# IvanPopov/video-flow-ml

Hardware: AMD Instinct MI355X
Metric: flow-fields/sec @1080p seq5 MOF_sintel (higher is better)
Workload: dtype mixed (per-layer MFMA count, f32 accumulate): {"corr": 1, "update_block.encoder.convf1": 1, "update_block.encoder.convf2": 1, "update_block.gru.convq1.iter": "2a", "update_block.gru.convzr1.iter": 1, "update_block.gru.convzr2.iter": 1, "update_block.mask.0": 1, "update_block.mask.2": 1, "update_bloc

## Files before the change

include/vfml.h:

```cpp
#ifndef VFML_H
#define VFML_H
#include <stddef.h>
#include <stdint.h>

#ifdef __cplusplus
extern "C" {
#endif

#define VFML_ABI_VERSION 27

enum {
  VFML_EPI_NONE = 0,
  VFML_EPI_RELU = 1,
  VFML_EPI_TANH = 2,
  VFML_EPI_SIGMOID = 3,
  VFML_EPI_TANH_RELU = 4,
  VFML_EPI_GRU_ZR = 5,
  VFML_EPI_GRU_Q = 6,
  VFML_EPI_ADD_AUX = 7,
};

enum { VFML_FMT_F32 = 0, VFML_FMT_S16 = 1,
       VFML_FMT_F16 = 2 };

// ... 25 lines not shown

int vfml_conv2d(const vfml_conv_desc* d, void* stream);

int vfml_conv2d_variant(const vfml_conv_desc* d, char* buf, int len);
int vfml_conv2d_split_variant(const vfml_conv_desc* d, const void* w_hi, const void* w_lo, int kp, float w_scale,
                              int in_fmt, int out_fmt, int aux_fmt, int k_order, char* buf, int len);
int vfml_conv2d_split_variant_at(int index, char* buf, int len);

int vfml_conv2d_split(const vfml_conv_desc* d, const void* w_hi, const void* w_lo, int kp, float w_scale,
                      int in_fmt, int out_fmt, int aux_fmt, int k_order, void* stream);
enum { VFML_KORDER_TAP = 0, VFML_KORDER_CBLOCK = 1, VFML_KORDER_CBLOCK64 = 2 };

int vfml_to_s16(const float* src, int64_t rows, int c, int ld_src, float* dst, int ld_dst, float scale, void* stream);

int vfml_split_f16(const float* src, int64_t rows, int k, int ld, float scale, void* hi, void* lo, int kp,
                   void* stream);

int vfml_softmax_rows_s16(const float* x, int64_t rows, int cols, int64_t ld_in, float* out, int64_t ld_out, float scale,
                          void* stream);

int vfml_softmax_rows_f16(const float* x, int64_t rows, int cols, int64_t ld_in, void* out, int64_t ld_out, float scale,
                          void* stream);

int64_t vfml_attention_plane_workspace_bytes(int p);
int vfml_attention_plane_f16(const float* q, int64_t ld_q, const float* k, int64_t ld_k, int p, int d, float score_scale,
                             float prob_scale, void* plane, int64_t ld_plane, void* workspace, void* stream);

int vfml_attention_bank_planes_f16(const float* q, int64_t ld_q, const float* const* keys, int64_t ld_k, int n_seg, int p, int d,
                                   float score_scale, float prob_scale, void* const* planes, int64_t ld_plane, void* workspace,
                                   void* stream);

int vfml_axpy_f32(const float* x, float* y, int64_t n, float scale, void* stream);

int vfml_transpose_to_s16(const float* src, int rows, int c, int ld, float scale, float* dst, int64_t ld_dst, void* stream);

enum { VFML_DW_RESIDUAL = 1, VFML_DW_GELU = 2 };
int vfml_dwconv2d(const float* x, int64_t ld_x, int n, int h, int w, int c, int k, const float* weight, const float* bias,
                  float* out, int64_t ld_out, int in_fmt, int out_fmt, int flags, void* stream);

int vfml_gelu_rows(const float* x, int64_t ld_x, float* out, int64_t ld_out, int64_t rows, int c, int in_fmt, int out_fmt,
                   void* stream);

int vfml_layernorm_rows(const float* x, int64_t ld_x, float* out, int64_t ld_out, int64_t rows, int c, const float* gamma,
                        const float* beta, float eps, int in_fmt, int out_fmt, void* stream);

int vfml_window_attention(const float* qkv, int64_t ld, int n, int h, int w, int c, int heads, int ws, const float* pad_row,
                          float* out, int64_t ld_out, int in_fmt, int out_fmt, void* stream);

int vfml_attention_shared_keys(const float* q, int64_t ld_q, const float* kv, int64_t ld_kv, int n, int p, int pk, int c, int heads,
                               float* out, int64_t ld_out, int q_fmt, int kv_fmt, int out_fmt, void* stream);

int vfml_add_to_s16(const float* x, int64_t ldx, const float* aux, int64_t ld_aux, float* out, int64_t ld_out, int64_t rows,
                    int c, float scale, void* stream);

int vfml_transpose_split_f16(const float* src, int rows, int c, int ld, float scale, void* hi, void* lo, int kp,
                             void* stream);

int vfml_frames_to_nhwc4(const void* src, int kind, int n, int H, int W,
                         float scale, float shift, float* dst, void* stream);

int64_t vfml_instnorm_workspace_bytes(int n, int hw, int c);
int vfml_instnorm_stats(const float* x, int n, int hw, int c, float eps,
                        float* stats, void* workspace, void* stream);
int vfml_instnorm_apply(const float* x, const float* stats, const float* res,
                        const float* res_stats, int n, int hw, int c, float* out, int out_fmt, void* stream);

int vfml_avgpool2x2(const float* x, int n, int h, int w, int c, float* out, void* stream);

int vfml_corr_lookup(const float* const* pyr, const int32_t* hl, const int32_t* wl,
                     const int32_t* ld, int levels, int radius, int nmaps, int q_per_map,
                     const float* coords, int ld_coords, float* out, int ld_out, int out_fmt, int vol_fmt, int vol_tile,
                     void* stream);
#define VFML_VOL_F16_LEVELS(m) (0x100 | (m))

int vfml_corr_lookup_indirect(const float* const* table, const int32_t* hl, const int32_t* wl, const int32_t* ld,
                              int levels, int radius, int nmaps, int q_per_map, const float* coords, int ld_coords,
                              float* out, int ld_out, int out_fmt, int vol_fmt, int vol_tile, void* stream);
int vfml_corr_lookup_indirect_bidir(const float* const* table, const int32_t* hl, const int32_t* wl, const int32_t* ld,
                                    int levels, int radius, int nmaps, int q_per_map, const float* coords, int ld_coords,
                                    int dir_coords, float* out, int ld_out, int dir_out, int dir_tab, int out_fmt, int vol_fmt,
                                    int vol_tile, void* stream);
int vfml_ptr_table_set(void* table, const void* const* ptrs, int n, void* stream);

#define VFML_SEED_NONE 0
#define VFML_SEED_LOAD 1
#define VFML_SEED_STORE 2
int vfml_window_seed(const void* cells, int ncentres, int rows, int cols, float* state, int ld_state, int h_off, int mf_off,
                     int ld_ctx, void* stream);

int vfml_flow_rows7(const float* flow, int n, int h, int w, float* rows, void* stream);

int vfml_conv3x3_c64(const float* in, int ld_in, int n, int h, int w, const void* w_hi, const void* w_lo, int kp, float w_scale,
                     const float* bias, float* out, int ldo, double* stats_part, void* stream);

int vfml_flow_half(const float* flow, int n, int h, int w, const void* w1_hi, int kp1, float w1_scale, const float* b1,
                   const void* w2_hi, int kp2, float w2_scale, const float* b2, float* out, int ld_out, void* stream);

int vfml_tapsum3x3(const float* t, int ld_t, const float* bias, int n, int h, int w, float* out, int parts, int64_t part_stride,
                   void* stream);
int vfml_tapsum3x3_update(const float* t, int ld_t, const float* bias, int n, int h, int w, int parts, int64_t part_stride,
                          float* coords1, float* flow_a, int ld_a, float* flow_b, int ld_b, int fmt_b, void* stream);

int vfml_coords_update(float* coords1, const float* delta, int n, int h, int w,
                       float* flow_a, int ld_a, float* flow_b, int ld_b, int fmt_b, void* stream);

int64_t vfml_flow_forward_interpolate_workspace_bytes(int n, int h, int w);
int vfml_flow_forward_interpolate(const float* flow, int ld_in, int n, int h, int w, float* out, int ld_out, int32_t* index,
                                  void* workspace, int64_t workspace_bytes, void* stream);
int vfml_coords_init(float* coords1, int n, int h, int w, void* stream);

int vfml_convex_upsample(const float* coords1, int ch, const float* mask, int ld_mask,
                         int h, int w, float* out, void* stream);

int64_t vfml_instnorm_finalize_workspace_bytes(int chunks, int c);
int vfml_instnorm_finalize(const double* part, int n, int chunks, int c, int hw, float eps, float* stats,
                           void* workspace, int64_t workspace_bytes, void* stream);

int vfml_stem7x7s2_chunks(int h, int w);
int vfml_stem7x7s2(const float* frames, int n, int h, int w, const void* w_hi, const void* w_lo, float w_scale,
                   const float* bias, float* out, double* stats_part, void* stream);

int vfml_flow_lod(const float* flow, int h, int w, float* out, void* stream);

enum { VFML_ENCODE_GAMEDEV = 0, VFML_ENCODE_RG8 = 1, VFML_ENCODE_RGB8 = 2 };
int vfml_flow_encode(const float* flow, int h, int w, int mode, float width, float height, float scale,
                     float clamp, float two_clamp, unsigned char* out, void* stream);

enum { VFML_TAA_SIMPLE = 0, VFML_TAA_BILINEAR = 1, VFML_TAA_BILATERAL = 2 };
enum { VFML_PIX_U8 = 0, VFML_PIX_F32 = 1, VFML_PIX_F64 = 2 };
int vfml_taa_blend(const void* current, int cur_type, const float* flow, const void* history, int hist_type,
                   void* out, int out_type, int h, int w, int mode, double alpha, double sigma_color, void* stream);

int vfml_flow_quality_map(const unsigned char* frame1, const unsigned char* frame2, const float* flow, int fh, int fw,
                          int h, int w, float threshold, unsigned char* out, void* stream);

#define VFML_CORRECT_RECORD 16
size_t vfml_flow_correct_workspace_bytes(int h, int w);
int vfml_flow_correct(const unsigned char* frame1, const unsigned char* frame2, const float* flow, const float* lod,
                      int lh, int lw, int h, int w, const double* twiddles, double good_threshold,
                      double fine_threshold, double region_radius, double template_radius, double search_radius,
                      float* out_flow, int* counts, double* records, int64_t record_capacity, void* workspace,
                      size_t workspace_bytes, void* stream);

enum { VFML_COLORIZE_HSV = 0, VFML_COLORIZE_WHEEL = 1 };
int vfml_flow_colorize(const float* flow, int h, int w, int mode, void* workspace, unsigned char* out, void* stream);

int vfml_flow_decode(const unsigned char* encoded, int h, int w, int mode, float clamp, float* flow, void* stream);

int vfml_flow_diff_overlay(const float* flow_a, const float* flow_b, int h, int w, unsigned char* out, void* stream);

enum { VFML_COMPOSE_SIDE_BY_SIDE = 0, VFML_COMPOSE_STACKED = 1, VFML_COMPOSE_GRID_2X2 = 2,
       VFML_COMPOSE_GRID_2X3 = 3 };
enum { VFML_COMPOSE_BGR = 1, VFML_COMPOSE_BOTTOM_UP = 2 };
int vfml_compose_frame(const void* const* tiles, const int* tile_types, int h, int w, int layout, int flags,
                       int64_t row_stride, unsigned char* out, void* stream);

int vfml_text_draw(const int32_t* plan, int plan_words, unsigned char* img, int h, int w, int64_t row_stride, int flags,
                   void* stream);

size_t vfml_flow_turbulence_workspace_bytes(int h, int w);
int vfml_flow_turbulence_map(const float* flow, int fh, int fw, int h, int w, int ksize, void* workspace,
                             unsigned char* out_bgr, unsigned char* out_index, float* out_tv, float* out_lohi,
                             void* stream);

int vfml_resize_u8(const unsigned char* src, int n, int H, int W, int64_t src_frame_stride, unsigned char* dst, int h,
                   int w, int64_t dst_frame_stride, const int32_t* xtab, const int32_t* ytab, void* stream);
// ... 67 lines not shown
```

video-flow-ml_amd/processing/videoflow_processor.py:

```python
import collections
import hashlib
import os

import numpy as np
import torch

from .videoflow_core import VideoFlowCore

try:
    import xxhash

    def _digest(buf):
        return xxhash.xxh3_128_digest(buf)
except ImportError:
    def _digest(buf):
        return hashlib.blake2b(buf, digest_size=16).digest()

HOST_FRAME_CACHE = 24


class VideoFlowProcessor:
    def __init__(self, device, fast_mode=False, tile_mode=False, sequence_length=5,
                 dataset='sintel', architecture='mof', variant='standard'):
        self.device = device
        self.fast_mode = fast_mode
        self.tile_mode = tile_mode
        self.sequence_length = sequence_length
        self.dataset = dataset
        self.architecture = architecture
        self.variant = variant
        self.core = VideoFlowCore(device, fast_mode, dataset, architecture, variant)
        self._dev_frames = collections.OrderedDict()
        print("VideoFlow Processor initialized:")
        for label, value in (("Device", device), ("Fast mode", fast_mode), ("Tile mode", tile_mode),
                             ("Sequence length", sequence_length), ("Dataset", dataset),
                             ("Architecture", architecture.upper()), ("Variant", variant)):
            print(f"  {label}: {value}")

    def load_model(self):
        print(f"VideoFlow model loaded successfully from: {self.core.load_model()}")

    def calculate_tile_grid(self, width, height, tile_size=1280):
        cols = -(-width // tile_size)
        rows = -(-height // tile_size)
        tiles = [{'x': c * tile_size, 'y': r * tile_size,
                  'width': min(tile_size, width - c * tile_size),
                  'height': min(tile_size, height - r * tile_size),
                  'col': c, 'row': r}
                 for r in range(rows) for c in range(cols)]
        return tile_size, tile_size, cols, rows, tiles

    def extract_tile(self, frame, tile_info):
        x, y = tile_info['x'], tile_info['y']
        return frame[y:y + tile_info['height'], x:x + tile_info['width']]

    def window_indices(self, num_frames, frame_idx):
        T = self.sequence_length
        half = T // 2
        start = max(0, frame_idx - half)
        idx = list(range(start, min(num_frames, frame_idx + half + 1)))
        while len(idx) < T:
            if start == 0:
                idx.insert(0, idx[0])
            else:
                idx.append(idx[-1])
        return idx[:T]

    def prepare_frame_sequence(self, frames, frame_idx):
        planes = []
        for i in self.window_indices(len(frames), frame_idx):
            f = frames[i]
            a = f.astype(np.float32) / 255.0 if f.dtype == np.uint8 else f.astype(np.float32)
            planes.append(torch.from_numpy(a).permute(2, 0, 1))
        return torch.stack(planes).unsqueeze(0).to(self.device)

    def _require_model(self):
        if not self.core.is_model_loaded():
            raise RuntimeError("Model not loaded. Call load_model() first.")

    def _flow_from_host_u8(self, frames, frame_idx):
        model = self.core.model
        if not (str(self.device).startswith('cuda') and hasattr(model, "forward_u8")):
            return None
        ids = self.window_indices(len(frames), frame_idx)
        f0 = frames[ids[0]]
        if not all(isinstance(frames[i], np.ndarray) and frames[i].dtype == np.uint8 and frames[i].ndim == 3 and
                   frames[i].shape == f0.shape for i in set(ids)):
            return None
        H, W, C = f0.shape
        if C != 3 or H % 8 or W % 8:
            return None
        keys = {}
        for i in set(ids):
            a = np.ascontiguousarray(frames[i])
            k = ("host-u8", _digest(memoryview(a).cast("B")), a.shape)
            keys[i] = k
            if k in self._dev_frames:
                self._dev_frames.move_to_end(k)
            else:
                self._dev_frames[k] = torch.from_numpy(a).to(self.device)
                while len(self._dev_frames) > HOST_FRAME_CACHE:
                    self._dev_frames.popitem(last=False)
        win = torch.stack([self._dev_frames[keys[i]] for i in ids])
        flows, _ = model.forward_u8(win, return_lowres=False, frame_keys=[keys[i] for i in ids], pick_only=self.PICK_ONLY)
        return flows[0, flows.shape[1] // 2].permute(1, 2, 0).cpu().numpy()

    def compute_optical_flow(self, frames, frame_idx):
        self._require_model()
        fast = self._flow_from_host_u8(frames, frame_idx)
        if fast is not None:
            return fast
        flow = self.core.compute_flow_from_tensor(self.prepare_frame_sequence(frames, frame_idx))
        return flow.permute(1, 2, 0).cpu().numpy()

    def compute_optical_flow_with_progress(self, frames, frame_idx, tile_pbar=None):
        self._require_model()

        def step(desc, n=0, reset=False):
            if tile_pbar is not None:
                tile_pbar.set_description(desc)
                if reset:
                    tile_pbar.reset()
                if n:
                    tile_pbar.update(n)

        step("Preparing frames", reset=True)
        fast = self._flow_from_host_u8(frames, frame_idx)
        if fast is not None:
            step("Completed", 4)
            return fast
        batch = self.prepare_frame_sequence(frames, frame_idx)
        step("Running VideoFlow", 2)
        flow = self.core.compute_flow_from_tensor(batch)
        step("Processing output", 1)
        out = flow.permute(1, 2, 0).cpu().numpy()
        step("Completed", 1)
        return out

    def compute_optical_flow_tiled(self, frames, frame_idx, tile_pbar=None, overall_pbar=None):
        if not self.tile_mode:
            return self.compute_optical_flow(frames, frame_idx)
        height, width = frames[frame_idx].shape[:2]
        tiles = self.calculate_tile_grid(width, height)[4]
        full = np.zeros((height, width, 2), dtype=np.float32)
        for k, t in enumerate(tiles):
            if overall_pbar is not None:
                overall_pbar.set_description(f"Tile {k + 1}/{len(tiles)} ({t['width']}x{t['height']})")
            crops = [self.extract_tile(f, t) for f in frames]
            full[t['y']:t['y'] + t['height'], t['x']:t['x'] + t['width']] = \
                self.compute_optical_flow_with_progress(crops, frame_idx, tile_pbar)
            if overall_pbar is not None:
                overall_pbar.update(1)
        return full

    def upload_clip(self, frames):
        if any(f.dtype != np.uint8 for f in frames):
            raise ValueError("upload_clip expects uint8 frames")
        from vfml.clip_id import clip_token
        host = torch.from_numpy(np.stack(frames))
        if str(self.device).startswith('cuda'):
            host = host.pin_memory()
        clip = host.to(self.device, non_blocking=True)
        clip_token(clip)
        return clip

    def compute_optical_flow_resident(self, clip, frame_idx, tile=None):
        self._require_model()
        from vfml.clip_id import clip_token
        from vfml.network import take_frames
        frame_ids = self.window_indices(clip.shape[0], frame_idx)
        win = take_frames(clip, frame_ids)
        rect = None
        if tile is not None:
            rect = (tile['x'], tile['y'], tile['width'], tile['height'])
            win = win[:, tile['y']:tile['y'] + tile['height'], tile['x']:tile['x'] + tile['width']]
        H, W = win.shape[1:3]
        model = self.core.model
        if H % 8 == 0 and W % 8 == 0 and hasattr(model, "forward_u8"):
            tok = clip_token(clip)
            keys = [(tok, i, rect) for i in frame_ids]
            flows, _ = model.forward_u8(win, return_lowres=False, frame_keys=keys, pick_only=self.PICK_ONLY)
            if ((tile is None or getattr(self, "tiles_in_frame_order", False)) and frame_idx + 1 < clip.shape[0]
                    and hasattr(model, "prefetch_frames")):
                nxt = self.window_indices(clip.shape[0], frame_idx + 1)
                if (nxt != frame_ids and nxt == list(range(nxt[0], nxt[0] + len(nxt)))
                        and max(nxt) <= getattr(clip, "_vfml_frames_ready", clip.shape[0]) - 1):
                    nwin = take_frames(clip, nxt)
                    if tile is not None:
                        nwin = nwin[:, tile['y']:tile['y'] + tile['height'], tile['x']:tile['x'] + tile['width']]
                    model.prefetch_frames(nwin, [(tok, i, rect) for i in nxt])
            return flows[0, flows.shape[1] // 2].permute(1, 2, 0)
        batch = (win.float() / 255.0).permute(0, 3, 1, 2).unsqueeze(0)
        return self.core.compute_flow_from_tensor(batch).permute(1, 2, 0)

    def compute_optical_flow_resident_batch(self, clip, frame_idxs):
        self._require_model()
        from vfml.clip_id import clip_token
        from vfml.network import take_frames
        model = self.core.model
        frame_idxs = list(frame_idxs)
        F, H, W = clip.shape[0], clip.shape[1], clip.shape[2]
        can_batch = getattr(model, "tri_frame", False) and hasattr(model, "forward_u8") and H % 8 == 0 and W % 8 == 0
        lo = self.sequence_length // 2 - 1
        triples = [self.window_indices(F, i)[lo:lo + 3] if self.sequence_length >= 3 else None for i in frame_idxs]
        out, k = [], 0
        while k < len(frame_idxs):
            e = k
            if can_batch and triples[k] is not None and triples[k][0] + 1 == triples[k][1] == triples[k][2] - 1:
                while (e + 1 < len(frame_idxs) and e + 1 - k < self.TRI_BATCH and
                       triples[e + 1] == [t + 1 for t in triples[e]]):
                    e += 1
            if e == k:
                out.append(self.compute_optical_flow_resident(clip, frame_idxs[k]))
            else:
                B = e - k + 1
                ids = list(range(triples[k][0], triples[e][2] + 1))
                tok = clip_token(clip)
                keys = [(tok, i, None) for i in ids]
                flows, _ = model.forward_u8(take_frames(clip, ids), return_lowres=False, frame_keys=keys, tri_batch=True)
                out.extend(flows[0, B + j].permute(1, 2, 0) for j in range(B))
            k = e + 1
        return out

    TRI_BATCH = int(os.environ.get("VFML_TRI_BATCH", "8"))
    PICK_ONLY = not os.environ.get("VFML_FULL_OUTPUT")

    def is_model_loaded(self):
        return self.core.is_model_loaded()

    def get_model_info(self):
        info = self.core.get_model_info()
        if info["status"] == "loaded":
            info.update(tile_mode=self.tile_mode, sequence_length=self.sequence_length,
                        processor_type="VideoFlowProcessor")
        return info

    def get_memory_usage(self):
        return self.core.get_memory_usage()

    def validate_frames(self, frames, frame_idx):
        if not isinstance(frames, list):
            raise ValueError("Frames must be a list of numpy arrays")
        if not frames:
            raise ValueError("Frames list cannot be empty")
        if not 0 <= frame_idx < len(frames):
            raise ValueError(f"Frame index {frame_idx} out of range [0, {len(frames)-1}]")
        f = frames[0]
        if not isinstance(f, np.ndarray):
            raise ValueError("Frames must be numpy arrays")
        if f.ndim != 3:
            raise ValueError(f"Frames must be 3D arrays [H,W,C], got shape {f.shape}")
        if f.shape[2] != 3:
            raise ValueError(f"Frames must have 3 color channels, got {f.shape[2]}")
        if f.dtype not in (np.uint8, np.float32, np.float64):
            raise ValueError(f"Unsupported frame dtype: {f.dtype}")
        if f.dtype != np.uint8:
            lo, hi = float(f.min()), float(f.max())
            if (hi > 1.0 or lo < 0.0) and not (hi <= 255.0 and lo >= 0.0):
                raise ValueError("Float frames must be in range [0.0, 1.0] or [0.0, 255.0]")

    def set_tile_mode(self, enabled):
        self.tile_mode = enabled

    def set_sequence_length(self, length):
# ... 4 lines not shown
```

video-flow-ml_amd/vfml/csrc/conv_gemm_split.hip:

```cpp
#include "conv_split_common.h"

namespace {

template <int BN, int WM, int WN, bool BIGC, bool IN16, int NM = 3>
__global__ __launch_bounds__(WM * WN * 64, 2) void conv_gemm_split_kernel(const SplitArgs a) {
  constexpr bool ALO = NM == 3 || NM == 2, BLO = NM == 3 || NM == 4;
  constexpr int NT = WM * WN * 64;
  constexpr int LR = NT / 4;
  constexpr int TM = BM / (WM * 32);
  constexpr int TN = BN / (WN * 32);
  constexpr int AU = BM / LR;
  constexpr int BU = BN / LR;
  constexpr int BUN = BU > 0 ? BU : 1;
  constexpr int RSA = BM + 2;
  constexpr int RSB = BN + 2;
  constexpr int SA = KG * RSA;
  constexpr int SB = KG * RSB;
  constexpr int LDC = BN + 4;

  extern __shared__ __attribute__((aligned(16))) char smem_raw[];
  h16x8* sAh = reinterpret_cast<h16x8*>(smem_raw);
  h16x8* sAl = sAh + 2 * SA;
  h16x8* sBh = sAl + 2 * SA;
  h16x8* sBl = sBh + 2 * SB;
  float* sC = reinterpret_cast<float*>(smem_raw);

  const int nwg = a.mtiles * a.ntiles;
  int bid = blockIdx.x;
  {
    const int q = nwg >> 3, r = nwg & 7, xcd = bid & 7;
    bid = (xcd < r ? xcd * (q + 1) : r * (q + 1) + (xcd - r) * q) + (bid >> 3);
  }
  const int nt = bid % a.ntiles;
  const int mt = bid / a.ntiles;
  const int m0 = mt * BM;
  const int n0 = nt * BN;

  const int t = threadIdx.x;
  const int kg = t & 3;
  const int lrow = t >> 2;

  int rp0[AU], rp1[AU];
  unsigned long long tapok[AU];
#pragma unroll
  for (int i = 0; i < AU; ++i) {
    const int m = m0 + lrow + LR * i;
    int iy0[1], ix0[1];
    tapok[i] = 0ull;
    if (m < a.M) {
      const int hw = a.ho * a.wo;
      const int n = m / hw;
      const int rem = m - n * hw;
      const int oy = rem / a.wo;
      const int ox = rem - oy * a.wo;
      iy0[0] = oy * a.stride - a.pad_h;
      ix0[0] = ox * a.stride - a.pad_w;
      const int pix = (n * a.H + iy0[0]) * a.W + ix0[0];
      rp0[i] = pix * a.ld0 + a.d0off;
      rp1[i] = pix * a.ld1 + a.d1off;
      for (int ky = 0; ky < a.kh; ++ky)
        for (int kx = 0; kx < a.kw; ++kx)
          if ((unsigned)(iy0[0] + ky) < (unsigned)a.H && (unsigned)(ix0[0] + kx) < (unsigned)a.W)
            tapok[i] |= 1ull << (ky * a.kw + kx);
    } else {
      rp0[i] = rp1[i] = 0;
    }
  }
  int kc[2], kky[2], kkx[2];
#pragma unroll
  for (int hf = 0; hf < 2; ++hf) {
    const int k = kg * 8 + hf * 4;
    const int tap = k / a.ctot;
    kc[hf] = k - tap * a.ctot;
    kky[hf] = tap / a.kw;
    kkx[hf] = tap - kky[hf] * a.kw;
  }
  int colbase[BUN];
#pragma unroll
  for (int i = 0; i < BUN; ++i) {
    const int col = n0 + lrow + LR * i;
    const bool colok = (BU > 0 || lrow < BN) && col < a.cout;
    colbase[i] = colok ? col * a.Kp * 2 : 0x40000000;
  }
// ... 96 lines not shown
      for (int e = 0; e < 16; ++e) acc[i][j][e] = 0.f;

  auto compute = [&](int buf) {
    const int oa = buf * SA + wm * (BM / WM) + r;
    const int ob = buf * SB + wn * (BN / WN) + r;
#pragma unroll
    for (int ks = 0; ks < KG / 2; ++ks) {
      h16x8 ah[TM], al[TM], bh[TN], bl[TN];
#pragma unroll
      for (int i = 0; i < TM; ++i) {
        ah[i] = sAh[oa + (2 * ks + half) * RSA + i * 32];
        if constexpr (ALO) al[i] = sAl[oa + (2 * ks + half) * RSA + i * 32];
      }
#pragma unroll
      for (int j = 0; j < TN; ++j) {
        bh[j] = sBh[ob + (2 * ks + half) * RSB + j * 32];
        if constexpr (BLO) bl[j] = sBl[ob + (2 * ks + half) * RSB + j * 32];
      }
#pragma unroll
      for (int i = 0; i < TM; ++i)
#pragma unroll
        for (int j = 0; j < TN; ++j) {
          acc[i][j] = __builtin_amdgcn_mfma_f32_32x32x16_f16(ah[i], bh[j], acc[i][j], 0, 0, 0);
          if constexpr (BLO) acc[i][j] = __builtin_amdgcn_mfma_f32_32x32x16_f16(ah[i], bl[j], acc[i][j], 0, 0, 0);
          if constexpr (ALO) acc[i][j] = __builtin_amdgcn_mfma_f32_32x32x16_f16(al[i], bh[j], acc[i][j], 0, 0, 0);
        }
    }
  };

  const int nk = ((a.K + BK - 1) / BK + 1) & ~1;
  load_tile(st0, 0);
  load_tile(st1, BK);
  store_tile(st0, 0);
  __syncthreads();
  for (int kt = 0; kt < nk; kt += 2) {
    load_tile(st0, (kt + 2) * BK);
    __builtin_amdgcn_sched_barrier(0);
    compute(0);
    __builtin_amdgcn_sched_barrier(0);
    store_tile(st1, 1);
    __syncthreads();
    load_tile(st1, (kt + 3) * BK);
    __builtin_amdgcn_sched_barrier(0);
    compute(1);
    __builtin_amdgcn_sched_barrier(0);
    store_tile(st0, 0);
    __syncthreads();
  }

  acc_to_lds<TM, TN, LDC>(acc, sC, wm * (BM / WM), wn * (BN / WN), r, half);
  __syncthreads();
  if (!epilogue_rows_fast<BN, NT>(a, sC, m0, n0, t, BM, 32, 0)) epilogue_rows<BN, NT>(a, sC, m0, n0, t);
  if (a.stats_part) {
    constexpr int RG = NT / BN;
    const int ch = t % BN, rg = t / BN;
    double s1 = 0.0, s2 = 0.0;
    if (n0 + ch < a.cout) {
      const float b = a.bias ? a.bias[n0 + ch] : 0.f;
      for (int row = rg; row < BM; row += RG) {
        if (m0 + row >= a.M) break;
        const double v = (double)((sC[row * LDC + ch] * a.w_inv + b) * a.out_scale);
        s1 += v;
        s2 += v * v;
      }
    }
    __syncthreads();
    double* fold = reinterpret_cast<double*>(sC);
    fold[(rg * BN + ch) * 2] = s1;
    fold[(rg * BN + ch) * 2 + 1] = s2;
    __syncthreads();
    if (rg == 0 && n0 + ch < a.cout) {
      for (int g = 1; g < RG; ++g) {
        s1 += vfml_lds_f64(&fold[(g * BN + ch) * 2]);
        s2 += vfml_lds_f64(&fold[(g * BN + ch) * 2 + 1]);
      }
      double* o = a.stats_part + ((int64_t)(m0 / BM) * a.cout + n0 + ch) * 2;
      o[0] = s1;
      o[1] = s2;
    }
  }
}



template <bool H16, bool BIAS>
__device__ __forceinline__ void gemm_resident_walk(const SplitArgs& a, char* smem) {
  constexpr int NW = 4;
  constexpr int RBM = 128, RBN = 64;
  constexpr int NSTEP = VFML_RESIDENT_KMAX / 64;
  constexpr int ASTEP = RBM * 128, BSTEP = RBN * 128;
  constexpr int BOFF = 0, BBUF = NSTEP * BSTEP, SLAB = BOFF + 2 * BBUF;
  constexpr int AP = RBM / (8 * NW), BP = RBN / (8 * NW);
  constexpr int ES = H16 ? 2 : 4;
  constexpr int NSTORE = 8, NSTORE_T = 16;
  constexpr int STORE_NT = 2;
  static_assert(NSTEP * ASTEP == 2 * BBUF, "the A image of a unit fills the two B buffers");
  static_assert(SLAB + NW * 32 * 32 * 4 == VFML_RESIDENT_LDS, "LDS budget of the resident-A walk: two workgroups per CU");

  const int t = threadIdx.x;
  const int lane = t & 63;
  const int wave = __builtin_amdgcn_readfirstlane(t >> 6);
  const int lrow = 8 * wave + (lane >> 3);
  const int piece = (lane & 7) ^ ((4 * wave + (lane >> 4)) & 7);
  const int nk = (a.Kp / 64 + 1) & ~1;
  const __amdgpu_buffer_rsrc_t rb = __builtin_amdgcn_make_buffer_rsrc(const_cast<char*>(a.wbase), 0, a.bytesb, 0x00020000);
  const int r = lane & 31, half = lane >> 5;
  const int q16 = (((r >> 1) & 7) ^ half) * 16;
  const int aoff = (wave * 32 + r) * 128 + q16;
  const int boff = r * 128 + q16;
  float* ws = reinterpret_cast<float*>(smem + SLAB) + wave * (32 * 32);
  const int c4 = (lane % 8) * 4, rr = lane / 8;

  const int units = a.mtiles * a.res_nc;
  for (int u = blockIdx.x; u < units; u += gridDim.x) {
    const int run = u / a.mtiles, mt = u - run * a.mtiles;
    const int nt0 = run * a.res_cl;
    const int nt1 = nt0 + a.res_cl < a.ntiles ? nt0 + a.res_cl : a.ntiles;
    const int m0 = mt * RBM;
    const int rows_valid = a.M - m0 < RBM ? a.M - m0 : RBM;
    __amdgpu_buffer_rsrc_t r0;
    if (a.tilebase)
      r0 = __builtin_amdgcn_make_buffer_rsrc(const_cast<float*>(a.in0) + (int64_t)m0 * a.ld0, 0,
                                             ((rows_valid - 1) * a.ld0 + a.d0off + a.c0) * 4, 0x00020000);
    else
      r0 = __builtin_amdgcn_make_buffer_rsrc(const_cast<float*>(a.in0), 0, a.bytes0, 0x00020000);
    int va[AP];
#pragma unroll
    for (int j = 0; j < AP; ++j) {
      const int m = m0 + 8 * NW * j + lrow;
      const int mrow = a.tilebase ? m - m0 : m;
      va[j] = m < a.M ? (mrow * a.ld0 + a.d0off) * 4 + piece * 32 : OOB;
    }
    auto issue_b = [&](int nt, int buf) {
      int colbase[BP];
#pragma unroll
      for (int j = 0; j < BP; ++j) {
        const int col = nt * RBN + 8 * NW * j + lrow;
        colbase[j] = col < a.cout ? a.whi_off + col * a.Kp * 2 + piece * 16 : (a.bhi ? 0x7ffffff0 : 0x40000000);
      }
      for (int s = 0; s < nk; ++s)
#pragma unroll
        for (int j = 0; j < BP; ++j)
          dma16(rb, colbase[j], s * 128, smem + BOFF + buf * BBUF + s * BSTEP + wave * (8 * 128) + j * (8 * NW * 128));
    };

    h16x8 af[4 * NSTEP];
#pragma unroll
    for (int q = 0; q < 4 * NSTEP; ++q) af[q] = h16x8{0, 0, 0, 0, 0, 0, 0, 0};
    lds_barrier();
    for (int s = 0; s < nk; ++s) {
      const bool past = s * 64 >= a.ctot;
#pragma unroll
      for (int j = 0; j < AP; ++j)
        dma16(r0, past ? OOB : va[j], s * 256, smem + s * ASTEP + wave * (8 * 128) + j * (8 * NW * 128));
    }
    asm volatile("s_waitcnt vmcnt(0)" ::: "memory");
    lds_barrier();
    static_for<NSTEP>([&](auto sc) {
      constexpr int s = decltype(sc)::value;
      if (s < nk) {
#pragma unroll
        for (int ks = 0; ks < 4; ++ks) af[s * 4 + ks] = *reinterpret_cast<const h16x8*>(smem + s * ASTEP + (aoff ^ (ks * 32)));
      }
    });
    lds_barrier();
    issue_b(nt0, 0);

    for (int nt = nt0; nt < nt1; ++nt) {
      const int buf = (nt - nt0) & 1;
      const int n0 = nt * RBN;
      if (nt == nt0) asm volatile("s_waitcnt vmcnt(0)" ::: "memory");
      else if (a.out_t) asm volatile("s_waitcnt vmcnt(%0)" ::"n"(NSTORE_T) : "memory");
      else asm volatile("s_waitcnt vmcnt(%0)" ::"n"(NSTORE) : "memory");
      lds_barrier();
      f32x4 bv[2] = {{0.f, 0.f, 0.f, 0.f}, {0.f, 0.f, 0.f, 0.f}};
      if constexpr (BIAS) {
#pragma unroll
        for (int j = 0; j < 2; ++j)
          if (n0 + j * 32 + c4 < a.cout) bv[j] = *reinterpret_cast<const f32x4*>(a.bias + n0 + j * 32 + c4);
      }
      if (nt + 1 < nt1) issue_b(nt + 1, buf ^ 1);

      f32x16 acc[2];
#pragma unroll
      for (int j = 0; j < 2; ++j)
#pragma unroll
        for (int e = 0; e < 16; ++e) acc[j][e] = 0.f;
      const char* bb = smem + BOFF + buf * BBUF;
      static_for<NSTEP / 2>([&](auto pc) {
        constexpr int s0 = 2 * decltype(pc)::value;
        if (s0 < nk) {
          h16x8 b0[8], b1[8];
#pragma unroll
          for (int q = 0; q < 8; ++q) {
            b0[q] = *reinterpret_cast<const h16x8*>(bb + (s0 + (q >> 2)) * BSTEP + (boff ^ ((q & 3) * 32)));
            b1[q] = *reinterpret_cast<const h16x8*>(bb + (s0 + (q >> 2)) * BSTEP + (boff ^ ((q & 3) * 32)) + 4096);
          }
#pragma unroll
          for (int q = 0; q < 8; ++q) {
            acc[0] = __builtin_amdgcn_mfma_f32_32x32x16_f16(af[s0 * 4 + q], b0[q], acc[0], 0, 0, 0);
            acc[1] = __builtin_amdgcn_mfma_f32_32x32x16_f16(af[s0 * 4 + q], b1[q], acc[1], 0, 0, 0);
          }
        }
      });

      const int cols_valid = a.cout - n0 < RBN ? a.cout - n0 : RBN;
      char* tbase = reinterpret_cast<char*>(a.out) + ((int64_t)m0 * a.ldo + n0) * ES;
      const __amdgpu_buffer_rsrc_t ro =
          __builtin_amdgcn_make_buffer_rsrc(tbase, 0, ((rows_valid - 1) * a.ldo + cols_valid) * ES, 0x00020000);
      const int rows_t = cols_valid, cols_t = rows_valid;
      __amdgpu_buffer_rsrc_t rt = ro;
      if (a.out_t) {
        char* tbase_t = reinterpret_cast<char*>(a.out_t) + ((int64_t)n0 * a.ld_out_t + m0) * ES;
        rt = __builtin_amdgcn_make_buffer_rsrc(tbase_t, 0, ((rows_t - 1) * a.ld_out_t + cols_t) * ES, 0x00020000);
      }
      static_for<2>([&](auto jc) {
        constexpr int j = decltype(jc)::value;
        const int gcol = j * 32 + c4;
#pragma unroll
        for (int e = 0; e < 16; ++e) ws[((e & 3) + 8 * (e >> 2) + 4 * half) * 32 + r] = acc[j][e];
#pragma unroll
        for (int p = 0; p < 4; ++p) {
          f32x4 v = *reinterpret_cast<const f32x4*>(ws + (p * 8 + rr) * 32 + c4);
#pragma unroll
          for (int e = 0; e < 4; ++e) {
            v[e] = (v[e] * a.w_inv + bv[j][e]) * a.out_scale;
            if (a.epilogue == VFML_EPI_RELU) v[e] = fmaxf(v[e], 0.f);
          }
          const int off = gcol < cols_valid ? ((wave * 32 + p * 8 + rr) * a.ldo + gcol) * ES : OOB;
          if constexpr (H16) {
            const h16x2 p0 = {(_Float16)v[0], (_Float16)v[1]}, p1 = {(_Float16)v[2], (_Float16)v[3]};
            const u32x2 hv = {__builtin_bit_cast(unsigned, p0), __builtin_bit_cast(unsigned, p1)};
            __builtin_amdgcn_raw_buffer_store_b64(hv, ro, off, 0, STORE_NT);
          } else {
            __builtin_amdgcn_raw_buffer_store_b128(__builtin_bit_cast(u32x4, v), ro, off, 0, STORE_NT);
          }
        }
        if (a.out_t) {
#pragma unroll
          for (int e = 0; e < 16; ++e) {
            const int row = (e & 3) + 8 * (e >> 2) + 4 * half;
            ws[r * 32 + ((row + (r >> 1)) & 31)] = acc[j][e];
          }
          const int g = lane >> 3, cl = lane & 7;
#pragma unroll
          for (int pp = 0; pp < 4; ++pp) {
            const int c = pp * 8 + cl;
            f32x4 v;
#pragma unroll
            for (int k = 0; k < 4; ++k) v[k] = ws[c * 32 + ((4 * g + k + (c >> 1)) & 31)] * a.w_inv * a.out_scale;
            const int trow = j * 32 + c;
            const int q0 = wave * 32 + 4 * g;
            const bool ok = trow < rows_t && q0 < cols_t;
            if constexpr (H16) {
              const h16x2 p0 = {(_Float16)v[0], (_Float16)v[1]}, p1 = {(_Float16)v[2], (_Float16)v[3]};
              const u32x2 hv = {__builtin_bit_cast(unsigned, p0), __builtin_bit_cast(unsigned, p1)};
              __builtin_amdgcn_raw_buffer_store_b64(hv, rt, ok ? (trow * a.ld_out_t + q0) * 2 : OOB, 0, STORE_NT);
            } else {
              __builtin_amdgcn_raw_buffer_store_b128(__builtin_bit_cast(u32x4, v), rt, ok ? (trow * a.ld_out_t + q0) * 4 : OOB, 0, STORE_NT);
            }
          }
        }
      });
    }
  }
}

template <int TM, int TN, int WM, int WN, bool PERSIST, bool FASTK, bool CSWAP = false, int NM = 3, bool MF16 = false, bool H16 = false>
__global__ __launch_bounds__(WM * WN * 64, (WM * WN == 4 ? 2 : 1)) void conv_gemm_dma_kernel(const SplitArgs a) {
  static_assert(!H16 || PERSIST, "VFML_FMT_F16 outputs (H16) exist in the persistent GEMM form only");
  static_assert(!(MF16 && PERSIST), "the persistent GEMM form runs 32x32x16 MFMAs (its 16x16x32 epilogue branches below are not maintained)");
  constexpr bool H64 = NM == 5;
  static_assert(!H64 || FASTK, "64-channel steps exist for the uniform-step loader only");
  constexpr bool BHI = NM == 2 || NM == 1 || H64;
  constexpr bool AHI = NM == 4 || NM == 1 || H64;
  constexpr int KSTEP = H64 ? 64 : BK;
  constexpr int NW = WM * WN, NT = NW * 64;
  constexpr int TBM = 32 * TM * WM, TBN = 32 * TN * WN;
  constexpr int AP = TBM / (8 * NW), BP = TBN / (8 * NW);
  static_assert(TBM % (8 * NW) == 0 && TBN % (8 * NW) == 0, "tile rows must split into whole pieces per wave");
  constexpr int ASZ = TBM * 128, BSZ = TBN * 128, STG = ASZ + BSZ;
  constexpr int LDC = TBN + 4;

  extern __shared__ __attribute__((aligned(16))) char smem_raw[];
  float* sC = reinterpret_cast<float*>(smem_raw);

  if constexpr (PERSIST && FASTK && !CSWAP && NM == 5 && !MF16) {
    if (a.resident) {
      if (a.bias) gemm_resident_walk<H16, true>(a, smem_raw);
      else gemm_resident_walk<H16, false>(a, smem_raw);
      return;
    }
  }

  const int total = a.mtiles * a.ntiles * (PERSIST ? a.ksplit : 1);
  int tile, tile_end, tile_step;
  {
    const int G = gridDim.x, xcd = blockIdx.x & 7, lw = blockIdx.x >> 3;
    const int q = total >> 3, r = total & 7;
    const int start = xcd < r ? xcd * (q + 1) : r * (q + 1) + (xcd - r) * q;
    tile_step = (G - xcd + 7) >> 3;
    tile = start + lw;
    tile_end = start + q + (xcd < r ? 1 : 0);
  }
  if (tile >= tile_end) return;

  const int t = threadIdx.x;
  const int lane = t & 63;
  const int wave = __builtin_amdgcn_readfirstlane(t >> 6);
  const int lrow = 8 * wave + (lane >> 3);
  const int piece = (lane & 7) ^ (MF16 && !H64 ? swz16((4 * wave + (lane >> 4)) & 7) : ((4 * wave + (lane >> 4)) & 7));
  const int kg = piece >> 1, hl = piece & 1;

  int rp0[AP], rp1[AP];
  unsigned long long tapok[AP];
  int colbase[BP];
  int kc, kky, kkx;
  int scb = 0, sky = 0, skx = 0;
  int m0, n0;
  int ks = 0;
  __amdgpu_buffer_rsrc_t r0 = __builtin_amdgcn_make_buffer_rsrc(
      reinterpret_cast<char*>(const_cast<float*>(a.in0)) - a.abias, 0, a.bytes0 + a.abias, 0x00020000);
  const __amdgpu_buffer_rsrc_t rb = __builtin_amdgcn_make_buffer_rsrc(const_cast<char*>(a.wbase), 0, a.bytesb, 0x00020000);

  const int nk = PERSIST && a.ksplit == 2 ? (((a.Kp / KSTEP + 1) >> 1) + 1) & ~1 : (a.Kp / KSTEP + 1) & ~1;
  auto setup = [&](int tl) {
    int nt, mt;
    if (PERSIST && a.ksplit == 2) {
      ks = tl & 1;
      tl >>= 1;
    }
    if (a.ntiles >= 8) {
      constexpr int GM = 8;
      const int gsz = GM * a.ntiles;
      const int g = tl / gsz, rem = tl - g * gsz;
      const int left = a.mtiles - g * GM;
      const int mrows = left < GM ? left : GM;
      nt = rem / mrows;
      mt = g * GM + (rem - nt * mrows);
    } else {
      nt = tl % a.ntiles;
      mt = tl / a.ntiles;
    }
    m0 = mt * TBM;
    n0 = nt * TBN;
#pragma unroll
    for (int j = 0; j < AP; ++j) {
      const int m = m0 + 8 * NW * j + lrow;
      tapok[j] = 0ull;
// ... 1030 lines not shown
             (out_fmt == VFML_FMT_F32 || out_fmt == VFML_FMT_F16) && !d->stats_part &&
             (d->cout >= DIRECT_MIN_COUT || out_fmt == VFML_FMT_F16) && d->cout % 4 == 0 && d->ldo % 4 == 0 && vfml_aligned16(d->out) &&
             (!d->bias || vfml_aligned16(d->bias));
  VFML_REQUIRE(out_fmt != VFML_FMT_F16 || (a.direct && a.fastk),
               "vfml_conv2d_split: VFML_FMT_F16 outputs are written by the GEMM form only (1x1 over whole 32-channel blocks, no "
               "addend / activation beyond ReLU, cout %% 4 == 0, ldo %% 4 == 0, 16-byte aligned out)");
  if (d->flags & VFML_CONV_SWAP_CROSS) {
    VFML_REQUIRE(a.direct && a.fastk, "vfml_conv2d_split: VFML_CONV_SWAP_CROSS is implemented by the GEMM form only "
                                      "(1x1 over whole 32-channel blocks, plain f32 out, cout >= 1024, cout %% 4 == 0)");
    a.cswap = 1;
  }
  if (bhi)
    VFML_REQUIRE(a.direct && a.fastk && !a.cswap, "vfml_conv2d_split: a weight operand without lo plane is implemented by the "
                                                    "GEMM form only (1x1 over whole 32-channel blocks, plain f32 out, cout >= 1024)");
  if (d->out_t) {
    VFML_REQUIRE(a.direct && a.fastk && a.pointwise && !d->bias && d->epilogue == VFML_EPI_NONE && a.M % 4 == 0 &&
                 d->ld_out_t % 4 == 0 && d->ld_out_t >= a.M && vfml_aligned16(d->out_t),
                 "vfml_conv2d_split: out_t needs the GEMM form (1x1 over whole 32-channel blocks, plain f32 out, cout >= 1024, cout %% 4 == 0), no bias / "
                 "epilogue, pixels %% 4 == 0, ld_out_t %% 4 == 0 and >= pixels, 16-byte alignment");
    a.out_t = d->out_t; a.ld_out_t = d->ld_out_t;
  }
  if (d->ksplit_ws) {
    VFML_REQUIRE(vfml_aligned16(d->ksplit_ws), "vfml_conv2d_split: ksplit_ws must be 16-byte aligned");
    const int64_t tiles = (int64_t)((a.M + 127) / 128) * ((d->cout + 127) / 128);
    const bool ksplit = a.direct && a.fastk && a.pointwise && out_fmt == VFML_FMT_F32 && !a.cswap && tiles <= 256 &&
                        kp >= 4096;
    if (ksplit) {
      a.ksplit = 2;
      a.out_k1 = d->ksplit_ws;
      a.out_t_k1 = d->ksplit_ws + (int64_t)a.M * d->ldo;
    }
  }
  if (d->proj_out) {
    VFML_REQUIRE(d->epilogue == VFML_EPI_RELU && !d->addend && !d->stats_part && !d->out_t && !a.direct,
                 "vfml_conv2d_split: proj_out goes with VFML_EPI_RELU, no addend / stats_part / out_t");
    VFML_REQUIRE(a.fastk && (a.nm == 3 || a.nm == 4) && d->cout % 128 == 0,
                 "vfml_conv2d_split: proj_out needs the uniform-step loader (channel-block weight order, whole 32-channel "
                 "blocks), the full split product or VFML_CONV_MFMA2A (which then holds for the projection too) and "
                 "cout %% 128 == 0");
    VFML_REQUIRE(d->proj_hi && d->proj_lo && d->proj_n > 0 && d->proj_n <= 48 && d->proj_n % 4 == 0 && d->proj_kp >= d->cout &&
                     d->proj_kp % 8 == 0 && d->ld_proj >= d->proj_n && d->ld_proj % 4 == 0 && vfml_aligned16(d->proj_out) &&
                     vfml_aligned16(d->proj_hi) && vfml_aligned16(d->proj_lo) && d->proj_scale > 0.f,
                 "vfml_conv2d_split: proj_hi / proj_lo [proj_n <= 48, %% 4 == 0][proj_kp >= cout] f16 planes, ld_proj >= proj_n, "
                 "16-byte alignment");
    const char* ph2 = (const char*)d->proj_hi;
    const char* pl2 = (const char*)d->proj_lo;
    const int64_t plane = (int64_t)d->proj_n * d->proj_kp * 2;
    VFML_REQUIRE(pl2 >= ph2 && (pl2 - ph2) + plane < (1ll << 30), "vfml_conv2d_split: proj_lo must follow proj_hi within 1 GiB");
    a.proj_w = ph2; a.proj_lo_off = (int)(pl2 - ph2); a.proj_bytes = (int)((pl2 - ph2) + plane);
    a.proj_n = d->proj_n; a.proj_kp = d->proj_kp; a.proj_inv = 1.0f / d->proj_scale;
    a.proj_out = d->proj_out; a.ld_proj = d->ld_proj;
  }
  return 0;
}

static int dma_tile_env() {
  const char* tile_env = getenv("VFML_DMA_TILE");
  if (!tile_env) return 0;
  int tm = 2, tn = 2, wm = 2, wn = 2;
  sscanf(tile_env, "%d,%d,%d,%d", &tm, &tn, &wm, &wn);
  return tm * 1000 + tn * 100 + wm * 10 + wn;
}

static int split_prepare(const vfml_conv_desc* d, const void* w_hi, const void* w_lo, int kp, float w_scale, int in_fmt, int out_fmt,
                         int aux_fmt, int k_order, int forced_tile, SplitArgs& a, SplitPlan& plan, const SplitVariant*& row) {
  if (const int rc = split_fill(d, w_hi, w_lo, kp, w_scale, in_fmt, out_fmt, aux_fmt, k_order, a)) return rc;
  if (const int rc = vfml_detail::plan_split(a, in_fmt == VFML_FMT_S16, d->flags, forced_tile, &plan)) return rc;
  a.nm = plan.nm;
  a.fastk = plan.fastk;
  a.resident = plan.resident ? 1 : 0;
  if (!plan.fastk) a.abias = 0;
  row = plan.family == vfml_detail::SPLIT_TAPX ? vfml_detail::tapx_variant(plan)
        : plan.family == vfml_detail::SPLIT_DMA ? vfml_detail::find_variant(DMA_VARIANTS, sizeof(DMA_VARIANTS) / sizeof(DMA_VARIANTS[0]), plan)
                                                : vfml_detail::find_variant(REG_VARIANTS, sizeof(REG_VARIANTS) / sizeof(REG_VARIANTS[0]), plan);
  if (!row) {
    char name[160];
    vfml_detail::variant_name(plan, name, sizeof(name));
    vfml_set_error("vfml_conv2d_split: no such variant: %s", name);
    return 1;
  }
  return 0;
}

extern "C" int vfml_conv2d_split(const vfml_conv_desc* d, const void* w_hi, const void* w_lo, int kp, float w_scale,
                                 int in_fmt, int out_fmt, int aux_fmt, int k_order, void* stream) {
  SplitArgs a;
  SplitPlan plan;
  const SplitVariant* row;
  if (const int rc = split_prepare(d, w_hi, w_lo, kp, w_scale, in_fmt, out_fmt, aux_fmt, k_order, dma_tile_env(), a, plan, row)) return rc;
  hipStream_t s = reinterpret_cast<hipStream_t>(stream);
  const int rc = row->launch(a, s);
  if (rc || !plan.add_rows) return rc;
  const int64_t quads = (int64_t)a.M * (d->cout / 4);
  const dim3 grid((unsigned)((quads + 255) / 256 < 65535 * 16 ? (quads + 255) / 256 : 65535 * 16));
  hipLaunchKernelGGL(add_rows_kernel, grid, dim3(256), 0, s, d->out, d->ksplit_ws, a.M, d->cout / 4, d->ldo);
  if (d->out_t)
    hipLaunchKernelGGL(add_rows_kernel, grid, dim3(256), 0, s, d->out_t, a.out_t_k1, d->cout, a.M / 4, d->ld_out_t);
  return vfml_check_launch("vfml_conv2d_split");
}

extern "C" int vfml_conv2d_split_variant(const vfml_conv_desc* d, const void* w_hi, const void* w_lo, int kp, float w_scale,
                                         int in_fmt, int out_fmt, int aux_fmt, int k_order, char* buf, int len) {
  VFML_REQUIRE(buf && len > 0, "vfml_conv2d_split_variant: no buffer");
  SplitArgs a;
  SplitPlan plan;
  const SplitVariant* row;
  if (const int rc = split_prepare(d, w_hi, w_lo, kp, w_scale, in_fmt, out_fmt, aux_fmt, k_order, dma_tile_env(), a, plan, row)) return rc;
  VFML_REQUIRE(vfml_detail::variant_name(row->key, buf, len) < len, "vfml_conv2d_split_variant: the name needs more than %d bytes", len);
  return 0;
}


extern "C" int vfml_conv2d_split_variant_at(int index, char* buf, int len) {
  VFML_REQUIRE(buf && len > 0, "vfml_conv2d_split_variant_at: no buffer");
  constexpr int nreg = (int)(sizeof(REG_VARIANTS) / sizeof(REG_VARIANTS[0])), ndma = (int)(sizeof(DMA_VARIANTS) / sizeof(DMA_VARIANTS[0]));
  if (index < 0) return 1;
  const SplitVariant* row = index < nreg          ? &REG_VARIANTS[index]
                            : index < nreg + ndma ? &DMA_VARIANTS[index - nreg]
                                                  : vfml_detail::tapx_variant_at(index - nreg - ndma);
  if (!row) return 1;
  VFML_REQUIRE(vfml_detail::variant_name(row->key, buf, len) < len, "vfml_conv2d_split_variant_at: the name needs more than %d bytes", len);
  return 0;
}
```

video-flow-ml_amd/vfml/csrc/conv_split_common.h:

```cpp
#pragma once
#include <hip/hip_fp16.h>
#include <stdlib.h>
#include <utility>
#include "vfml_common.h"


namespace vfml_detail {
struct SplitArgs {
  const float* in0; const float* in1;
  const _Float16* whi; const _Float16* wlo; const float* bias;
  const float* aux0; const float* aux1; const float* addend;
  float* out;
  int c0, ld0, c1, ld1, ctot, ld_addend;
  int H, W, ho, wo;
  int kh, kw, stride, pad_h, pad_w;
  int M, K, Kp, cout;
  int d0off, d1off;
  int bytes0, bytesw;
  int ldo, ld_aux0, ld_aux1;
  int epilogue, split;
  float out_scale, w_inv;
  int mtiles, ntiles;
  int vec_ok;
  int out16, aux16;
  int out_h16;
  const char* wbase; int whi_off, wlo_off, bytesb;
  int korder;
  int direct;
  int pointwise;
  int fastk, abias, src1_delta;
  int tilebase;
  float* out_t; int ld_out_t;
  int cswap;
  int bhi;
  double* stats_part;
  int nm;
  int ksplit; float* out_k1; float* out_t_k1;
  const char* proj_w; int proj_lo_off, proj_bytes, proj_n, proj_kp; float proj_inv; float* proj_out; int ld_proj;
  const float* const* addend_ind;
  int resident, res_nc, res_cl;
};
#define VFML_RESIDENT_KMAX 256
#define VFML_RESIDENT_LDS (80 * 1024)
#define VFML_TAPX_KWMAX 5

enum SplitFamily { SPLIT_REG, SPLIT_DMA, SPLIT_TAPX };
struct SplitPlan {
  SplitFamily family;
  int bn;
  int tm, tn;
  int wm, wn;
  bool bigc, in16;
  bool persist, fastk, cswap, mf16, h16;
  int nm;
  bool add_rows;
  bool resident;
};
int plan_split(const SplitArgs& a, bool in16, int flags, int forced_tile, SplitPlan* plan);
constexpr SplitPlan reg_plan(int bn, int wm, int wn, bool bigc, bool in16, int nm) {
  return {SPLIT_REG, bn, 0, 0, wm, wn, bigc, in16, false, false, false, false, false, nm, false};
}
constexpr SplitPlan dma_plan(int tm, int tn, int wm, int wn, bool persist, bool fastk, bool cswap, int nm, bool mf16, bool h16) {
  return {SPLIT_DMA, 0, tm, tn, wm, wn, false, false, persist, fastk, cswap, mf16, h16, nm, false};
}
constexpr SplitPlan tapx_plan(int tm, int tn, int wm, int wn, int nm) {
  return {SPLIT_TAPX, 0, tm, tn, wm, wn, false, false, false, true, false, true, false, nm, false};
}
struct SplitVariant {
  SplitPlan key;
  int (*launch)(SplitArgs& a, hipStream_t s);
};
const SplitVariant* find_variant(const SplitVariant* rows, size_t n, const SplitPlan& plan);
int variant_name(const SplitPlan& key, char* buf, int len);
const SplitVariant* tapx_variant(const SplitPlan& plan);
const SplitVariant* tapx_variant_at(int index);
}
using vfml_detail::SplitArgs;
using vfml_detail::SplitPlan;
using vfml_detail::SplitVariant;

namespace {

template <class F, int... I>
__device__ __forceinline__ void static_for_impl(F&& f, std::integer_sequence<int, I...>) {
  (f(std::integral_constant<int, I>{}), ...);
}
template <int N, class F>
__device__ __forceinline__ void static_for(F&& f) {
  static_for_impl(f, std::make_integer_sequence<int, N>{});
}

typedef _Float16 h16x8 __attribute__((ext_vector_type(8)));
typedef _Float16 h16x2 __attribute__((ext_vector_type(2)));
typedef __fp16 fp16x2 __attribute__((ext_vector_type(2)));

constexpr int BM = 128;
constexpr int BK = 32;
constexpr int KG = BK / 8;

typedef unsigned int u32x4 __attribute__((ext_vector_type(4)));
typedef unsigned int u32x2 __attribute__((ext_vector_type(2)));

__device__ __forceinline__ u32x4 bload16(__amdgpu_buffer_rsrc_t rsrc, int voff_bytes) {
  return __builtin_bit_cast(u32x4, __builtin_amdgcn_raw_buffer_load_b128(rsrc, voff_bytes, 0, 0));
}
constexpr int OOB = 0x7fffffff;

__device__ __forceinline__ float sigmoidf_(float v) { return 1.0f / (1.0f + expf(-v)); }

typedef const __attribute__((address_space(1))) float* vfml_gfptr;
typedef const __attribute__((address_space(1))) f32x4* vfml_gf4ptr;
__device__ __forceinline__ vfml_gfptr addend_of(const SplitArgs& a) {
  return (vfml_gfptr)(a.addend_ind ? *a.addend_ind : a.addend);
}

union U8 {
  h16x8 v;
  h16x2 p[4];
};

__device__ __forceinline__ void split4(const f32x4 x, U8& hi, U8& lo, int at) {
#pragma unroll
  for (int e = 0; e < 2; ++e) vfml_split2(x[2 * e], x[2 * e + 1], hi.p[at / 2 + e], lo.p[at / 2 + e]);
}

__device__ __forceinline__ float epi1(float v, int epilogue, bool lowhalf, float x0, float x1) {
  switch (epilogue) {
    case VFML_EPI_RELU: return fmaxf(v, 0.f);
    case VFML_EPI_TANH: return tanhf(v);
    case VFML_EPI_SIGMOID: return sigmoidf_(v);
    case VFML_EPI_TANH_RELU: return lowhalf ? tanhf(v) : fmaxf(v, 0.f);
    case VFML_EPI_GRU_ZR: v = sigmoidf_(v); return lowhalf ? v : v * x0;
    case VFML_EPI_GRU_Q: return (1.f - x0) * x1 + x0 * tanhf(v);
    case VFML_EPI_ADD_AUX: return x0 + v;
    default: return v;
  }
}

template <int TM, int TN, int LDC>
__device__ __forceinline__ void acc_to_lds(const f32x16 (&acc)[TM][TN], float* sC, int row0, int col0, int r, int half) {
#pragma unroll
  for (int j = 0; j < TN; ++j)
#pragma unroll
    for (int i = 0; i < TM; ++i)
#pragma unroll
      for (int e = 0; e < 16; ++e) {
        const int row = row0 + i * 32 + (e & 3) + 8 * (e >> 2) + 4 * half;
        const int col = col0 + j * 32 + r;
        sC[row * LDC + col] = acc[i][j][e];
      }
}

template <int BN, int NT>
__device__ __forceinline__ void epilogue_rows(const SplitArgs& a, const float* sC, int m0, int n0, int t,
                                              int nrows = BM, int rstride = 32, int roff = 0) {
  constexpr int LDC = BN + 4;
  constexpr int C8 = BN / 8;
  constexpr int RPP = NT / C8;
// ... 315 lines not shown
```

video-flow-ml_amd/vfml/csrc/flow_ops.hip:

```cpp
#include <stdlib.h>
#include "vfml_common.h"

namespace {

constexpr int MAX_LEVELS = 6;
constexpr int MAX_MAPS = 8;
constexpr int MAX_RADIUS = 4;
constexpr int PATCH = 2 * MAX_RADIUS + 2;
#ifndef VFML_LOOKUP_WAVES
#define VFML_LOOKUP_WAVES 4
#endif
constexpr int LOOKUP_WAVES = VFML_LOOKUP_WAVES;
constexpr int FIXED_LEVELS = 4;
static_assert(FIXED_LEVELS == 4, "corr_lookup_fixed_kernel selects among four levels");

struct LookupArgs {
  const float* pyr[MAX_MAPS][MAX_LEVELS];
  const float* const* table;
  int hl[MAX_LEVELS], wl[MAX_LEVELS], ld[MAX_LEVELS];
  int levels, radius, nq, q_per_map;
  const float* coords; int ld_coords;
  float* out; int ld_out;
  int out16;
  int vol16;
  int tws, ths;
  int qw;
  int dir_maps, dir_coords, dir_out;
  int dir_tab;
};

__device__ __forceinline__ void lookup_rows(const LookupArgs& a, int q, int& map, int64_t& crow, int64_t& orow) {
  const int dir = a.dir_maps && map >= a.dir_maps;
  const int64_t qd = q - (dir ? a.dir_maps * a.q_per_map : 0);
  if (dir) map += a.dir_tab - a.dir_maps;
  crow = qd * a.ld_coords + (dir ? a.dir_coords : 0);
  orow = qd * a.ld_out + (dir ? a.dir_out : 0);
}

__device__ __forceinline__ int tiled_at(int y, int x, int w, int tws, int ths) {
  const int tpr = (w + (1 << tws) - 1) >> tws;
  return ((((y >> ths) * tpr + (x >> tws)) << (tws + ths)) + ((y & ((1 << ths) - 1)) << tws) + (x & ((1 << tws) - 1)));
}

__device__ __forceinline__ float bilinear4(float nw, float ne, float sw, float se, float wx0, float fx, float wy0, float fy) {
  float v = ne * (fx * wy0);
  v = __builtin_fmaf(nw, wx0 * wy0, v);
  v = __builtin_fmaf(sw, wx0 * fy, v);
  v = __builtin_fmaf(se, fx * fy, v);
  return v;
}

__global__ __launch_bounds__(64 * LOOKUP_WAVES) void corr_lookup_kernel(const LookupArgs a) {
  __shared__ float patch[LOOKUP_WAVES][MAX_LEVELS][PATCH * PATCH];
  __shared__ float frac[LOOKUP_WAVES][MAX_LEVELS][2];
  const int lane = threadIdx.x & 63;
  const int wv = threadIdx.x >> 6;
  const int q = blockIdx.x * LOOKUP_WAVES + wv;
  const bool live = q < a.nq;
  int map = live ? q / a.q_per_map : 0;
  const int qq = q - map * a.q_per_map;
  const int side = 2 * a.radius + 2;
  const int win = 2 * a.radius + 1;
  const int psz = side * side;
  int64_t crow = 0, orow = 0;
  if (live) lookup_rows(a, q, map, crow, orow);
  if (live) {
    const float cx = a.coords[crow + 0];
    const float cy = a.coords[crow + 1];
    const int total = a.levels * psz;
    const int qrow = (a.tws | a.ths) ? tiled_at(qq / a.qw, qq % a.qw, a.qw, a.tws, a.ths) : qq;
    for (int e = lane; e < total; e += 64) {
      const int l = e / psz;
      const int idx = e - l * psz;
      const int py = idx / side, px = idx - py * side;
      const float inv = 1.0f / (float)(1 << l);
      const float x = cx * inv, y = cy * inv;
      const float fx0 = floorf(x), fy0 = floorf(y);
      const int x0 = (int)fminf(fmaxf(fx0, -65536.f), 65536.f) - a.radius;
      const int y0 = (int)fminf(fmaxf(fy0, -65536.f), 65536.f) - a.radius;
      const int xx = x0 + px, yy = y0 + py;
      float v = 0.f;
      if (xx >= 0 && xx < a.wl[l] && yy >= 0 && yy < a.hl[l])
        v = (a.table ? a.table[map * a.levels + l] : a.pyr[map][l])[(int64_t)qrow * a.ld[l] + tiled_at(yy, xx, a.wl[l], a.tws, a.ths)];
      patch[wv][l][idx] = v;
      if (idx == 0) {
        frac[wv][l][0] = x - fx0;
        frac[wv][l][1] = y - fy0;
      }
    }
  }
  __syncthreads();
  if (!live) return;
  const int nout = a.levels * win * win;
  float* o = a.out + orow;
  const int nwrite = a.out16 ? (nout + 7) & ~7 : nout;
  for (int c = lane; c < nwrite; c += 64) {
    if (c >= nout) {
      _Float16* u = reinterpret_cast<_Float16*>(o + (c & ~7));
      u[c & 7] = (_Float16)0.f;
      u[8 + (c & 7)] = (_Float16)0.f;
      continue;
    }
    const int l = c / (win * win);
    const int rem = c - l * win * win;
    const int i = rem / win, j = rem - i * win;
    const float fx = frac[wv][l][0], fy = frac[wv][l][1];
    const float* p = &patch[wv][l][j * side + i];
    const float wx0 = 1.f - fx, wy0 = 1.f - fy;
    const float v = bilinear4(p[0], p[1], p[side], p[side + 1], wx0, fx, wy0, fy);
    if (a.out16) {
      vfml_h16x2 hh, ll;
      vfml_split2(v, 0.f, hh, ll);
      _Float16* u = reinterpret_cast<_Float16*>(o + (c & ~7));
      u[c & 7] = hh[0];
      u[8 + (c & 7)] = ll[0];
    } else {
      o[c] = v;
    }
  }
}

__device__ __forceinline__ float bilinear4w(float nw, float ne, float sw, float se, float w00, float w10, float w01, float w11) {
  float v = ne * w10;
  v = __builtin_fmaf(nw, w00, v);
  v = __builtin_fmaf(sw, w01, v);
  v = __builtin_fmaf(se, w11, v);
  return v;
}

__device__ __forceinline__ void wave_lds_sync() {
  __builtin_amdgcn_fence(__ATOMIC_RELEASE, "workgroup");
  __builtin_amdgcn_wave_barrier();
  __builtin_amdgcn_fence(__ATOMIC_ACQUIRE, "workgroup");
}

template <int R, bool OUT16, int V16 = 0>
__global__ __launch_bounds__(64 * LOOKUP_WAVES) void corr_lookup_fixed_kernel(const LookupArgs a) {
  constexpr int SIDE = 2 * R + 2, PSZ = SIDE * SIDE, WIN = 2 * R + 1, WW = WIN * WIN;
  constexpr int NOUTPAD = (FIXED_LEVELS * WW + 7) & ~7;
  static_assert(PSZ <= 128 && FIXED_LEVELS * WIN <= 64 && NOUTPAD / 8 <= 64, "one wave: at most two gather passes per level");
  __shared__ float patch[LOOKUP_WAVES][FIXED_LEVELS][PSZ];
  __shared__ __attribute__((aligned(16))) float outs[LOOKUP_WAVES][NOUTPAD];
  const int lane = threadIdx.x & 63;
  const int wv = __builtin_amdgcn_readfirstlane(threadIdx.x >> 6);
  const int q = blockIdx.x * LOOKUP_WAVES + wv;
  if (q >= a.nq) return;
  int map = __builtin_amdgcn_readfirstlane(q / a.q_per_map);
  const int qq = q - map * a.q_per_map;
  const int qrow = __builtin_amdgcn_readfirstlane((a.tws | a.ths) ? tiled_at(qq / a.qw, qq % a.qw, a.qw, a.tws, a.ths) : qq);
  int64_t crow, orow;
  lookup_rows(a, q, map, crow, orow);
  const float cx = a.coords[crow + 0];
  const float cy = a.coords[crow + 1];
  const int pyA = lane / SIDE, pxA = lane - pyA * SIDE;
  const int pyB = (lane + 64) / SIDE, pxB = (lane + 64) - pyB * SIDE;
  const bool inB = lane + 64 < PSZ;
  const float* pl[FIXED_LEVELS];
  if (a.table) {
#pragma unroll
    for (int l = 0; l < FIXED_LEVELS; ++l) pl[l] = a.table[map * a.levels + (l < a.levels ? l : 0)];
  } else {
#pragma unroll
    for (int l = 0; l < FIXED_LEVELS; ++l) pl[l] = a.pyr[map][l < a.levels ? l : 0];
  }
  float va[FIXED_LEVELS], vb[FIXED_LEVELS];
  bool oka[FIXED_LEVELS], okb[FIXED_LEVELS];
#pragma unroll
  for (int l = 0; l < FIXED_LEVELS; ++l) {
    const bool have = l < a.levels;
    const int ll = have ? l : 0;
    const bool v16 = (V16 >> l) & 1;
    const int ES = v16 ? 2 : 4;
    const char* base = reinterpret_cast<const char*>(pl[l]) + (int64_t)qrow * a.ld[ll] * ES;
    const int wl = a.wl[ll], hl = a.hl[ll];
    const float inv = __builtin_bit_cast(float, (127 - l) << 23);
    const float x = cx * inv, y = cy * inv;
    const int x0 = (int)fminf(fmaxf(floorf(x), -65536.f), 65536.f) - R;
    const int y0 = (int)fminf(fmaxf(floorf(y), -65536.f), 65536.f) - R;
    auto texel = [&](int px, int py, bool in, float& out, bool& ok) {
      const int xx = x0 + px, yy = y0 + py;
      ok = have && in && xx >= 0 && xx < wl && yy >= 0 && yy < hl;
      const int at = tiled_at(min(max(yy, 0), hl - 1), min(max(xx, 0), wl - 1), wl, a.tws, a.ths);
      if (v16) out = (float)((const __attribute__((address_space(1))) _Float16*)base)[at];
      else out = ((const __attribute__((address_space(1))) float*)base)[at];
    };
    texel(pxA, pyA, true, va[l], oka[l]);
    if constexpr (PSZ > 64) texel(pxB, pyB, inB, vb[l], okb[l]);
    else { vb[l] = 0.f; okb[l] = false; }
  }
#pragma unroll
  for (int l = 0; l < FIXED_LEVELS; ++l) {
    va[l] = oka[l] ? va[l] : 0.f;
    vb[l] = okb[l] ? vb[l] : 0.f;
  }
#pragma unroll
  for (int l = 0; l < FIXED_LEVELS; ++l) {
    if (l < a.levels) {
      if (PSZ > 64 || lane < PSZ) patch[wv][l][lane] = va[l];
      if constexpr (PSZ > 64) if (inB) patch[wv][l][lane + 64] = vb[l];
    }
  }
  const int nout = a.levels * WW;
  const int nunits = (nout + 7) >> 3;
  if (lane >= 56 && nout + (lane - 56) < nunits * 8) outs[wv][nout + (lane - 56)] = 0.f;
  wave_lds_sync();
  if (lane < a.levels * WIN) {
    const int l = lane / WIN, i = lane - l * WIN;
    const float inv = __builtin_bit_cast(float, (127 - l) << 23);
    const float x = cx * inv, y = cy * inv;
    const float fx = x - floorf(x), fy = y - floorf(y);
    const float wx0 = 1.f - fx, wy0 = 1.f - fy;
    const float w00 = wx0 * wy0, w10 = fx * wy0, w01 = wx0 * fy, w11 = fx * fy;
    const float* p = &patch[wv][l][i];
    float* o = &outs[wv][l * WW + i * WIN];
    float nw = p[0], ne = p[1];
#pragma unroll
    for (int j = 0; j < WIN; ++j) {
      const float sw = p[(j + 1) * SIDE], se = p[(j + 1) * SIDE + 1];
      o[j] = bilinear4w(nw, ne, sw, se, w00, w10, w01, w11);
      nw = sw; ne = se;
    }
  }
  wave_lds_sync();
  if (lane < nunits) {
    float* o = a.out + orow + lane * 8;
    const f32x4 v0 = *reinterpret_cast<const f32x4*>(&outs[wv][lane * 8]);
    const f32x4 v1 = *reinterpret_cast<const f32x4*>(&outs[wv][lane * 8 + 4]);
    if (OUT16) {
      vfml_h16x2 h0, h1, h2, h3, l0, l1, l2, l3;
      vfml_split2(v0[0], v0[1], h0, l0);
      vfml_split2(v0[2], v0[3], h1, l1);
      vfml_split2(v1[0], v1[1], h2, l2);
      vfml_split2(v1[2], v1[3], h3, l3);
      uint4 hv, lv;
      hv.x = __builtin_bit_cast(unsigned, h0); hv.y = __builtin_bit_cast(unsigned, h1);
      hv.z = __builtin_bit_cast(unsigned, h2); hv.w = __builtin_bit_cast(unsigned, h3);
      lv.x = __builtin_bit_cast(unsigned, l0); lv.y = __builtin_bit_cast(unsigned, l1);
      lv.z = __builtin_bit_cast(unsigned, l2); lv.w = __builtin_bit_cast(unsigned, l3);
      *reinterpret_cast<uint4*>(o) = hv;
      *reinterpret_cast<uint4*>(o + 4) = lv;
    } else {
#pragma unroll
      for (int h = 0; h < 2; ++h) {
        const int c = lane * 8 + 4 * h;
        const f32x4 w = h ? v1 : v0;
        if (c + 3 < nout && (((uintptr_t)(o + 4 * h)) & 15u) == 0) {
          *reinterpret_cast<f32x4*>(o + 4 * h) = w;
        } else {
#pragma unroll
          for (int k = 0; k < 4; ++k)
            if (c + k < nout) o[4 * h + k] = w[k];
        }
      }
    }
  }
}

__global__ void coords_init_kernel(f32x4* __restrict__ coords, int h, int w, int64_t total) {
  for (int64_t p = (int64_t)blockIdx.x * blockDim.x + threadIdx.x; p < total; p += (int64_t)gridDim.x * blockDim.x) {
    const int x = (int)(p % w);
    const int y = (int)((p / w) % h);
// ... 483 lines not shown
```

video-flow-ml_amd/vfml/hip.py:

```python
import ctypes
import os
import subprocess
from ctypes import POINTER, c_char_p, c_double, c_float, c_int, c_int32, c_int64, c_void_p

import torch

_HERE = os.path.dirname(os.path.abspath(__file__))
LIB_PATH = os.environ.get("VFML_LIB") or os.path.join(_HERE, "libvfml_hip.so")
CSRC = os.path.join(_HERE, "csrc")
SOURCES = ["api.hip", "conv_gemm.hip", "conv_gemm_split.hip", "conv_gemm_tapx.hip", "conv_split_plan.hip", "stem.hip", "flow_half.hip", "enc_conv.hip", "norm_pool.hip", "flow_ops.hip", "effects.hip", "correct.hip", "render.hip", "text.hip", "turbulence.hip", "resize.hip", "jpeg.hip", "jpeg_decode.hip", "jpeg_decode_sync.hip", "deflate.hip", "attention.hip", "dwconv.hip", "twins.hip", "warm_start.hip"]

STATS_ROWS_F32, STATS_ROWS_S16 = 128, 32
EPI_NONE, EPI_RELU, EPI_TANH, EPI_SIGMOID, EPI_TANH_RELU, EPI_GRU_ZR, EPI_GRU_Q, EPI_ADD_AUX = range(8)
FMT_F32, FMT_S16, FMT_F16 = 0, 1, 2


def vol_f16_levels(mask):
    return 0x100 | mask


def _vol_mask(vol_fmt, levels):
    return (15 if vol_fmt == FMT_F16 else (vol_fmt & 15 if vol_fmt & 0x100 else 0)) & ((1 << levels) - 1)

KORDER_TAP, KORDER_CBLOCK, KORDER_CBLOCK64 = 0, 1, 2
CONV_SWAP_CROSS, CONV_MFMA2, CONV_MFMA1, CONV_MFMA2A, CONV_PER_TAP = 1, 2, 4, 8, 16


class ConvDesc(ctypes.Structure):
    _fields_ = [
        ("in0", c_void_p), ("c0", c_int32), ("ld0", c_int32),
        ("in1", c_void_p), ("c1", c_int32), ("ld1", c_int32),
        ("n", c_int32), ("h", c_int32), ("w", c_int32),
        ("weight", c_void_p), ("bias", c_void_p),
        ("cout", c_int32), ("kh", c_int32), ("kw", c_int32), ("stride", c_int32),
        ("pad_h", c_int32), ("pad_w", c_int32),
        ("out", c_void_p), ("ldo", c_int32),
        ("epilogue", c_int32), ("split", c_int32), ("out_scale", c_float),
        ("aux0", c_void_p), ("ld_aux0", c_int32),
        ("aux1", c_void_p), ("ld_aux1", c_int32),
        ("addend", c_void_p), ("ld_addend", c_int32),
        ("out_t", c_void_p), ("ld_out_t", c_int32),
        ("flags", c_int32),
        ("stats_part", c_void_p),
        ("ksplit_ws", c_void_p),
        ("proj_hi", c_void_p), ("proj_lo", c_void_p), ("proj_n", c_int32), ("proj_kp", c_int32), ("proj_scale", c_float),
        ("proj_out", c_void_p), ("ld_proj", c_int32),
        ("addend_ind", c_void_p),
    ]


COMMON_FLAGS = ["-fno-slp-vectorize"]
EXTRA_FLAGS = {}


def build(force=False, verbose=False):
    srcs = [os.path.join(CSRC, s) for s in SOURCES]
    hdrs = [os.path.join(CSRC, "vfml_common.h"), os.path.join(CSRC, "conv_split_common.h"),
            os.path.join(CSRC, "jet_table.inc"), os.path.join(CSRC, "jpeg_tables.inc"), os.path.join(CSRC, "jpeg_decode_common.h"),
            os.path.join(CSRC, "jpeg_sync_steps.h"), os.path.join(CSRC, "deflate_code.h"), os.path.join(_HERE, "..", "..", "include", "vfml.h")]
    deps = srcs + hdrs
    if not force and os.path.exists(LIB_PATH) and all(
            os.path.getmtime(LIB_PATH) >= os.path.getmtime(d) for d in deps):
        return LIB_PATH
    objdir = os.path.join(CSRC, "_obj")
    os.makedirs(objdir, exist_ok=True)
    newest_hdr = max(os.path.getmtime(h) for h in hdrs)
    jobs = []
    for src in srcs:
        obj = os.path.join(objdir, os.path.basename(src) + ".o")
        if force or not os.path.exists(obj) or os.path.getmtime(obj) < max(os.path.getmtime(src), newest_hdr):
            cmd = ["hipcc", "--offload-arch=gfx950", "-O3", "-std=c++17", "-fPIC"] + COMMON_FLAGS + EXTRA_FLAGS.get(os.path.basename(src), []) + [
                "-c", src, "-o", obj]
            if verbose:
                print(" ".join(cmd))
            jobs.append((cmd, subprocess.Popen(cmd)))
    for cmd, p in jobs:
        if p.wait() != 0:
            raise subprocess.CalledProcessError(p.returncode, cmd)
    cmd = ["hipcc", "--offload-arch=gfx950", "-fPIC", "-shared", "-o", LIB_PATH] + [
        os.path.join(objdir, os.path.basename(src) + ".o") for src in srcs]
    if verbose:
        print(" ".join(cmd))
    subprocess.run(cmd, check=True)
    return LIB_PATH


_lib = None


def lib():
    global _lib
    if _lib is not None:
        return _lib
    if not os.path.exists(LIB_PATH):
        raise RuntimeError(
            f"vfml HIP extension not built: {LIB_PATH} is missing. Run `python -c 'import __graft_entry__ as g; "
            f"g.build()'` (needs hipcc). There is no CPU fallback for the flow engine.")
    L = ctypes.CDLL(LIB_PATH)
    L.vfml_last_error.restype = c_char_p
    L.vfml_abi_version.restype = c_int
    L.vfml_conv2d.argtypes = [POINTER(ConvDesc), c_void_p]
    L.vfml_conv2d_split.argtypes = [POINTER(ConvDesc), c_void_p, c_void_p, c_int, c_float, c_int, c_int, c_int, c_int,
                                    c_void_p]
    L.vfml_conv2d_variant.argtypes = [POINTER(ConvDesc), c_char_p, c_int]
    L.vfml_conv2d_split_variant.argtypes = L.vfml_conv2d_split.argtypes[:-1] + [c_char_p, c_int]
    L.vfml_conv2d_split_variant_at.argtypes = [c_int, c_char_p, c_int]
    L.vfml_to_s16.argtypes = [c_void_p, c_int64, c_int, c_int, c_void_p, c_int, c_float, c_void_p]
    L.vfml_softmax_rows_s16.argtypes = [c_void_p, c_int64, c_int, c_int64, c_void_p, c_int64, c_float, c_void_p]
    L.vfml_transpose_split_f16.argtypes = [c_void_p, c_int, c_int, c_int, c_float, c_void_p, c_void_p, c_int, c_void_p]
    L.vfml_split_f16.argtypes = [c_void_p, c_int64, c_int, c_int, c_float, c_void_p, c_void_p, c_int, c_void_p]
    L.vfml_frames_to_nhwc4.argtypes = [c_void_p, c_int, c_int, c_int, c_int, c_float, c_float, c_void_p, c_void_p]
    L.vfml_instnorm_workspace_bytes.restype = c_int64
    L.vfml_instnorm_workspace_bytes.argtypes = [c_int, c_int, c_int]
    L.vfml_instnorm_stats.argtypes = [c_void_p, c_int, c_int, c_int, c_float, c_void_p, c_void_p, c_void_p]
    L.vfml_softmax_rows_f16.argtypes = [c_void_p, c_int64, c_int, c_int64, c_void_p, c_int64, c_float, c_void_p]
    L.vfml_attention_plane_workspace_bytes.restype = c_int64
    L.vfml_attention_plane_workspace_bytes.argtypes = [c_int]
    L.vfml_attention_plane_f16.argtypes = [c_void_p, c_int64, c_void_p, c_int64, c_int, c_int, c_float, c_float, c_void_p, c_int64,
                                           c_void_p, c_void_p]
    L.vfml_attention_bank_planes_f16.argtypes = [c_void_p, c_int64, POINTER(c_void_p), c_int64, c_int, c_int, c_int, c_float, c_float,
                                                 POINTER(c_void_p), c_int64, c_void_p, c_void_p]
    L.vfml_axpy_f32.argtypes = [c_void_p, c_void_p, c_int64, c_float, c_void_p]
    L.vfml_dwconv2d.argtypes = [c_void_p, c_int64, c_int, c_int, c_int, c_int, c_int, c_void_p, c_void_p, c_void_p, c_int64, c_int, c_int,
                                c_int, c_void_p]
    L.vfml_gelu_rows.argtypes = [c_void_p, c_int64, c_void_p, c_int64, c_int64, c_int, c_int, c_int, c_void_p]
    L.vfml_layernorm_rows.argtypes = [c_void_p, c_int64, c_void_p, c_int64, c_int64, c_int, c_void_p, c_void_p, c_float, c_int, c_int,
                                      c_void_p]
    L.vfml_window_attention.argtypes = [c_void_p, c_int64, c_int, c_int, c_int, c_int, c_int, c_int, c_void_p, c_void_p, c_int64,
                                        c_int, c_int, c_void_p]
    L.vfml_attention_shared_keys.argtypes = [c_void_p, c_int64, c_void_p, c_int64, c_int, c_int, c_int, c_int, c_int, c_void_p,
                                             c_int64, c_int, c_int, c_int, c_void_p]
    L.vfml_transpose_to_s16.argtypes = [c_void_p, c_int, c_int, c_int, c_float, c_void_p, c_int64, c_void_p]
    L.vfml_add_to_s16.argtypes = [c_void_p, c_int64, c_void_p, c_int64, c_void_p, c_int64, c_int64, c_int, c_float, c_void_p]
    L.vfml_instnorm_finalize.argtypes = [c_void_p, c_int, c_int, c_int, c_int, c_float, c_void_p, c_void_p, c_int64, c_void_p]
    L.vfml_instnorm_finalize_workspace_bytes.restype = c_int64
    L.vfml_instnorm_finalize_workspace_bytes.argtypes = [c_int, c_int]
    L.vfml_stem7x7s2_chunks.argtypes = [c_int, c_int]
    L.vfml_stem7x7s2.argtypes = [c_void_p, c_int, c_int, c_int, c_void_p, c_void_p, c_float, c_void_p, c_void_p, c_void_p, c_void_p]
    L.vfml_instnorm_apply.argtypes = [c_void_p, c_void_p, c_void_p, c_void_p, c_int, c_int, c_int, c_void_p, c_int, c_void_p]
    L.vfml_avgpool2x2.argtypes = [c_void_p, c_int, c_int, c_int, c_int, c_void_p, c_void_p]
    L.vfml_corr_lookup.argtypes = [POINTER(c_void_p), POINTER(c_int32), POINTER(c_int32), POINTER(c_int32),
                                   c_int, c_int, c_int, c_int, c_void_p, c_int, c_void_p, c_int, c_int, c_int, c_int, c_void_p]
    L.vfml_corr_lookup_indirect.argtypes = [c_void_p, POINTER(c_int32), POINTER(c_int32), POINTER(c_int32),
                                            c_int, c_int, c_int, c_int, c_void_p, c_int, c_void_p, c_int, c_int, c_int, c_int,
                                            c_void_p]
    L.vfml_corr_lookup_indirect_bidir.argtypes = [c_void_p, POINTER(c_int32), POINTER(c_int32), POINTER(c_int32),
                                                  c_int, c_int, c_int, c_int, c_void_p, c_int, c_int, c_void_p, c_int, c_int,
                                                  c_int, c_int, c_int, c_int, c_void_p]
    L.vfml_ptr_table_set.argtypes = [c_void_p, POINTER(c_void_p), c_int, c_void_p]
    L.vfml_window_seed.argtypes = [c_void_p, c_int, c_int, c_int, c_void_p, c_int, c_int, c_int, c_int, c_void_p]
    L.vfml_tapsum3x3_update.argtypes = [c_void_p, c_int, c_void_p, c_int, c_int, c_int, c_int, ctypes.c_int64, c_void_p, c_void_p,
                                        c_int, c_void_p, c_int, c_int, c_void_p]
    L.vfml_conv3x3_c64.argtypes = [c_void_p, c_int, c_int, c_int, c_int, c_void_p, c_void_p, c_int, c_float, c_void_p, c_void_p,
                                   c_int, c_void_p, c_void_p]
    L.vfml_flow_half.argtypes = [c_void_p, c_int, c_int, c_int, c_void_p, c_int, c_float, c_void_p, c_void_p, c_int, c_float,
                                 c_void_p, c_void_p, c_int, c_void_p]
    L.vfml_coords_init.argtypes = [c_void_p, c_int, c_int, c_int, c_void_p]
    L.vfml_flow_rows7.argtypes = [c_void_p, c_int, c_int, c_int, c_void_p, c_void_p]
    L.vfml_tapsum3x3.argtypes = [c_void_p, c_int, c_void_p, c_int, c_int, c_int, c_void_p, c_int, ctypes.c_int64, c_void_p]
    L.vfml_coords_update.argtypes = [c_void_p, c_void_p, c_int, c_int, c_int, c_void_p, c_int, c_void_p, c_int,
                                     c_int, c_void_p]
    L.vfml_flow_forward_interpolate_workspace_bytes.restype = c_int64
    L.vfml_flow_forward_interpolate_workspace_bytes.argtypes = [c_int, c_int, c_int]
    L.vfml_flow_forward_interpolate.argtypes = [c_void_p, c_int, c_int, c_int, c_int, c_void_p, c_int, c_void_p, c_void_p, c_int64,
                                                c_void_p]
    L.vfml_flow_lod.argtypes = [c_void_p, c_int, c_int, c_void_p, c_void_p]
    L.vfml_flow_encode.argtypes = [c_void_p, c_int, c_int, c_int, c_float, c_float, c_float, c_float, c_float, c_void_p,
                                   c_void_p]
    L.vfml_taa_blend.argtypes = [c_void_p, c_int, c_void_p, c_void_p, c_int, c_void_p, c_int, c_int, c_int, c_int, c_double,
                                 c_double, c_void_p]
    L.vfml_flow_quality_map.argtypes = [c_void_p, c_void_p, c_void_p, c_int, c_int, c_int, c_int, c_float, c_void_p, c_void_p]
    L.vfml_flow_correct_workspace_bytes.argtypes = [c_int, c_int]
    L.vfml_flow_correct_workspace_bytes.restype = ctypes.c_size_t
    L.vfml_flow_correct.argtypes = [c_void_p, c_void_p, c_void_p, c_void_p, c_int, c_int, c_int, c_int, c_void_p,
                                    c_double, c_double, c_double, c_double, c_double, c_void_p, c_void_p, c_void_p,
                                    ctypes.c_int64, c_void_p, ctypes.c_size_t, c_void_p]
    L.vfml_flow_colorize.argtypes = [c_void_p, c_int, c_int, c_int, c_void_p, c_void_p, c_void_p]
    L.vfml_flow_decode.argtypes = [c_void_p, c_int, c_int, c_int, c_float, c_void_p, c_void_p]
    L.vfml_flow_diff_overlay.argtypes = [c_void_p, c_void_p, c_int, c_int, c_void_p, c_void_p]
    L.vfml_compose_frame.argtypes = [POINTER(c_void_p), POINTER(c_int32), c_int, c_int, c_int, c_int, c_int64, c_void_p,
                                     c_void_p]
    L.vfml_text_draw.argtypes = [c_void_p, c_int, c_void_p, c_int, c_int, c_int64, c_int, c_void_p]
    L.vfml_flow_turbulence_workspace_bytes.argtypes = [c_int, c_int]
    L.vfml_flow_turbulence_workspace_bytes.restype = ctypes.c_size_t
    L.vfml_flow_turbulence_map.argtypes = [c_void_p, c_int, c_int, c_int, c_int, c_int, c_void_p, c_void_p, c_void_p, c_void_p,
                                           c_void_p, c_void_p]
    L.vfml_resize_u8.argtypes = [c_void_p, c_int, c_int, c_int, c_int64, c_void_p, c_int, c_int, c_int64, c_void_p, c_void_p,
                                 c_void_p]
    L.vfml_jpeg_workspace_bytes.restype = c_int64
    L.vfml_jpeg_workspace_bytes.argtypes = [c_int, c_int]
    L.vfml_jpeg_scan_capacity.restype = c_int64
    L.vfml_jpeg_scan_capacity.argtypes = [c_int, c_int]
    L.vfml_jpeg_encode_rgb.argtypes = [c_void_p, c_int, c_int, c_int64, c_void_p, c_void_p, c_void_p, c_int64, c_void_p,
                                       c_void_p]
    L.vfml_jpeg_sampled_workspace_bytes.restype = c_int64
    L.vfml_jpeg_sampled_workspace_bytes.argtypes = [c_int, c_int, c_int]
    L.vfml_jpeg_sampled_scan_capacity.restype = c_int64
    L.vfml_jpeg_sampled_scan_capacity.argtypes = [c_int, c_int, c_int]
    L.vfml_jpeg_encode_rgb_sampled.argtypes = [c_void_p, c_int, c_int, c_int64, c_int, c_void_p, c_void_p, c_void_p, c_int64,
                                               c_void_p, c_void_p]
    L.vfml_jpeg_decode_workspace_bytes.restype = c_int64
    L.vfml_jpeg_decode_workspace_bytes.argtypes = [c_int, c_int, c_int64]
    L.vfml_jpeg_decode_rgb.argtypes = [c_void_p, c_int64, c_int, c_int, c_int, c_void_p, c_void_p, c_int, c_int, c_void_p,
                                       c_void_p, c_int64, c_void_p, c_void_p]
    L.vfml_jpeg_decode_sync_workspace_bytes.restype = c_int64
    L.vfml_jpeg_decode_sync_workspace_bytes.argtypes = [c_int, c_int, c_int64, c_int]
    L.vfml_jpeg_decode_rgb_sync.argtypes = [c_void_p, c_int64, c_int, c_int, c_int, c_void_p, c_void_p, c_int, c_int, c_int,
                                            c_void_p, c_void_p, c_int64, c_void_p, c_void_p]
    L.vfml_jpeg_decode_sampled_workspace_bytes.restype = c_int64
    L.vfml_jpeg_decode_sampled_workspace_bytes.argtypes = [c_int, c_int, c_int, c_int64]
    L.vfml_jpeg_decode_rgb_sampled.argtypes = [c_void_p, c_int64, c_int, c_int, c_int, c_int, c_void_p, c_void_p, c_int, c_int,
                                               c_void_p, c_void_p, c_int64, c_void_p, c_void_p]
    L.vfml_jpeg_decode_sync_sampled_workspace_bytes.restype = c_int64
    L.vfml_jpeg_decode_sync_sampled_workspace_bytes.argtypes = [c_int, c_int, c_int, c_int64, c_int]
    L.vfml_jpeg_decode_rgb_sync_sampled.argtypes = [c_void_p, c_int64, c_int, c_int, c_int, c_int, c_void_p, c_void_p, c_int,
                                                    c_int, c_int, c_void_p, c_void_p, c_int64, c_void_p, c_void_p]
    for fn in (L.vfml_deflate_capacity, L.vfml_deflate_workspace_bytes, L.vfml_inflate_workspace_bytes):
        fn.restype = c_int64
        fn.argtypes = [c_int64, c_int]
    L.vfml_deflate_huffman.argtypes = [c_void_p, c_int64, c_int, ctypes.c_uint32, c_void_p, c_void_p, c_int64, c_void_p, c_void_p,
                                       c_void_p, c_void_p]
    L.vfml_inflate_chunks.argtypes = [c_void_p, c_int64, c_void_p, c_int, c_int, c_int64, ctypes.c_uint32, c_void_p, c_void_p,
                                      c_void_p, c_void_p, c_void_p]
    L.vfml_convex_upsample.argtypes = [c_void_p, c_int, c_void_p, c_int, c_int, c_int, c_void_p, c_void_p]
    for name in EXPORTS:
        getattr(L, name)
    if L.vfml_abi_version() != 27:
        raise RuntimeError("libvfml_hip.so ABI version mismatch")
    _lib = L
    return L


EXPORTS = [
    "vfml_conv2d", "vfml_conv2d_split", "vfml_conv2d_variant", "vfml_conv2d_split_variant", "vfml_conv2d_split_variant_at", "vfml_split_f16", "vfml_to_s16", "vfml_softmax_rows_s16", "vfml_softmax_rows_f16", "vfml_attention_plane_workspace_bytes", "vfml_attention_plane_f16", "vfml_attention_bank_planes_f16", "vfml_axpy_f32", "vfml_dwconv2d", "vfml_gelu_rows", "vfml_layernorm_rows", "vfml_window_attention", "vfml_attention_shared_keys", "vfml_transpose_to_s16", "vfml_add_to_s16",
    "vfml_transpose_split_f16", "vfml_frames_to_nhwc4", "vfml_instnorm_workspace_bytes", "vfml_instnorm_stats",
    "vfml_instnorm_apply", "vfml_instnorm_finalize", "vfml_instnorm_finalize_workspace_bytes", "vfml_avgpool2x2", "vfml_corr_lookup", "vfml_corr_lookup_indirect", "vfml_corr_lookup_indirect_bidir",
    "vfml_ptr_table_set", "vfml_window_seed", "vfml_coords_update", "vfml_coords_init", "vfml_tapsum3x3", "vfml_tapsum3x3_update", "vfml_flow_rows7", "vfml_flow_half", "vfml_conv3x3_c64",
    "vfml_flow_forward_interpolate_workspace_bytes", "vfml_flow_forward_interpolate",
    "vfml_convex_upsample", "vfml_stem7x7s2", "vfml_stem7x7s2_chunks", "vfml_flow_lod", "vfml_flow_encode", "vfml_taa_blend", "vfml_flow_quality_map", "vfml_flow_correct_workspace_bytes", "vfml_flow_correct",
    "vfml_flow_colorize", "vfml_compose_frame", "vfml_flow_decode", "vfml_flow_diff_overlay", "vfml_text_draw",
    "vfml_flow_turbulence_workspace_bytes", "vfml_flow_turbulence_map", "vfml_resize_u8",
    "vfml_jpeg_workspace_bytes", "vfml_jpeg_scan_capacity", "vfml_jpeg_encode_rgb",
    "vfml_jpeg_sampled_workspace_bytes", "vfml_jpeg_sampled_scan_capacity", "vfml_jpeg_encode_rgb_sampled",
    "vfml_jpeg_decode_workspace_bytes", "vfml_jpeg_decode_rgb",
    "vfml_jpeg_decode_sync_workspace_bytes", "vfml_jpeg_decode_rgb_sync",
    "vfml_jpeg_decode_sampled_workspace_bytes", "vfml_jpeg_decode_rgb_sampled",
    "vfml_jpeg_decode_sync_sampled_workspace_bytes", "vfml_jpeg_decode_rgb_sync_sampled",
    "vfml_deflate_capacity", "vfml_deflate_workspace_bytes", "vfml_deflate_huffman",
    "vfml_inflate_workspace_bytes", "vfml_inflate_chunks",
    "vfml_last_error", "vfml_abi_version",
]


def _check(rc, what):
    if rc != 0:
        raise RuntimeError(f"{what} failed (rc={rc}): {lib().vfml_last_error().decode()}")


def _stream():
    return c_void_p(torch.cuda.current_stream().cuda_stream)


def _ptr(t, offset=0):
    if t is None:
        return None
    return c_void_p(t.data_ptr() + 4 * offset)


def _dev(t, dtype=torch.float32):
    if not (t.is_cuda and t.dtype == dtype and t.is_contiguous()):
        raise ValueError(f"expected a contiguous {dtype} device tensor, got {t.dtype} {t.device} "
                         f"contiguous={t.is_contiguous()}")
    return t


_PROFILE = None


_PROFILE_HBM = None


def profile_begin():
    global _PROFILE, _PROFILE_HBM
    _PROFILE = []
    _PROFILE_HBM = []


def profile_end_hbm():
    rec = _PROFILE_HBM or []
    torch.cuda.synchronize()
    out = {}
    for name, nbytes, e0, e1 in rec:
        d = out.setdefault(name, {"launches": 0, "bytes": 0.0, "ms": 0.0})
        d["launches"] += 1
        d["bytes"] += nbytes
        d["ms"] += e0.elapsed_time(e1)
    return out


def profile_end():
    global _PROFILE, _PROFILE_HBM
    rec, _PROFILE = _PROFILE or [], None
    _PROFILE_HBM = None
    torch.cuda.synchronize()
    out = {}
    for variant, flops, nbytes, e0, e1, shape in rec:
        d = out.setdefault(variant, {"launches": 0, "flops": 0.0, "bytes": 0.0, "ms": 0.0, "shapes": {}})
        ms = e0.elapsed_time(e1)
        for t in (d, d["shapes"].setdefault(shape, {"launches": 0, "flops": 0.0, "bytes": 0.0, "ms": 0.0})):
            t["launches"] += 1
            t["flops"] += flops
            t["bytes"] += nbytes
            t["ms"] += ms
    return out


class SplitWeight:

    def __init__(self, rows, k, device):
        self.rows, self.k, self.kp = rows, k, (k + 31) // 32 * 32
# ... 209 lines not shown

ATT_BANK_MAX = 9


def attention_bank_planes(q, keys, p, planes, score_scale=None, d=128, ld_q=None, ld_k=None, q_off=0, k_offs=None,
                          workspace=None):
    n = len(keys)
    if len(planes) != n or not all(isinstance(a, PlainWeight) for a in planes):
        raise ValueError("attention_bank_planes: one PlainWeight per key set")
    if n and any(a.kp != planes[0].kp or a.scale != planes[0].scale or a.rows < p for a in planes):
        raise ValueError("attention_bank_planes: planes of one row stride and one scale, at least p rows each")
    dev = planes[0].hi.device if n else q.device
    if workspace is None:
        workspace = torch.empty(max(1, attention_plane_workspace_bytes(p) // 4), dtype=torch.float32, device=dev)
    if workspace.dtype != torch.float32 or workspace.numel() * 4 < attention_plane_workspace_bytes(p):
        raise ValueError("attention_bank_planes: workspace of 2 p floats")
    k_offs = k_offs or [0] * n
    kptr = (c_void_p * max(1, n))(*[_dev(k).data_ptr() + 4 * o for k, o in zip(keys, k_offs)])
    pptr = (c_void_p * max(1, n))(*[a.hi.data_ptr() for a in planes])
    _check(lib().vfml_attention_bank_planes_f16(_ptr(_dev(q), q_off), ld_q or d, kptr, ld_k or d, n, p, d,
                                                float(score_scale if score_scale is not None else 1.0 / d ** 0.5),
                                                planes[0].scale if n else 1.0, pptr, planes[0].kp if n else 0,
                                                c_void_p(workspace.data_ptr()), _stream()),
           "vfml_attention_bank_planes_f16")


def axpy_f32(x, y, n, scale=1.0, x_off=0, y_off=0):
    _check(lib().vfml_axpy_f32(_ptr(_dev(x), x_off), _ptr(_dev(y), y_off), n, float(scale), _stream()), "vfml_axpy_f32")


DW_RESIDUAL, DW_GELU = 1, 2


def dwconv2d(x, ld_x, n, h, w, c, k, weight, bias, out, ld_out, x_off=0, out_off=0, in_fmt=FMT_F32, out_fmt=FMT_F32,
             residual=False, gelu=False):
    _check(lib().vfml_dwconv2d(_ptr(_dev(x), x_off), ld_x, n, h, w, c, k, _ptr(_dev(weight)), _ptr(_dev(bias)),
                               _ptr(_dev(out), out_off), ld_out, in_fmt, out_fmt,
                               (DW_RESIDUAL if residual else 0) | (DW_GELU if gelu else 0), _stream()), "vfml_dwconv2d")


def gelu_rows(x, ld_x, out, ld_out, rows, c, x_off=0, out_off=0, in_fmt=FMT_F32, out_fmt=FMT_F32):
    _check(lib().vfml_gelu_rows(_ptr(_dev(x), x_off), ld_x, _ptr(_dev(out), out_off), ld_out, rows, c, in_fmt, out_fmt,
                                _stream()), "vfml_gelu_rows")


def layernorm_rows(x, ld_x, out, ld_out, rows, c, gamma, beta, eps=1e-5, x_off=0, out_off=0, in_fmt=FMT_F32, out_fmt=FMT_F32):
    _check(lib().vfml_layernorm_rows(_ptr(_dev(x), x_off), ld_x, _ptr(_dev(out), out_off), ld_out, rows, c, _ptr(_dev(gamma)),
                                     _ptr(_dev(beta)), float(eps), in_fmt, out_fmt, _stream()), "vfml_layernorm_rows")


def window_attention(qkv, ld, n, h, w, c, heads, ws, pad_row, out, ld_out, qkv_off=0, out_off=0, in_fmt=FMT_F32, out_fmt=FMT_F32):
    _check(lib().vfml_window_attention(_ptr(_dev(qkv), qkv_off), ld, n, h, w, c, heads, ws, _ptr(_dev(pad_row)),
                                       _ptr(_dev(out), out_off), ld_out, in_fmt, out_fmt, _stream()), "vfml_window_attention")


def attention_shared_keys(q, ld_q, kv, ld_kv, n, p, pk, c, heads, out, ld_out, q_off=0, kv_off=0, out_off=0, q_fmt=FMT_F32,
                          kv_fmt=FMT_F32, out_fmt=FMT_F32):
    _check(lib().vfml_attention_shared_keys(_ptr(_dev(q), q_off), ld_q, _ptr(_dev(kv), kv_off), ld_kv, n, p, pk, c, heads,
                                            _ptr(_dev(out), out_off), ld_out, q_fmt, kv_fmt, out_fmt, _stream()),
           "vfml_attention_shared_keys")


def transpose_to_s16(src, rows, c, ld, dst, ld_dst, scale=1.0, src_off=0, dst_off=0):
    _check(lib().vfml_transpose_to_s16(_ptr(_dev(src), src_off), rows, c, ld, float(scale), _ptr(_dev(dst), dst_off), ld_dst,
                                       _stream()), "vfml_transpose_to_s16")


def add_to_s16(x, ldx, aux, ld_aux, out, ld_out, rows, c, scale=1.0, x_off=0, aux_off=0, out_off=0):
    _check(lib().vfml_add_to_s16(_ptr(_dev(x), x_off), ldx, _ptr(_dev(aux), aux_off), ld_aux, _ptr(_dev(out), out_off), ld_out,
                                 rows, c, float(scale), _stream()), "vfml_add_to_s16")


def to_s16(src, rows, c, ld_src, dst, ld_dst, src_off=0, dst_off=0, scale=1.0):
    _check(lib().vfml_to_s16(_ptr(_dev(src), src_off), rows, c, ld_src, _ptr(_dev(dst), dst_off), ld_dst, float(scale),
                             _stream()), "vfml_to_s16")


def ptr_table_set(table, tensors):
    n = len(tensors)
    if not (table.is_cuda and table.dtype == torch.int64 and table.numel() >= n):
        raise ValueError("ptr_table_set: table must be an int64 device tensor with room for the pointers")
    ptrs = (c_void_p * n)(*[t if isinstance(t, int) else t.data_ptr() for t in tensors])
    _check(lib().vfml_ptr_table_set(c_void_p(table.data_ptr()), ptrs, n, _stream()), "vfml_ptr_table_set")


SEED_NONE, SEED_LOAD, SEED_STORE = 0, 1, 2


def window_seed(cells, ncentres, rows, cols, state, ld_state, h_off, mf_off, ld_ctx):
    if not (cells.is_cuda and cells.dtype == torch.int64 and cells.numel() >= 3 * ncentres):
        raise ValueError("window_seed: cells must be an int64 device tensor, three per centre frame")
    _check(lib().vfml_window_seed(c_void_p(cells.data_ptr()), ncentres, rows, cols, _ptr(_dev(state)), ld_state, h_off, mf_off,
                                  ld_ctx, _stream()), "vfml_window_seed")


def corr_lookup(pyrs, hl, wl, ld, radius, q_per_map, coords, coords_off, ld_coords, out, out_off, ld_out,
                out_fmt=FMT_F32, table=None, nmaps=None, vol_fmt=FMT_F32, vol_tile=0, bidir=None):
    L = len(hl)
    if bidir is not None:
        dir_coords, dir_out, dir_tab = bidir

        def launch():
            _check(lib().vfml_corr_lookup_indirect_bidir(c_void_p(table.data_ptr()), (c_int32 * L)(*hl), (c_int32 * L)(*wl),
                                                         (c_int32 * L)(*ld), L, radius, nmaps, q_per_map,
                                                         _ptr(_dev(coords), coords_off), ld_coords, dir_coords,
                                                         _ptr(_dev(out), out_off), ld_out, dir_out, dir_tab, out_fmt, vol_fmt,
                                                         vol_tile, _stream()), "vfml_corr_lookup_indirect_bidir")
    elif table is not None:
        def launch():
            _check(lib().vfml_corr_lookup_indirect(c_void_p(table.data_ptr()), (c_int32 * L)(*hl), (c_int32 * L)(*wl),
                                                   (c_int32 * L)(*ld), L, radius, nmaps, q_per_map,
                                                   _ptr(_dev(coords), coords_off), ld_coords, _ptr(_dev(out), out_off),
                                                   ld_out, out_fmt, vol_fmt, vol_tile, _stream()), "vfml_corr_lookup_indirect")
    else:
        if pyrs and torch.is_tensor(pyrs[0]):
            pyrs = [pyrs]
        nmaps, L = len(pyrs), len(pyrs[0])
        ptrs = (c_void_p * (nmaps * L))(*[p.data_ptr() for m in pyrs for p in m])

        def launch():
            _check(lib().vfml_corr_lookup(ptrs, (c_int32 * L)(*hl), (c_int32 * L)(*wl), (c_int32 * L)(*ld), L, radius,
                                          nmaps, q_per_map, _ptr(_dev(coords), coords_off), ld_coords,
                                          _ptr(_dev(out), out_off), ld_out, out_fmt, vol_fmt, vol_tile, _stream()), "vfml_corr_lookup")
    if _PROFILE_HBM is None:
        launch()
        return
    e0, e1 = torch.cuda.Event(enable_timing=True), torch.cuda.Event(enable_timing=True)
    e0.record()
    launch()
    e1.record()
    q = (2 if bidir is not None else 1) * nmaps * q_per_map
    m16 = _vol_mask(vol_fmt, L)
    texel_bytes = sum(2.0 if (m16 >> l) & 1 else 4.0 for l in range(L))
    _PROFILE_HBM.append(("corr_lookup", q * ((2 * radius + 2) ** 2 * texel_bytes + L * (2 * radius + 1) ** 2 * 4.0), e0, e1))


class VolTile:

    def __init__(self, tws, ths):
        self.tws, self.ths = tws, ths
        self.code = tws + 16 * ths
        self._pos = {}

    def count(self, h, w):
        return ((((h - 1) >> self.ths) + 1) * (((w - 1) >> self.tws) + 1)) << (self.tws + self.ths)

    def position(self, h, w, dev):
        key = (h, w, str(dev))
        if key not in self._pos:
            y = torch.arange(h, device=dev, dtype=torch.int64).view(h, 1)
            x = torch.arange(w, device=dev, dtype=torch.int64).view(1, w)
            tpr = ((w - 1) >> self.tws) + 1
            pos = ((((y >> self.ths) * tpr + (x >> self.tws)) << (self.tws + self.ths))
                   + ((y & ((1 << self.ths) - 1)) << self.tws) + (x & ((1 << self.tws) - 1)))
            self._pos[key] = pos.reshape(-1).contiguous()
        return self._pos[key]

    def rows(self, x, h, w, c):
        n = self.count(h, w)
        out = torch.zeros(n, c, device=x.device, dtype=x.dtype)
        out.index_copy_(0, self.position(h, w, x.device), x.view(h * w, c))
        return out.view(-1)


def coords_init(coords1, n, h, w):
    _check(lib().vfml_coords_init(_ptr(_dev(coords1)), n, h, w, _stream()), "vfml_coords_init")
# ... 659 lines not shown
```

video-flow-ml_amd/vfml/network.py:

```python
import os
import types

import torch
import torch.nn as nn

from . import hip, update_block
from .weights import (BASE_CORR_LEVELS, BASE_CORR_RADIUS, GMA_NO_BIAS, TWINS_STAGES, TWINS_WS, conv_spec, corr_channel_subset,
                      is_depthwise, pack_conv_weight, pcblock_hidden, sk_blocks, twins_spec)

ATT_SCALE = 16384.0


def cor_pad(cor, split):
    return (cor + 15) // 16 * 16 if split else (cor + 3) // 4 * 4


def take_frames(src, idx):
    idx = list(idx)
    if all(b == a + 1 for a, b in zip(idx, idx[1:])):
        return src[idx[0]:idx[0] + len(idx)]
    return torch.stack([src[i] for i in idx])


class _Holder(nn.Module):
# ... 670 lines not shown

        def stats_of(t, hw, c, slot):
            s = st[slot * n * 128 * 2:]
            hip.instnorm_stats(t, n, hw, c, s, ws)
            return s

        split_prec = self._split()
        AF = hip.FMT_S16 if split_prec else hip.FMT_F32
        part_len = n * ((h2 * w2 + 31) // 32) * 64 * 2
        parts = self._buf("enc_part", 3 * part_len, dev, torch.float64) if split_prec else None
        fold_ws = self._buf("enc_foldws", min(n, 8) * 64 * 128 * 2, dev, torch.float64) if split_prec else None

        def conv_stats(src, c, hh_, ww_, name, planes, dst, slot, k, stride=1, pad=0, src_fmt=hip.FMT_F32):
            wgt, b = P[name]
            nm = self._nm(name) if split_prec else 3
            ho_, wo_ = (hh_ + 2 * pad - k) // stride + 1, (ww_ + 2 * pad - k) // stride + 1
            hw = ho_ * wo_
            rows = hip.STATS_ROWS_S16 if src_fmt == hip.FMT_S16 else hip.STATS_ROWS_F32
            if not (split_prec and (n == 1 or hw % rows == 0)):
                hip.conv2d(src, c, c, n, hh_, ww_, wgt, b, planes, k, k, dst, planes, stride=stride, pad_h=pad, pad_w=pad,
                           mfma=nm, in_fmt=src_fmt)
                return stats_of(dst, hw, planes, slot)
            chunks = (hw + rows - 1) // rows
            part = parts[slot * part_len:]
            if (c == 64 and planes == 64 and k == 3 and stride == 1 and pad == 1 and nm == 3 and src_fmt == hip.FMT_S16
                    and ww_ % 32 == 0 and getattr(wgt, "order", None) == hip.KORDER_CBLOCK and wgt.kp == 576 and wgt.lo is not None):
                hip.conv3x3_c64(src, c, n, hh_, ww_, wgt, b, dst, planes, stats_part=part)
            else:
                hip.conv2d(src, c, c, n, hh_, ww_, wgt, b, planes, k, k, dst, planes, stride=stride, pad_h=pad, pad_w=pad,
                           stats_part=part, mfma=nm, in_fmt=src_fmt)
            s = st[slot * n * 128 * 2:]
            hip.instnorm_finalize(part, n, chunks, planes, hw, s, workspace=fold_ws)
            return s

        stem = P.get(f"{prefix}.conv1.stem")
        if stem is not None and split_prec and self._nm(f"{prefix}.conv1") == 3:
            chunks = hip.stem_chunks(H, W)
            part = parts[0:]
            hip.stem7x7s2(x, n, H, W, stem[0], stem[1], raw, stats_part=part)
            s0 = st[0:]
            hip.instnorm_finalize(part, n, chunks, 64, h2 * w2, s0, workspace=fold_ws)
        else:
            s0 = conv_stats(x, 4, H, W, f"{prefix}.conv1", 64, raw, 0, 7, stride=2, pad=3)
        cur = act[0]
        hip.instnorm_apply(raw, s0, n, h2 * w2, 64, cur, out_fmt=AF)
        ch, hh, ww, ci = 64, h2, w2, 0
        for li, (planes, stride) in enumerate([(64, 1), (96, 2), (128, 2)], start=1):
            for bi in range(2):
                stv = stride if bi == 0 else 1
                ho, wo = (hh, ww) if stv == 1 else ((hh - 1) // 2 + 1, (ww - 1) // 2 + 1)
                name = f"{prefix}.layer{li}.{bi}"
                y = act[(ci + 1) % 3]
                nxt = act[(ci + 2) % 3]
                s1 = conv_stats(cur, ch, hh, ww, f"{name}.conv1", planes, raw, 0, 3, stride=stv, pad=1, src_fmt=AF)
                hip.instnorm_apply(raw, s1, n, ho * wo, planes, y, out_fmt=AF)
                s2 = conv_stats(y, planes, ho, wo, f"{name}.conv2", planes, raw, 1, 3, pad=1, src_fmt=AF)
                if stv != 1:
                    s3 = conv_stats(cur, ch, hh, ww, f"{name}.downsample.0", planes, raw2, 2, 1, stride=stv, src_fmt=AF)
                    hip.instnorm_apply(raw, s2, n, ho * wo, planes, nxt, res=raw2, res_stats=s3, out_fmt=AF)
                else:
                    hip.instnorm_apply(raw, s2, n, ho * wo, planes, nxt, res=cur, out_fmt=AF)
                cur, ci = nxt, (ci + 2) % 3
                ch, hh, ww = planes, ho, wo
        wgt, b = P[f"{prefix}.conv2"]
        hip.conv2d(cur, 128, 128, n, hh, ww, wgt, b, 256, 1, 1, out, ldo, out_off=out_off, epilogue=epilogue,
                   split=split, out_fmt=out_fmt, in_fmt=AF, mfma=self._nm(f"{prefix}.conv2") if split_prec else 3)
        return hh, ww

    @torch.no_grad()
    def forward(self, images, data=None, return_lowres=True):
        if not isinstance(images, torch.Tensor) or not images.is_cuda:
            raise RuntimeError("MOFNetHIP runs on an MI355X (HIP) device only; got "
                               f"{getattr(images, 'device', type(images))}. There is no CPU fallback in the shipped engine.")
        if images.dim() != 5 or images.shape[2] != 3:
            raise ValueError(f"images must be [B,N,3,H,W], got {tuple(images.shape)}")
        if images.shape[0] != 1:
            raise ValueError(f"Batch size must be 1, got {images.shape[0]}")
        src = images[0]
        if src.dtype != torch.float32:
            src = src.float()
        return self._run(src.contiguous(), src.shape[0], src.shape[2], src.shape[3], return_lowres)

    @torch.no_grad()
    def forward_u8(self, frames, return_lowres=True, frame_keys=None, tri_batch=False, pick_only=False):
        if not (isinstance(frames, torch.Tensor) and frames.is_cuda and frames.dtype == torch.uint8
                and frames.dim() == 4 and frames.shape[3] == 3):
            raise ValueError("forward_u8 expects a uint8 [N,H,W,3] device tensor")
        if frame_keys is not None and len(frame_keys) != frames.shape[0]:
            raise ValueError("frame_keys must have one entry per frame")
        if tri_batch and not self.tri_frame:
            raise ValueError("tri_batch applies to tri-frame (BOF) networks")
        return self._run(frames.contiguous(), frames.shape[0], frames.shape[1], frames.shape[2], return_lowres,
                         frame_keys, tri_batch, pick_only and not return_lowres)

    FEATURE_CACHE_FRAMES = 12
    FMAP_ROW_SCALE = 16.0

    def clear_feature_cache(self):
        self._join_prefetch()
        self._feat_cache.clear()
        self._pyr_free = []

    def prefetch_frames(self, frames, frame_keys):
        if (frame_keys is None or self._pre_body is None or os.environ.get("VFML_PREFETCH", "1") == "0" or self.tri_frame):
            return
        cfg = self.cfg
        N, H, W = frames.shape[0], frames.shape[1], frames.shape[2]
        if N < 3 or H % 8 or W % 8 or len(frame_keys) != N:
            return
        L, dev = cfg.corr_levels, frames.device
        h, w = H // 8, W // 8
        AF = hip.FMT_S16 if self._split() else hip.FMT_F32
        geo = self._volume_geometry(H, W, L, AF)
        hl, wl, Sl = geo.hl, geo.wl, geo.Sl
        keys = [(k, H, W, L, self._plan_key(), self._packed_serial) for k in frame_keys]
        need_f = [j for j in range(N) if ("f", keys[j]) not in self._feat_cache]
        need_c = [j for j in range(1, N - 1) if ("c", keys[j]) not in self._feat_cache]
        if not need_f and not need_c:
            return
        main = torch.cuda.current_stream(dev)
        side = self._side.get(dev)
        if side is None:
            side = self._side[dev] = torch.cuda.Stream(device=dev)
        P = self._pack(dev)
        if "serial" in os.environ.get("VFML_PREFETCH_DBG", ""):
            side.wait_stream(main)
        else:
            side.wait_event(self._pre_body)
        frames.record_stream(side)
        with torch.cuda.stream(side):
            new = []
            if need_f:
                new += list(self._frame_features(frames, need_f, keys, H, W, P, dev, L, hl, wl, Sl, vt=geo.VT).values())
            if need_c:
                new += list(self._frame_context(frames, need_c, keys, H, W, P, dev, h * w, N - 2).values())
            done = torch.cuda.Event()
            done.record(side)

        def walk(x):
            if isinstance(x, torch.Tensor):
                x.record_stream(main)
            elif isinstance(x, (list, tuple)):
                for y in x:
                    walk(y)
            elif isinstance(x, dict):
                for y in x.values():
                    walk(y)
            elif hasattr(x, "planes") and isinstance(getattr(x, "planes"), torch.Tensor):
                x.planes.record_stream(main)
        walk(new)
        self._prefetch_done, self._prefetch_dev = done, dev

    def _pyramid_buffers(self, sizes, dev, limit):
        while sum(1 for k in self._feat_cache if k[0] == "p") >= limit:
            oldest = next(k for k in self._feat_cache if k[0] == "p")
            self._pyr_free.append(self._feat_cache.pop(oldest))
        for i, bufs in enumerate(self._pyr_free):
            if [b.numel() for b in bufs] == sizes and bufs[0].device == dev:
                return self._pyr_free.pop(i)
        del self._pyr_free[:]
        return [torch.empty(n, device=dev) for n in sizes]

    def _cache_get(self, kind, key):
        ent = self._feat_cache.get((kind, key))
        if ent is not None:
            self._feat_cache.move_to_end((kind, key))
        return ent

    def _cache_put(self, kind, key, value, limit=None):
        self._feat_cache[(kind, key)] = value
        while sum(1 for k in self._feat_cache if k[0] == kind) > (limit or self.FEATURE_CACHE_FRAMES):
            oldest = next(k for k in self._feat_cache if k[0] == kind)
            del self._feat_cache[oldest]

    def _volume_geometry(self, H, W, L, AF):
        cfg = self.cfg
        h, w = H // 8, W // 8
        hl, wl = [h], [w]
        for l in range(1, L):
            hl.append(hl[-1] // 2)
            wl.append(wl[-1] // 2)
        Sl = [hl[l] * wl[l] for l in range(L)]
        VT = self._tile()
        Nl = [VT.count(hl[l], wl[l]) for l in range(L)] if VT is not None else Sl
        Pv = Nl[0]
        TILE = VT.code if VT is not None else 0
        mask = self.CORR_VOLUMES[getattr(cfg, "corr_volume", "f32")] & ((1 << L) - 1)
        if not (mask and AF == hip.FMT_S16 and Pv % 4 == 0 and all(s % 4 == 0 for s in Nl) and L <= 4
                and cfg.corr_radius in (3, 4)):
            mask = 0
        v16 = [bool((mask >> l) & 1) for l in range(L)]
        VFl = [hip.FMT_F16 if v16[l] else hip.FMT_F32 for l in range(L)]
        VF = (hip.FMT_F32 if not mask else hip.FMT_F16 if mask == (1 << L) - 1 else hip.vol_f16_levels(mask))
        ldl = []
        for l in range(L):
            unit = 64 if v16[l] else 32
            n = (Nl[l] + unit - 1) // unit * unit
            ldl.append(n if (n // unit) % 2 else n + unit)
        psz = [(Pv * ldl[l] + 1) // 2 if v16[l] else Pv * ldl[l] for l in range(L)]
        return types.SimpleNamespace(L=L, AF=AF, hl=hl, wl=wl, Sl=Sl, VT=VT, Nl=Nl, Pv=Pv, TILE=TILE, vol16=mask, VF=VF,
                                     VFl=VFl, ldl=ldl, psz=psz)

    def _window_pyramids(self, feats, keys, N, geo, dev):
        D, L = self.cfg.feat_dim, geo.L
        AF, VFl, Nl, Pv, ldl, psz = geo.AF, geo.VFl, geo.Nl, geo.Pv, geo.ldl, geo.psz
        scale = 1.0 / float(D) ** 0.5
        if AF == hip.FMT_S16:
            scale /= self.FMAP_ROW_SCALE
        lim = 2 * (N - 2) + 2
        pyrs = {"f": [], "b": []}
        for c in range(1, N - 1):
            for d, tgt in (("f", c + 1), ("b", c - 1)):
                pk = ("p", keys[c], keys[tgt]) if keys is not None else None
                if pk is not None and self.gma and d == "b" and keys[c] == keys[tgt]:
                    pk += ("b",)
                pyr = self._cache_get("p", pk) if pk is not None else None
                if pyr is None:
                    if pk is None:
                        pyr = [self._buf(f"pyr_{d}{c}_{l}", psz[l], dev) for l in range(L)]
                    else:
                        pyr = self._pyramid_buffers(psz, dev, limit=lim)
                        self._cache_put("p", pk, pyr, limit=lim)
                    rk = ("p", keys[tgt], keys[c]) if pk is not None else None
                    gemm_form = AF == hip.FMT_S16 and Pv % 4 == 0 and Nl[0] >= 1024
                    dual = rk is not None and d == "f" and gemm_form and ("p", rk) not in self._feat_cache
                    rev = None
                    if dual:
                        rev = self._pyramid_buffers(psz, dev, limit=lim)
                        self._cache_put("p", rk, rev, limit=lim)
                    cnm = self._nm("corr") if self._split() else 3
                    for l in range(L):
                        hip.conv2d(feats[c][0], D, D, 1, 1, Pv, feats[tgt][1][l], None, Nl[l], 1, 1, pyr[l],
                                   ldl[l], out_scale=scale, in_fmt=AF, out_fmt=VFl[l],
                                   swap_cross=(d == "b" and l == 0 and gemm_form and cnm == 3),
                                   out_t=rev[0] if dual and l == 0 else None, ld_out_t=ldl[0] if dual and l == 0 else 0,
                                   mfma=cnm)
                    if dual:
                        for l in range(1, L):
                            hip.conv2d(feats[tgt][0], D, D, 1, 1, Pv, feats[c][1][l], None, Nl[l], 1, 1, rev[l],
                                       ldl[l], out_scale=scale, in_fmt=AF, out_fmt=VFl[l], mfma=cnm)
                pyrs[d].append(pyr)
        return pyrs

    def _frame_features(self, src, sel, keys, H, W, P, dev, L, hl, wl, Sl, vt=None):
        D = self.cfg.feat_dim
        split = self._split()
        out, todo = {}, []
        for j in sel:
            ent = self._cache_get("f", keys[j]) if keys is not None else None
            if ent is not None:
                out[j] = ent
            else:
                todo.append(j)
        if todo:
            m, Pn = len(todo), hl[0] * wl[0]
            frames = self._buf("frames", m * H * W * 4, dev)
            hip.frames_to_nhwc4(take_frames(src, todo).contiguous(), m, H, W, float(self.cfg.input_scale), float(self.cfg.input_shift),
                                frames)
            fmap = torch.empty(m * Pn * D, device=dev)
            (self._twins_encoder if self.twins else self._encoder)("fnet", frames, m, H, W, P, dev, fmap, D, 0, hip.EPI_NONE, 0)
            levels = [fmap]
            for l in range(1, L):
                t = torch.empty(m * Sl[l] * D, device=dev)
                hip.avgpool2x2(levels[-1], m, hl[l - 1], wl[l - 1], D, t)
                levels.append(t)
            for i, j in enumerate(todo):
                tg = []
                for l in range(L):
                    f = levels[l][i * Sl[l] * D:(i + 1) * Sl[l] * D]
                    nl = Sl[l]
                    if vt is not None:
                        f, nl = vt.rows(f, hl[l], wl[l], D), vt.count(hl[l], wl[l])
                    tg.append(hip.SplitWeight(nl, D, dev).fill(f, scale=16.0) if split else f)
                fm = fmap[i * Pn * D:(i + 1) * Pn * D]
                if vt is not None:
                    fm, Pn_rows = vt.rows(fm, hl[0], wl[0], D), vt.count(hl[0], wl[0])
                else:
                    Pn_rows = Pn
                if split:
                    fm16 = torch.empty(Pn_rows * D, device=dev)
                    hip.to_s16(fm, Pn_rows, D, D, fm16, D, scale=self.FMAP_ROW_SCALE)
                    fm = fm16
                ent = (fm, tg)
                out[j] = ent
                if keys is not None:
                    self._cache_put("f", keys[j], ent)
        return out

    def _frame_context(self, src, sel, keys, H, W, P, dev, Pn, M=1):
        out, todo = {}, []
        st = self._context_store(dev, Pn, max(M, len(sel)))
        att = self._attention_store(dev, Pn, max(M, len(sel))) if self.gma else None
        for j in sel:
            ent = self._cache_get("c", keys[j]) if keys is not None else None
            if ent is not None and ent[3] == st["serial"] and (att is None or ent[5] == att["serial"]):
                out[j] = ent
            else:
                todo.append(j)
        if todo:
            m = len(todo)
            frames = self._buf("frames", m * H * W * 4, dev)
            hip.frames_to_nhwc4(take_frames(src, todo).contiguous(), m, H, W,
                                float(self.cfg.input_scale), float(self.cfg.input_shift), frames)
            ctx = torch.empty(m * Pn * 256, device=dev)
            AF = hip.FMT_S16 if self._split() else hip.FMT_F32
            (self._twins_encoder if self.twins else self._encoder)("cnet", frames, m, H, W, P, dev, ctx, 256, 0, hip.EPI_TANH_RELU,
                                                                   self.hidden_dim, out_fmt=AF)
            h8, w8 = H // 8, W // 8
            R, Mst = st["R"], st["M"]
            for i, j in enumerate(todo):
                cx = ctx[i * Pn * 256:(i + 1) * Pn * 256]
                busy = {e[2] for e in out.values()}
                slot = self._context_slot(st, ("c", keys[j]) if keys is not None else None, busy)
                add = {}
                for k, (kh, kw) in () if self.sk else (("1", (1, 5)), ("2", (5, 1))):
                    for g, co in (("zr", 256), ("q", 128)):
                        wgt, b = P[f"update_block.gru.conv{g}{k}.ctx"]
                        S = st["S"][g + k]
                        hip.conv2d(cx, 128, 256, 1, h8, w8, wgt, b, co, kh, kw, S, co, in0_off=128, out_off=slot * Pn * co,
                                   pad_h=kh // 2, pad_w=kw // 2, in_fmt=AF,
                                   mfma=self._nm(f"update_block.gru.conv{g}{k}.ctx") if self._split() else 3)
                        add[g + k] = S[slot * Pn * co:(slot + 1) * Pn * co]
                        if slot < Mst - 1:
                            S[(R + slot) * Pn * co:(R + slot + 1) * Pn * co].copy_(add[g + k])
                ent = (cx, add, slot, st["serial"])
                if att is not None:
                    aslot = self._attention_slot(att, ("c", keys[j]) if keys is not None else None,
                                                 {e[4] for e in out.values()})
                    self._build_attention(att, aslot, cx, h8, w8, Pn, P, dev, AF)
                    ent += (aslot, att["serial"])
                out[j] = ent
                if keys is not None:
                    self._cache_put("c", keys[j], out[j])
        return out

    def _state_columns(self):
        GLD, cols = 768, dict(Z=0, RH=128, HH=256, INP=384, MF=512, MT=640, MG=None, XC=256)
        if self.gma:
            GLD = 896
            cols.update(MG=768, XC=384)
        if self.sk:
            GLD = 640 if self.gma else 512
            cols.update(HH=0, INP=128, MF=256, MT=384, MG=512)
        return GLD, cols

    def _window_state(self, P, dev, M, h, w, geo, R, AF, cor_p):
        MP = M * h * w
        GLD, cols = self._state_columns()
        if self.gma and self._att_store is not None:
            self._att_store["live"] = set()

        def rows(name, c):
            return self._buf(name, MP * c, dev)
        return update_block.window_state(
            P, self._nm if self._split() else (lambda layer: 3),
            AF, h, w, geo, R, rows("gru_state", GLD), GLD, cols, 2 * cor_p, cor_p, self._rows7, self._tapsum,
            corr=self._buf("corr", MP * 2 * cor_p, dev, zero=True),
            c1=rows("c1", 256), cf=rows("cf", 256), f1=rows("f1", 128), fh=rows("fh", 256), flow4=rows("flow4", 4),
            delta=rows("delta", 4), fh_taps=rows("fh_taps", 2 * 36),
            frows=rows("flow_rows7", 32), coords1=rows("coords1", 4))

    def _seed_plan(self, s, ctx, keys, dev, M, R, pick_only):
        cfg, it0 = self.cfg, None
        if (self.iter0_store and not self.sk and keys is not None and self._split() and not self.tri_frame and M >= 2
                and cfg.decoder_depth >= 1 and not (pick_only and cfg.decoder_depth + 1 < M)):
            it0 = self._iter0_store(dev, s.Pn, M)
            warm, seeds, it0_new = it0["ring"].plan(keys, tail=(R,))
            self.iter0_stats["warm" if warm else "cold"] += 1
            self.iter0_last = (warm, [slot for slot, _ in seeds])
        else:
            warm, seeds, it0_new = False, [(None, hip.SEED_NONE)] * M, []
        seed_cells = self._buf("seed_cells", 64, dev, torch.int64)
        hip.ptr_table_set(seed_cells, [v for i, (slot, mode) in enumerate(seeds) for v in
                                       (ctx[i + 1][0], it0["S"][slot * s.Pn * 128:] if slot is not None else 0, mode)])
        return it0, warm, it0_new, seed_cells

    def _gate_addends(self, ctx, dev, Pn, M):
        st = self._ctx_store
        RING, Mst = st["R"], st["M"]
        slots = [ctx[c][2] for c in range(1, M + 1)]
        st["live"] = set(slots)
        first = slots[0]
        if not self.sk and (not self._split() or os.environ.get("VFML_CTX_GATHER", "0") == "1" or
                            not all(s == first + i or (first + i >= RING and s == first + i - RING and s < Mst - 1)
                                    for i, s in enumerate(slots))):
            first = RING + Mst - 1
            for i, c in enumerate(range(1, M + 1)):
                for name, co in self.CTX_GATES:
                    st["S"][name][(first + i) * Pn * co:(first + i + 1) * Pn * co].copy_(ctx[c][1][name])
        gate_add = {name: st["S"].get(name) for name, _ in self.CTX_GATES}
        gate_off = {name: first * Pn * co for name, co in self.CTX_GATES}
        gate_ind = None
        if self._split() and not self.sk:
            cells = self._buf("gate_add_cells", 8, dev, torch.int64)
            hip.ptr_table_set(cells, [st["S"][name][gate_off[name]:] for name, _ in self.CTX_GATES])
            gate_ind = {name: (cells, i) for i, (name, _) in enumerate(self.CTX_GATES)}
        return gate_add, gate_off, gate_ind

    def _pyramid_tables(self, pyrs, dev, M, L, cor_p):
        if 2 * M <= 8 and 2 * M * L <= 48:
            tab_fb = self._buf("pyr_table_fb", 64, dev, torch.int64)
            hip.ptr_table_set(tab_fb, [p for d in ("f", "b") for m in pyrs[d] for p in m])
            return (tab_fb,), (2, cor_p, M)
        tab_f = self._buf("pyr_table_f", 64, dev, torch.int64)
        tab_b = self._buf("pyr_table_b", 64, dev, torch.int64)
        hip.ptr_table_set(tab_f, [p for m in pyrs["f"] for p in m])
        hip.ptr_table_set(tab_b, [p for m in pyrs["b"] for p in m])
        return (tab_f, tab_b), None

    def _gma_readout(self, s, win, ng):
        att = self._att_store
        update_block.attention_readout(s, "update_block.aggregator.to_v", [att["A"][k] for k in win.att_slots[:ng]],
                                       att["plain"], att["ldA"], att["P8"], self._gamma, ATT_SCALE, s.MF, s.MG, win.readout)

    def _iteration(self, s, win, it, ng, nm, branch):
        ub = update_block
        ne, r0 = (1, (win.M - 1) * s.Pn) if win.warm and it == 0 else (nm, 0)
        join = None
        if branch is not None:
            fork = torch.cuda.Event()
            fork.record()
            with torch.cuda.stream(branch):
                branch.wait_event(fork)
                ub.flow_half(s, ne, r0)
                join = torch.cuda.Event()
                join.record()
        ub.lookup(s, ne, r0, win.tables, win.bidir)
        ub.convc1(s, ne, r0)
        ub.convc2(s, ne, r0)
        if join is None:
            ub.flow_half(s, ne, r0)
        else:
            torch.cuda.current_stream(win.dev).wait_event(join)
        ub.encoder_conv(s, ne, r0)
        if it == 0:
            hip.window_seed(win.seed_cells, win.M, s.Pn, 128, s.G, s.GLD, s.HH, s.MF, 256)
        if self.gma:
            self._gma_readout(s, win, ng)
        update_block.temporal_fusion(s, win.M if self.tri_frame else nm, stack=not self.tri_frame)
        ub.sep_conv_gru(s, ng, *win.gates)
        ub.flow_head(s, ng)

    def _sk_iteration(self, s, win, ng, nm):
        ub, P, h, w, G, GLD, ws = "update_block", s.P, s.h, s.w, s.G, s.GLD, win.sk_ws
        blk = self._pcblock
        update_block.lookup(s, nm, 0, win.tables, win.bidir)
        blk(f"{ub}.encoder.convc1", P, s.corr, s.ld_corr, 0, nm, h, w, s.c1, 256, 0, ws, gelu_out=True)
        blk(f"{ub}.encoder.convc2", P, s.c1, 256, 0, nm, h, w, s.cf, 256, 0, ws)
        wgt, b = P[f"{ub}.encoder.convf1"]
        hip.conv2d(s.flow4, 4, 4, nm, h, w, wgt, b, 128, 1, 1, s.f1, 128, out_fmt=s.AF, mfma=s.nm(f"{ub}.encoder.convf1"))
        blk(f"{ub}.encoder.convf2", P, s.f1, 128, 0, nm, h, w, s.cf, 256, 192, ws)
        blk(f"{ub}.encoder.conv", P, s.cf, 256, 0, nm, h, w, G, GLD, s.MF, ws)
        if self.gma:
            self._gma_readout(s, win, ng)
        update_block.temporal_fusion(s, win.M if self.tri_frame else nm, stack=not self.tri_frame)
        blk(f"{ub}.gru", P, G, GLD, 0, ng, h, w, G, GLD, s.HH, ws)
        blk(f"{ub}.flow_head", P, G, GLD, s.HH, ng, h, w, s.delta, 4, 0, ws, out_fmt=hip.FMT_F32)
        update_block.update_coords(s, ng)

    def _run(self, src, N, H, W, return_lowres, frame_keys=None, tri_batch=False, pick_only=False):
        cfg = self.cfg
        if N < 3:
            raise ValueError(f"need at least 3 frames, got {N}")
        if self.tri_frame and N > 3 and not tri_batch:
            lo = N // 2 - 1
            src = src[lo:lo + 3].contiguous()
            frame_keys = frame_keys[lo:lo + 3] if frame_keys is not None else None
            N = 3
        if H % 8 or W % 8:
            raise ValueError("H and W must be multiples of 8 (use InputPadder)")
        L, R = cfg.corr_levels, cfg.corr_radius
        h, w = H // 8, W // 8
        if (h >> (L - 1)) < 2 or (w >> (L - 1)) < 2:
            raise ValueError(f"frame {H}x{W} too small for a {L}-level correlation pyramid")
        dev = src.device
        self._join_prefetch()
        M = N - 2
        Pn = h * w
        if self.gma and Pn > 32768:
            raise ValueError(f"frame {H}x{W}: the GMA aggregator attends over all {Pn} cells of a frame and is built for at "
                             f"most 32768; process larger frames in tiles (--tile)")
        MP = M * Pn
        P = self._pack(dev)
        AF = hip.FMT_S16 if self._split() else hip.FMT_F32
        cor_p = cor_pad(L * (2 * R + 1) ** 2, AF == hip.FMT_S16)
        short = pick_only and not self.tri_frame

        with torch.cuda.device(dev):
            geo = self._volume_geometry(H, W, L, AF)
            keys = None
            if frame_keys is not None:
                keys = [(k, H, W, L, self._plan_key(), self._packed_serial) for k in frame_keys]

            feats = self._frame_features(src, list(range(N)), keys, H, W, P, dev, L, geo.hl, geo.wl, geo.Sl, vt=geo.VT)
            pyrs = self._window_pyramids(feats, keys, N, geo, dev)
            s = self._window_state(P, dev, M, h, w, geo, R, AF, cor_p)
            ctx = self._frame_context(src, list(range(1, N - 1)), keys, H, W, P, dev, Pn, M)
            win = types.SimpleNamespace(M=M, dev=dev, att_slots=(), readout=None)
            if self.gma:
                att = self._att_store
                win.att_slots = tuple(ctx[c][4] for c in range(1, N - 1))
                att["live"] = set(win.att_slots)
                win.readout = update_block.readout_scratch(self._buf, dev, MP, Pn, self.ATT_DIM, att["ldA"], att["plain"],
                                                           att["vt"])
            it0, win.warm, it0_new, win.seed_cells = self._seed_plan(s, ctx, keys, dev, M, R, pick_only)
            win.gates = self._gate_addends(ctx, dev, Pn, M)
            win.sk_ws = self._sk_workspace(MP, dev) if self.sk else None
            win.tables, win.bidir = self._pyramid_tables(pyrs, dev, M, L, cor_p)
            no, nflows = (1, 1) if short else (M, 2 * M)
            up_fixed = self._buf("up_out", nflows * H * W * 2, dev)
            mask = self._buf("mask", MP * 1152, dev)

            def body():
                update_block.init_coords(s, M)
                branch = None
                if os.environ.get("VFML_FLOW_BRANCH", "0") == "1" and self._split():
                    branch = self._side2.get(dev)
                    if branch is None:
                        branch = self._side2[dev] = torch.cuda.Stream(device=dev)
                if self.sk:
                    hip.window_seed(win.seed_cells, M, Pn, 256, s.G, s.GLD, s.HH, s.MF, 256)
                for it in range(cfg.decoder_depth):
                    left = cfg.decoder_depth - 1 - it
                    ng = min(M, left + 1) if short else M
                    nm = min(M, left + 2) if short else M
                    if self.sk:
                        self._sk_iteration(s, win, ng, nm)
                    else:
                        self._iteration(s, win, it, ng, nm, branch)
                if cfg.decoder_depth == 0 and not self.sk:
                    hip.window_seed(win.seed_cells, M, Pn, 128, s.G, s.GLD, s.HH, s.MF, 256)
                update_block.mask_head(s, no, mask, 1152)
                if short:
                    hip.convex_upsample(s.coords1, 0, 2, mask, 576, 1152, h, w, up_fixed)
                else:
                    for d in range(2):
                        for c in range(M):
                            hip.convex_upsample(s.coords1, c * Pn * 4, 2 * d, mask, c * Pn * 1152 + d * 576, 1152, h, w,
                                                up_fixed, out_off=(d * M + c) * H * W * 2)

            gkey = (H, W, N, M, bool(tri_batch), bool(pick_only), cfg.decoder_depth, L, R, self._plan_key(), geo.vol16,
                    self._packed_serial, str(dev), os.environ.get("VFML_FLOW_BRANCH", "0"), win.warm, win.att_slots)
            if self.sk:
                gkey += ("sk",)
            self._pre_body = torch.cuda.Event()
            self._pre_body.record(torch.cuda.current_stream(dev))
            try:
                self._run_body(body, gkey, dev)
            except BaseException:
                if it0_new:
                    it0["ring"].forget(it0_new)
                raise
            up = up_fixed.clone().view(nflows, H, W, 2)
            flow = up.permute(0, 3, 1, 2).unsqueeze(0)
            if short:
                return flow, None
            low = s.flow4.view(M, h, w, 4)[..., :].clone() if return_lowres else None
        return flow, low


def build_network(cfg):
    return MOFNetHIP(cfg)
```

video-flow-ml_amd/vfml/update_block.py:

```python
import types

from . import hip

UB = "update_block"


def window_state(P, nm, AF, h, w, geo, R, G, GLD, cols, ld_corr, cor_p, rows7, tapsum, **maps):
    return types.SimpleNamespace(P=P, nm=nm, AF=AF, h=h, w=w, Pn=h * w, geo=geo, R=R, G=G, GLD=GLD, ld_corr=ld_corr, cor_p=cor_p,
                                 rows7=rows7, tapsum=tapsum,
                                 fuse=AF == hip.FMT_S16,
                                 **cols, **maps)


def _put_flow(s):
    return dict(flow_a=s.flow4, ld_a=4, flow_b=s.G, ld_b=s.GLD, flow_b_off=s.MF + 124, fmt_b=s.AF)


def init_coords(s, n, flow_init=None):
    hip.coords_init(s.coords1, n, s.h, s.w)
    hip.coords_update(s.coords1, flow_init, n, s.h, s.w, **_put_flow(s))


def lookup(s, n, r0, tables=(), bidir=None, pyrs=None):
    g = s.geo
    if pyrs is not None:
        hip.corr_lookup(pyrs, g.hl, g.wl, g.ldl, s.R, s.Pn, s.coords1, r0 * 4, 4, s.corr, r0 * s.ld_corr, s.ld_corr,
                        out_fmt=s.AF, vol_fmt=g.VF, vol_tile=g.TILE)
        return
    t0 = r0 // s.Pn * g.L
    for d, tab in enumerate(tables):
        hip.corr_lookup(None, g.hl, g.wl, g.ldl, s.R, s.Pn, s.coords1, r0 * 4 + 2 * d, 4, s.corr, r0 * s.ld_corr + d * s.cor_p,
                        s.ld_corr, out_fmt=s.AF, table=tab[t0:], nmaps=n, vol_fmt=g.VF, vol_tile=g.TILE, bidir=bidir)


def convc1(s, n, r0):
    wgt, b = s.P[f"{UB}.encoder.convc1"]
    hip.conv2d(s.corr, s.ld_corr, s.ld_corr, n, s.h, s.w, wgt, b, 256, 1, 1, s.c1, 256, epilogue=hip.EPI_RELU,
               in0_off=r0 * s.ld_corr, out_off=r0 * 256, in_fmt=s.AF, out_fmt=s.AF, mfma=s.nm(f"{UB}.encoder.convc1"))


def convc2(s, n, r0):
    wgt, b = s.P[f"{UB}.encoder.convc2"]
    hip.conv2d(s.c1, 256, 256, n, s.h, s.w, wgt, b, 192, 3, 3, s.cf, 256, in0_off=r0 * 256, out_off=r0 * 256,
               pad_h=1, pad_w=1, epilogue=hip.EPI_RELU, in_fmt=s.AF, out_fmt=s.AF, mfma=s.nm(f"{UB}.encoder.convc2"))


def flow_half(s, n, r0):
    nm1, nm2 = s.nm(f"{UB}.encoder.convf1"), s.nm(f"{UB}.encoder.convf2")
    wgt, b = s.P[f"{UB}.encoder.convf1"]
    wgt2, b2 = s.P[f"{UB}.encoder.convf2"]
    if (s.fuse and s.rows7 and nm1 == 1 and nm2 == 1
            and getattr(wgt2, "order", None) == hip.KORDER_CBLOCK64 and wgt.kp == 224 and wgt2.kp == 1152):
        hip.flow_half(s.flow4[r0 * 4:], n, s.h, s.w, wgt, b, wgt2, b2, s.cf, 256, out_off=r0 * 256 + 192)
        return
    if s.rows7:
        hip.flow_rows7(s.flow4[r0 * 4:], n, s.h, s.w, s.frows[r0 * 32:])
        hip.conv2d(s.frows, 32, 32, n, s.h, s.w, wgt, b, 128, 7, 1, s.f1, 128, pad_h=3, epilogue=hip.EPI_RELU,
                   in0_off=r0 * 32, out_off=r0 * 128, in_fmt=s.AF, out_fmt=s.AF, mfma=nm1)
    else:
        hip.conv2d(s.flow4, 4, 4, n, s.h, s.w, wgt, b, 128, 7, 7, s.f1, 128, pad_h=3, pad_w=3, epilogue=hip.EPI_RELU,
                   in0_off=r0 * 4, out_off=r0 * 128, out_fmt=s.AF, mfma=nm1)
    hip.conv2d(s.f1, 128, 128, n, s.h, s.w, wgt2, b2, 64, 3, 3, s.cf, 256, in0_off=r0 * 128, out_off=r0 * 256 + 192,
               pad_h=1, pad_w=1, epilogue=hip.EPI_RELU, in_fmt=s.AF, out_fmt=s.AF, mfma=nm2)


def encoder_conv(s, n, r0):
    wgt, b = s.P[f"{UB}.encoder.conv"]
    hip.conv2d(s.cf, 256, 256, n, s.h, s.w, wgt, b, 124, 3, 3, s.G, s.GLD, in0_off=r0 * 256, out_off=r0 * s.GLD + s.MF,
               pad_h=1, pad_w=1, epilogue=hip.EPI_RELU, in_fmt=s.AF, out_fmt=s.AF, mfma=s.nm(f"{UB}.encoder.conv"))


def readout_scratch(buf, dev, rows, Pn, AD, ldA, plain, vt=None):
    ro = types.SimpleNamespace(AD=AD, vt=vt, val=buf("att_v", rows * AD, dev))
    if plain:
        ro.vrows = buf("att_vt", AD * ldA, dev)
        ro.out = buf("att_ro", AD * ldA, dev)
        ro.out_t = buf("att_ro_t", Pn * AD, dev)
        ro.ws = buf("att_ro_ws", AD * ldA + Pn * AD, dev)
    return ro


def plane_readout(s, a, ldA, ro, val, val_off=0):
    hip.transpose_to_s16(val, s.Pn, ro.AD, ro.AD, ro.vrows, ldA, scale=16.0, src_off=val_off)
    hip.conv2d(ro.vrows, ldA, ldA, ro.AD, 1, 1, a, None, s.Pn, 1, 1, ro.out, ldA, out_scale=1.0 / 16.0,
               in_fmt=s.AF, out_t=ro.out_t, ld_out_t=ro.AD, mfma=1, ksplit_ws=ro.ws)


def attention_readout(s, layer, planes, plain, ldA, P8, gamma, att_scale, src, dst, ro, addend=None):
    if addend is not None and not (plain and len(planes) == 1):
        raise ValueError("attention_readout: an addend needs the plane form and a single frame")
    n, Pn, AD, G, GLD, AF = len(planes), s.Pn, ro.AD, s.G, s.GLD, s.AF
    wgt, b = s.P[layer]
    hip.conv2d(G, 128, GLD, n, s.h, s.w, wgt, b, AD, 1, 1, ro.val, AD, in0_off=src, in_fmt=AF, mfma=s.nm(layer))
    for k, a in enumerate(planes):
        if plain:
            plane_readout(s, a, ldA, ro, ro.val, k * Pn * AD)
            if addend is not None:
                hip.axpy_f32(addend, ro.out_t, Pn * AD)
            hip.add_to_s16(ro.out_t, AD, G, GLD, G, GLD, Pn, AD, scale=gamma, aux_off=k * Pn * GLD + src,
                           out_off=k * Pn * GLD + dst)
        else:
            vt = ro.vt.fill_transposed(ro.val, Pn, ld=AD, scale=16.0, src_off=k * Pn * AD)
            hip.conv2d(a, P8, ldA, Pn, 1, 1, vt, None, AD, 1, 1, G, GLD, out_off=k * Pn * GLD + dst,
                       out_scale=gamma / att_scale, epilogue=hip.EPI_ADD_AUX, aux0=G, ld_aux0=GLD,
                       aux0_off=k * Pn * GLD + src, in_fmt=AF, out_fmt=AF, aux_fmt=AF,
                       mfma=s.nm(layer.rsplit(".", 1)[0] + ".readout"))


def temporal_fusion(s, n, stack):
    wgt, b = s.P[f"{UB}.tprop"]
    nb, nh = (1, n) if stack else (n, 1)
    hip.conv2d(s.G, 128, s.GLD, nb, nh, s.Pn, wgt, b, 128, 3, 1, s.G, s.GLD, in0_off=s.MF, out_off=s.MT, pad_h=1,
               epilogue=hip.EPI_RELU, in_fmt=s.AF, out_fmt=s.AF, mfma=s.nm(f"{UB}.tprop"))


# ... 52 lines not shown
```

Baseline: 46.58.

## Compute level-0 correlation volume on demand around lookup windows

Stops computing the full level-0 all-pairs correlation GEMM up front and adds an ensure kernel that runs before each lookup. The kernel computes only the correlation tiles that the current coordinates' windows touch, and tracks which tiles are done in a per-pyramid bitmap. The resident-A GEMM walk moves into a shared header so the new kernel can reuse it. The aim is to skip level-0 tiles that are never sampled, at the cost of per-iteration ensure launches, bitmap bookkeeping and possible recomputation overhead; dense_corr disables the path for tiled crops.

```diff
diff --git a/include/vfml.h b/include/vfml.h
--- a/include/vfml.h
+++ b/include/vfml.h
@@ -131,6 +131,11 @@
                                     int vol_tile, void* stream);
 int vfml_ptr_table_set(void* table, const void* const* ptrs, int n, void* stream);
 
+int vfml_corr_level0_ensure(const vfml_conv_desc* d, const void* w_hi, const void* w_lo, int kp, float w_scale, int in_fmt,
+                            int out_fmt, int k_order, const void* const* cells, int centres, int dirs, int dir_cells,
+                            const float* coords, int ld_coords, int dir_coords, int h, int w, int radius, int vol_tile,
+                            uint32_t* counter, void* stream);
+
 #define VFML_SEED_NONE 0
 #define VFML_SEED_LOAD 1
 #define VFML_SEED_STORE 2
diff --git a/video-flow-ml_amd/processing/videoflow_processor.py b/video-flow-ml_amd/processing/videoflow_processor.py
--- a/video-flow-ml_amd/processing/videoflow_processor.py
+++ b/video-flow-ml_amd/processing/videoflow_processor.py
@@ -78,7 +78,7 @@
         if not self.core.is_model_loaded():
             raise RuntimeError("Model not loaded. Call load_model() first.")
 
-    def _flow_from_host_u8(self, frames, frame_idx):
+    def _flow_from_host_u8(self, frames, frame_idx, tile_crop=False):
         model = self.core.model
         if not (str(self.device).startswith('cuda') and hasattr(model, "forward_u8")):
             return None
@@ -102,7 +102,8 @@
                 while len(self._dev_frames) > HOST_FRAME_CACHE:
                     self._dev_frames.popitem(last=False)
         win = torch.stack([self._dev_frames[keys[i]] for i in ids])
-        flows, _ = model.forward_u8(win, return_lowres=False, frame_keys=[keys[i] for i in ids], pick_only=self.PICK_ONLY)
+        flows, _ = model.forward_u8(win, return_lowres=False, frame_keys=[keys[i] for i in ids], pick_only=self.PICK_ONLY,
+                                    dense_corr=tile_crop)
         return flows[0, flows.shape[1] // 2].permute(1, 2, 0).cpu().numpy()
 
     def compute_optical_flow(self, frames, frame_idx):
@@ -113,7 +114,7 @@
         flow = self.core.compute_flow_from_tensor(self.prepare_frame_sequence(frames, frame_idx))
         return flow.permute(1, 2, 0).cpu().numpy()
 
-    def compute_optical_flow_with_progress(self, frames, frame_idx, tile_pbar=None):
+    def compute_optical_flow_with_progress(self, frames, frame_idx, tile_pbar=None, tile_crop=False):
         self._require_model()
 
         def step(desc, n=0, reset=False):
@@ -125,7 +126,7 @@
                     tile_pbar.update(n)
 
         step("Preparing frames", reset=True)
-        fast = self._flow_from_host_u8(frames, frame_idx)
+        fast = self._flow_from_host_u8(frames, frame_idx, tile_crop)
         if fast is not None:
             step("Completed", 4)
             return fast
@@ -148,7 +149,7 @@
                 overall_pbar.set_description(f"Tile {k + 1}/{len(tiles)} ({t['width']}x{t['height']})")
             crops = [self.extract_tile(f, t) for f in frames]
             full[t['y']:t['y'] + t['height'], t['x']:t['x'] + t['width']] = \
-                self.compute_optical_flow_with_progress(crops, frame_idx, tile_pbar)
+                self.compute_optical_flow_with_progress(crops, frame_idx, tile_pbar, tile_crop=True)
             if overall_pbar is not None:
                 overall_pbar.update(1)
         return full
@@ -179,7 +180,8 @@
         if H % 8 == 0 and W % 8 == 0 and hasattr(model, "forward_u8"):
             tok = clip_token(clip)
             keys = [(tok, i, rect) for i in frame_ids]
-            flows, _ = model.forward_u8(win, return_lowres=False, frame_keys=keys, pick_only=self.PICK_ONLY)
+            flows, _ = model.forward_u8(win, return_lowres=False, frame_keys=keys, pick_only=self.PICK_ONLY,
+                                        dense_corr=tile is not None)
             if ((tile is None or getattr(self, "tiles_in_frame_order", False)) and frame_idx + 1 < clip.shape[0]
                     and hasattr(model, "prefetch_frames")):
                 nxt = self.window_indices(clip.shape[0], frame_idx + 1)
diff --git a/video-flow-ml_amd/vfml/csrc/conv_gemm_split.hip b/video-flow-ml_amd/vfml/csrc/conv_gemm_split.hip
--- a/video-flow-ml_amd/vfml/csrc/conv_gemm_split.hip
+++ b/video-flow-ml_amd/vfml/csrc/conv_gemm_split.hip
@@ -1,4 +1,5 @@
 #include "conv_split_common.h"
+#include "gemm_resident_walk.h"
 
 namespace {
 
@@ -261,189 +262,6 @@
 }
 
 
-
-template <bool H16, bool BIAS>
-__device__ __forceinline__ void gemm_resident_walk(const SplitArgs& a, char* smem) {
-  constexpr int NW = 4;
-  constexpr int RBM = 128, RBN = 64;
-  constexpr int NSTEP = VFML_RESIDENT_KMAX / 64;
-  constexpr int ASTEP = RBM * 128, BSTEP = RBN * 128;
-  constexpr int BOFF = 0, BBUF = NSTEP * BSTEP, SLAB = BOFF + 2 * BBUF;
-  constexpr int AP = RBM / (8 * NW), BP = RBN / (8 * NW);
-  constexpr int ES = H16 ? 2 : 4;
-  constexpr int NSTORE = 8, NSTORE_T = 16;
-  constexpr int STORE_NT = 2;
-  static_assert(NSTEP * ASTEP == 2 * BBUF, "the A image of a unit fills the two B buffers");
-  static_assert(SLAB + NW * 32 * 32 * 4 == VFML_RESIDENT_LDS, "LDS budget of the resident-A walk: two workgroups per CU");
-
-  const int t = threadIdx.x;
-  const int lane = t & 63;
-  const int wave = __builtin_amdgcn_readfirstlane(t >> 6);
-  const int lrow = 8 * wave + (lane >> 3);
-  const int piece = (lane & 7) ^ ((4 * wave + (lane >> 4)) & 7);
-  const int nk = (a.Kp / 64 + 1) & ~1;
-  const __amdgpu_buffer_rsrc_t rb = __builtin_amdgcn_make_buffer_rsrc(const_cast<char*>(a.wbase), 0, a.bytesb, 0x00020000);
-  const int r = lane & 31, half = lane >> 5;
-  const int q16 = (((r >> 1) & 7) ^ half) * 16;
-  const int aoff = (wave * 32 + r) * 128 + q16;
-  const int boff = r * 128 + q16;
-  float* ws = reinterpret_cast<float*>(smem + SLAB) + wave * (32 * 32);
-  const int c4 = (lane % 8) * 4, rr = lane / 8;
-
-  const int units = a.mtiles * a.res_nc;
-  for (int u = blockIdx.x; u < units; u += gridDim.x) {
-    const int run = u / a.mtiles, mt = u - run * a.mtiles;
-    const int nt0 = run * a.res_cl;
-    const int nt1 = nt0 + a.res_cl < a.ntiles ? nt0 + a.res_cl : a.ntiles;
-    const int m0 = mt * RBM;
-    const int rows_valid = a.M - m0 < RBM ? a.M - m0 : RBM;
-    __amdgpu_buffer_rsrc_t r0;
-    if (a.tilebase)
-      r0 = __builtin_amdgcn_make_buffer_rsrc(const_cast<float*>(a.in0) + (int64_t)m0 * a.ld0, 0,
-                                             ((rows_valid - 1) * a.ld0 + a.d0off + a.c0) * 4, 0x00020000);
-    else
-      r0 = __builtin_amdgcn_make_buffer_rsrc(const_cast<float*>(a.in0), 0, a.bytes0, 0x00020000);
-    int va[AP];
-#pragma unroll
-    for (int j = 0; j < AP; ++j) {
-      const int m = m0 + 8 * NW * j + lrow;
-      const int mrow = a.tilebase ? m - m0 : m;
-      va[j] = m < a.M ? (mrow * a.ld0 + a.d0off) * 4 + piece * 32 : OOB;
-    }
-    auto issue_b = [&](int nt, int buf) {
-      int colbase[BP];
-#pragma unroll
-      for (int j = 0; j < BP; ++j) {
-        const int col = nt * RBN + 8 * NW * j + lrow;
-        colbase[j] = col < a.cout ? a.whi_off + col * a.Kp * 2 + piece * 16 : (a.bhi ? 0x7ffffff0 : 0x40000000);
-      }
-      for (int s = 0; s < nk; ++s)
-#pragma unroll
-        for (int j = 0; j < BP; ++j)
-          dma16(rb, colbase[j], s * 128, smem + BOFF + buf * BBUF + s * BSTEP + wave * (8 * 128) + j * (8 * NW * 128));
-    };
-
-    h16x8 af[4 * NSTEP];
-#pragma unroll
-    for (int q = 0; q < 4 * NSTEP; ++q) af[q] = h16x8{0, 0, 0, 0, 0, 0, 0, 0};
-    lds_barrier();
-    for (int s = 0; s < nk; ++s) {
-      const bool past = s * 64 >= a.ctot;
-#pragma unroll
-      for (int j = 0; j < AP; ++j)
-        dma16(r0, past ? OOB : va[j], s * 256, smem + s * ASTEP + wave * (8 * 128) + j * (8 * NW * 128));
-    }
-    asm volatile("s_waitcnt vmcnt(0)" ::: "memory");
-    lds_barrier();
-    static_for<NSTEP>([&](auto sc) {
-      constexpr int s = decltype(sc)::value;
-      if (s < nk) {
-#pragma unroll
-        for (int ks = 0; ks < 4; ++ks) af[s * 4 + ks] = *reinterpret_cast<const h16x8*>(smem + s * ASTEP + (aoff ^ (ks * 32)));
-      }
-    });
-    lds_barrier();
-    issue_b(nt0, 0);
-
-    for (int nt = nt0; nt < nt1; ++nt) {
-      const int buf = (nt - nt0) & 1;
-      const int n0 = nt * RBN;
-      if (nt == nt0) asm volatile("s_waitcnt vmcnt(0)" ::: "memory");
-      else if (a.out_t) asm volatile("s_waitcnt vmcnt(%0)" ::"n"(NSTORE_T) : "memory");
-      else asm volatile("s_waitcnt vmcnt(%0)" ::"n"(NSTORE) : "memory");
-      lds_barrier();
-      f32x4 bv[2] = {{0.f, 0.f, 0.f, 0.f}, {0.f, 0.f, 0.f, 0.f}};
-      if constexpr (BIAS) {
-#pragma unroll
-        for (int j = 0; j < 2; ++j)
-          if (n0 + j * 32 + c4 < a.cout) bv[j] = *reinterpret_cast<const f32x4*>(a.bias + n0 + j * 32 + c4);
-      }
-      if (nt + 1 < nt1) issue_b(nt + 1, buf ^ 1);
-
-      f32x16 acc[2];
-#pragma unroll
-      for (int j = 0; j < 2; ++j)
-#pragma unroll
-        for (int e = 0; e < 16; ++e) acc[j][e] = 0.f;
-      const char* bb = smem + BOFF + buf * BBUF;
-      static_for<NSTEP / 2>([&](auto pc) {
-        constexpr int s0 = 2 * decltype(pc)::value;
-        if (s0 < nk) {
-          h16x8 b0[8], b1[8];
-#pragma unroll
-          for (int q = 0; q < 8; ++q) {
-            b0[q] = *reinterpret_cast<const h16x8*>(bb + (s0 + (q >> 2)) * BSTEP + (boff ^ ((q & 3) * 32)));
-            b1[q] = *reinterpret_cast<const h16x8*>(bb + (s0 + (q >> 2)) * BSTEP + (boff ^ ((q & 3) * 32)) + 4096);
-          }
-#pragma unroll
-          for (int q = 0; q < 8; ++q) {
-            acc[0] = __builtin_amdgcn_mfma_f32_32x32x16_f16(af[s0 * 4 + q], b0[q], acc[0], 0, 0, 0);
-            acc[1] = __builtin_amdgcn_mfma_f32_32x32x16_f16(af[s0 * 4 + q], b1[q], acc[1], 0, 0, 0);
-          }
-        }
-      });
-
-      const int cols_valid = a.cout - n0 < RBN ? a.cout - n0 : RBN;
-      char* tbase = reinterpret_cast<char*>(a.out) + ((int64_t)m0 * a.ldo + n0) * ES;
-      const __amdgpu_buffer_rsrc_t ro =
-          __builtin_amdgcn_make_buffer_rsrc(tbase, 0, ((rows_valid - 1) * a.ldo + cols_valid) * ES, 0x00020000);
-      const int rows_t = cols_valid, cols_t = rows_valid;
-      __amdgpu_buffer_rsrc_t rt = ro;
-      if (a.out_t) {
-        char* tbase_t = reinterpret_cast<char*>(a.out_t) + ((int64_t)n0 * a.ld_out_t + m0) * ES;
-        rt = __builtin_amdgcn_make_buffer_rsrc(tbase_t, 0, ((rows_t - 1) * a.ld_out_t + cols_t) * ES, 0x00020000);
-      }
-      static_for<2>([&](auto jc) {
-        constexpr int j = decltype(jc)::value;
-        const int gcol = j * 32 + c4;
-#pragma unroll
-        for (int e = 0; e < 16; ++e) ws[((e & 3) + 8 * (e >> 2) + 4 * half) * 32 + r] = acc[j][e];
-#pragma unroll
-        for (int p = 0; p < 4; ++p) {
-          f32x4 v = *reinterpret_cast<const f32x4*>(ws + (p * 8 + rr) * 32 + c4);
-#pragma unroll
-          for (int e = 0; e < 4; ++e) {
-            v[e] = (v[e] * a.w_inv + bv[j][e]) * a.out_scale;
-            if (a.epilogue == VFML_EPI_RELU) v[e] = fmaxf(v[e], 0.f);
-          }
-          const int off = gcol < cols_valid ? ((wave * 32 + p * 8 + rr) * a.ldo + gcol) * ES : OOB;
-          if constexpr (H16) {
-            const h16x2 p0 = {(_Float16)v[0], (_Float16)v[1]}, p1 = {(_Float16)v[2], (_Float16)v[3]};
-            const u32x2 hv = {__builtin_bit_cast(unsigned, p0), __builtin_bit_cast(unsigned, p1)};
-            __builtin_amdgcn_raw_buffer_store_b64(hv, ro, off, 0, STORE_NT);
-          } else {
-            __builtin_amdgcn_raw_buffer_store_b128(__builtin_bit_cast(u32x4, v), ro, off, 0, STORE_NT);
-          }
-        }
-        if (a.out_t) {
-#pragma unroll
-          for (int e = 0; e < 16; ++e) {
-            const int row = (e & 3) + 8 * (e >> 2) + 4 * half;
-            ws[r * 32 + ((row + (r >> 1)) & 31)] = acc[j][e];
-          }
-          const int g = lane >> 3, cl = lane & 7;
-#pragma unroll
-          for (int pp = 0; pp < 4; ++pp) {
-            const int c = pp * 8 + cl;
-            f32x4 v;
-#pragma unroll
-            for (int k = 0; k < 4; ++k) v[k] = ws[c * 32 + ((4 * g + k + (c >> 1)) & 31)] * a.w_inv * a.out_scale;
-            const int trow = j * 32 + c;
-            const int q0 = wave * 32 + 4 * g;
-            const bool ok = trow < rows_t && q0 < cols_t;
-            if constexpr (H16) {
-              const h16x2 p0 = {(_Float16)v[0], (_Float16)v[1]}, p1 = {(_Float16)v[2], (_Float16)v[3]};
-              const u32x2 hv = {__builtin_bit_cast(unsigned, p0), __builtin_bit_cast(unsigned, p1)};
-              __builtin_amdgcn_raw_buffer_store_b64(hv, rt, ok ? (trow * a.ld_out_t + q0) * 2 : OOB, 0, STORE_NT);
-            } else {
-              __builtin_amdgcn_raw_buffer_store_b128(__builtin_bit_cast(u32x4, v), rt, ok ? (trow * a.ld_out_t + q0) * 4 : OOB, 0, STORE_NT);
-            }
-          }
-        }
-      });
-    }
-  }
-}
 
 template <int TM, int TN, int WM, int WN, bool PERSIST, bool FASTK, bool CSWAP = false, int NM = 3, bool MF16 = false, bool H16 = false>
 __global__ __launch_bounds__(WM * WN * 64, (WM * WN == 4 ? 2 : 1)) void conv_gemm_dma_kernel(const SplitArgs a) {
@@ -1640,6 +1458,19 @@
   return 0;
 }
 
+int vfml_detail::prepare_resident_gemm(const vfml_conv_desc* d, const void* w_hi, const void* w_lo, int kp, float w_scale,
+                                       int in_fmt, int out_fmt, int k_order, const char* who, SplitArgs* a) {
+  SplitPlan plan;
+  const SplitVariant* row;
+  if (const int rc = split_prepare(d, w_hi, w_lo, kp, w_scale, in_fmt, out_fmt, VFML_FMT_F32, k_order, 0, *a, plan, row)) return rc;
+  VFML_REQUIRE(plan.family == vfml_detail::SPLIT_DMA && plan.persist && plan.resident && plan.nm == 5 && !plan.h16 && !plan.add_rows,
+               "%s: the level-0 call must be one the library runs on the resident-A walk of its GEMM form (split-row "
+               "features of at most %d channels, one MFMA per product, f32 volume, cout >= 1024)", who, VFML_RESIDENT_KMAX);
+  a->mtiles = (a->M + 127) / 128;
+  a->ntiles = (a->cout + 63) / 64;
+  return 0;
+}
+
 extern "C" int vfml_conv2d_split(const vfml_conv_desc* d, const void* w_hi, const void* w_lo, int kp, float w_scale,
                                  int in_fmt, int out_fmt, int aux_fmt, int k_order, void* stream) {
   SplitArgs a;
diff --git a/video-flow-ml_amd/vfml/csrc/conv_split_common.h b/video-flow-ml_amd/vfml/csrc/conv_split_common.h
--- a/video-flow-ml_amd/vfml/csrc/conv_split_common.h
+++ b/video-flow-ml_amd/vfml/csrc/conv_split_common.h
@@ -74,6 +74,8 @@
 int variant_name(const SplitPlan& key, char* buf, int len);
 const SplitVariant* tapx_variant(const SplitPlan& plan);
 const SplitVariant* tapx_variant_at(int index);
+int prepare_resident_gemm(const vfml_conv_desc* d, const void* w_hi, const void* w_lo, int kp, float w_scale, int in_fmt,
+                          int out_fmt, int k_order, const char* who, SplitArgs* a);
 }
 using vfml_detail::SplitArgs;
 using vfml_detail::SplitPlan;
diff --git a/video-flow-ml_amd/vfml/csrc/corr_ensure.hip b/video-flow-ml_amd/vfml/csrc/corr_ensure.hip
--- /dev/null
+++ b/video-flow-ml_amd/vfml/csrc/corr_ensure.hip
@@ -0,0 +1,145 @@
+#include "gemm_resident_walk.h"
+#include "corr_window.h"
+
+namespace {
+
+constexpr int ENSURE_MASK_WORDS = 64;
+
+struct EnsureArgs {
+  SplitArgs g;
+  const void* const* cells;
+  const float* coords;
+  unsigned* counter;
+  int ld_coords, dir_coords;
+  int centres, dirs, dir_cells;
+  int q_per_map;
+  int h, w, radius, tws, ths;
+  int wpr;
+};
+
+struct MaskCols {
+  unsigned v;
+  int nw;
+  __device__ __forceinline__ unsigned word(int w) const {
+    return (unsigned)__builtin_amdgcn_readlane((int)v, __builtin_amdgcn_readfirstlane(w));
+  }
+  __device__ __forceinline__ int from(int at) const {
+    int w = at >> 5;
+    if (w >= nw) return -1;
+    unsigned m = word(w) & (~0u << (at & 31));
+    while (!m) {
+      if (++w >= nw) return -1;
+      m = word(w);
+    }
+    return w * 32 + __builtin_ctz(m);
+  }
+  __device__ __forceinline__ int first() const { return from(0); }
+  __device__ __forceinline__ int next(int nt) const { return from(nt + 1); }
+};
+
+__device__ __forceinline__ const void* uniform_cell(const void* const* cell) {
+  const uint64_t v = reinterpret_cast<uint64_t>(*cell);
+  const unsigned lo = (unsigned)__builtin_amdgcn_readfirstlane((int)(unsigned)v);
+  const unsigned hi = (unsigned)__builtin_amdgcn_readfirstlane((int)(unsigned)(v >> 32));
+  return reinterpret_cast<const void*>(((uint64_t)hi << 32) | lo);
+}
+
+typedef __attribute__((address_space(1))) unsigned* gu32ptr;
+typedef const __attribute__((address_space(1))) float* gf32cptr;
+
+__global__ __launch_bounds__(256, 2) void corr_ensure_kernel(const EnsureArgs e) {
+  extern __shared__ __attribute__((aligned(16))) char smem[];
+  unsigned* mask = reinterpret_cast<unsigned*>(smem);
+  const int t = threadIdx.x, lane = t & 63;
+  const int mtiles = e.g.mtiles;
+  const int units = e.centres * e.dirs * mtiles;
+  const int tsh = e.tws + e.ths;
+  const int tpr = (e.w + (1 << e.tws) - 1) >> e.tws;
+  const int side = 2 * e.radius + 2;
+  for (int u = blockIdx.x; u < units; u += gridDim.x) {
+    const int k = u / mtiles, mt = u - k * mtiles;
+    const int dir = k / e.centres, c = k - dir * e.centres;
+    const void* const* cell = e.cells + (dir * e.dir_cells + c) * 4;
+    const gu32ptr bitmap = (gu32ptr)uniform_cell(cell + 3) + mt * e.wpr;
+    lds_barrier();
+    if (t < ENSURE_MASK_WORDS) mask[t] = 0u;
+    lds_barrier();
+    if (t < 128) {
+      const int row = mt * 128 + t;
+      const int tile = row >> tsh, in = row & ((1 << tsh) - 1);
+      const int ty = tile / tpr, tx = tile - ty * tpr;
+      const int y = (ty << e.ths) + (in >> e.tws), x = (tx << e.tws) + (in & ((1 << e.tws) - 1));
+      if (row < e.g.M && y < e.h && x < e.w) {
+        const gf32cptr cr = (gf32cptr)e.coords + ((int64_t)c * e.q_per_map + y * e.w + x) * e.ld_coords + dir * e.dir_coords;
+        const int x0 = window_origin(cr[0], e.radius);
+        const int y0 = window_origin(cr[1], e.radius);
+        const int xlo = max(x0, 0), xhi = min(x0 + side - 1, e.w - 1);
+        const int ylo = max(y0, 0), yhi = min(y0 + side - 1, e.h - 1);
+        if (xlo <= xhi && ylo <= yhi) {
+          for (int yy = ylo; yy <= yhi; yy = ((yy >> e.ths) + 1) << e.ths)
+            for (int xx = xlo; xx <= xhi; xx = ((xx >> e.tws) + 1) << e.tws) {
+              const int ct = tiled_at(yy, xx, e.w, e.tws, e.ths) >> 6;
+              atomicOr(&mask[ct >> 5], 1u << (ct & 31));
+            }
+        }
+      }
+    }
+    lds_barrier();
+    if (t < e.wpr) mask[t] &= ~bitmap[t];
+    lds_barrier();
+    const unsigned need = lane < e.wpr ? mask[lane] : 0u;
+    const MaskCols cols{need, e.wpr};
+    int cnt = 0;
+    for (int w = 0; w < e.wpr; ++w) cnt += __builtin_popcount(cols.word(w));
+    if (cnt == 0) continue;
+
+    SplitArgs a = e.g;
+    a.in0 = a.in1 = reinterpret_cast<const float*>(uniform_cell(cell));
+    a.wbase = reinterpret_cast<const char*>(uniform_cell(cell + 1));
+    a.out = reinterpret_cast<float*>(const_cast<void*>(uniform_cell(cell + 2)));
+    gemm_resident_unit<false, false>(a, smem, mt, cols);
+
+    asm volatile("s_waitcnt vmcnt(0)" ::: "memory");
+    lds_barrier();
+    if (t < e.wpr && need) atomicOr((unsigned*)bitmap + t, need);
+    if (t == 0 && e.counter) atomicAdd(e.counter, (unsigned)cnt);
+  }
+}
+
+}
+
+extern "C" int vfml_corr_level0_ensure(const vfml_conv_desc* d, const void* w_hi, const void* w_lo, int kp, float w_scale,
+                                       int in_fmt, int out_fmt, int k_order, const void* const* cells, int centres, int dirs,
+                                       int dir_cells, const float* coords, int ld_coords, int dir_coords, int h, int w,
+                                       int radius, int vol_tile, uint32_t* counter, void* stream) {
+  const char* who = "vfml_corr_level0_ensure";
+  VFML_REQUIRE(d && cells && coords, "%s: null desc / cells / coords", who);
+  EnsureArgs e;
+  if (const int rc = vfml_detail::prepare_resident_gemm(d, w_hi, w_lo, kp, w_scale, in_fmt, out_fmt, k_order, who, &e.g)) return rc;
+  const SplitArgs& a = e.g;
+  VFML_REQUIRE(!a.bias && !a.out_t && a.epilogue == VFML_EPI_NONE && a.whi_off == 0 && a.d0off == 0 && a.tilebase,
+               "%s: the level-0 call has no bias, twin or activation, its hi plane leads its planes and its rows are one "
+               "split-row source", who);
+  e.tws = vol_tile & 15;
+  e.ths = vol_tile >> 4;
+  VFML_REQUIRE(vol_tile >= 0 && e.ths <= 6 && e.tws + e.ths <= 6, "%s: vol_tile: tiles of at most 64 texels", who);
+  VFML_REQUIRE(h > 0 && w > 0 && radius >= 1 && radius <= 4, "%s: empty level image, or radius outside 1..4", who);
+  const int64_t tiled = (int64_t)(((h - 1) >> e.ths) + 1) * (((w - 1) >> e.tws) + 1) << (e.tws + e.ths);
+  VFML_REQUIRE(tiled == a.M && tiled == a.cout, "%s: the call's rows (%d) and columns (%d) must be the %lld positions of the "
+               "tiled %d x %d level image", who, a.M, a.cout, (long long)tiled, h, w);
+  e.wpr = (a.ntiles + 31) / 32;
+  VFML_REQUIRE(e.wpr <= ENSURE_MASK_WORDS, "%s: at most %d column tiles per volume row", who, ENSURE_MASK_WORDS * 32);
+  VFML_REQUIRE(centres >= 1 && (dirs == 1 || dirs == 2) && dir_cells >= (dirs == 2 ? centres : 0) && ld_coords >= 2 &&
+               dir_coords >= 0, "%s: centres >= 1, one or two directions, the second direction's cells behind the first's", who);
+  VFML_REQUIRE((reinterpret_cast<uintptr_t>(cells) & 7u) == 0 && (!counter || (reinterpret_cast<uintptr_t>(counter) & 3u) == 0),
+               "%s: cells are 8-byte aligned, the counter 4-byte", who);
+  e.cells = cells; e.coords = coords; e.counter = counter;
+  e.ld_coords = ld_coords; e.dir_coords = dir_coords;
+  e.centres = centres; e.dirs = dirs; e.dir_cells = dir_cells;
+  e.q_per_map = h * w; e.h = h; e.w = w; e.radius = radius;
+  if (const int rc = vfml_lds_cap(reinterpret_cast<const void*>(&corr_ensure_kernel), VFML_RESIDENT_LDS, who)) return rc;
+  const int64_t units = (int64_t)centres * dirs * a.mtiles;
+  hipLaunchKernelGGL(corr_ensure_kernel, dim3((int)(units > 512 ? 512 : units)), dim3(256), VFML_RESIDENT_LDS,
+                     reinterpret_cast<hipStream_t>(stream), e);
+  return vfml_check_launch(who);
+}
diff --git a/video-flow-ml_amd/vfml/csrc/corr_window.h b/video-flow-ml_amd/vfml/csrc/corr_window.h
--- /dev/null
+++ b/video-flow-ml_amd/vfml/csrc/corr_window.h
@@ -0,0 +1,15 @@
+#pragma once
+#include "vfml_common.h"
+
+namespace {
+
+__device__ __forceinline__ int tiled_at(int y, int x, int w, int tws, int ths) {
+  const int tpr = (w + (1 << tws) - 1) >> tws;
+  return ((((y >> ths) * tpr + (x >> tws)) << (tws + ths)) + ((y & ((1 << ths) - 1)) << tws) + (x & ((1 << tws) - 1)));
+}
+
+__device__ __forceinline__ int window_origin(float c, int radius) {
+  return (int)fminf(fmaxf(floorf(c), -65536.f), 65536.f) - radius;
+}
+
+}
diff --git a/video-flow-ml_amd/vfml/csrc/flow_ops.hip b/video-flow-ml_amd/vfml/csrc/flow_ops.hip
--- a/video-flow-ml_amd/vfml/csrc/flow_ops.hip
+++ b/video-flow-ml_amd/vfml/csrc/flow_ops.hip
@@ -1,5 +1,6 @@
 #include <stdlib.h>
 #include "vfml_common.h"
+#include "corr_window.h"
 
 namespace {
 
@@ -37,10 +38,6 @@
   orow = qd * a.ld_out + (dir ? a.dir_out : 0);
 }
 
-__device__ __forceinline__ int tiled_at(int y, int x, int w, int tws, int ths) {
-  const int tpr = (w + (1 << tws) - 1) >> tws;
-  return ((((y >> ths) * tpr + (x >> tws)) << (tws + ths)) + ((y & ((1 << ths) - 1)) << tws) + (x & ((1 << tws) - 1)));
-}
 
 __device__ __forceinline__ float bilinear4(float nw, float ne, float sw, float se, float wx0, float fx, float wy0, float fy) {
   float v = ne * (fx * wy0);
@@ -76,8 +73,8 @@
       const float inv = 1.0f / (float)(1 << l);
       const float x = cx * inv, y = cy * inv;
       const float fx0 = floorf(x), fy0 = floorf(y);
-      const int x0 = (int)fminf(fmaxf(fx0, -65536.f), 65536.f) - a.radius;
-      const int y0 = (int)fminf(fmaxf(fy0, -65536.f), 65536.f) - a.radius;
+      const int x0 = window_origin(x, a.radius);
+      const int y0 = window_origin(y, a.radius);
       const int xx = x0 + px, yy = y0 + py;
       float v = 0.f;
       if (xx >= 0 && xx < a.wl[l] && yy >= 0 && yy < a.hl[l])
@@ -175,8 +172,8 @@
     const int wl = a.wl[ll], hl = a.hl[ll];
     const float inv = __builtin_bit_cast(float, (127 - l) << 23);
     const float x = cx * inv, y = cy * inv;
-    const int x0 = (int)fminf(fmaxf(floorf(x), -65536.f), 65536.f) - R;
-    const int y0 = (int)fminf(fmaxf(floorf(y), -65536.f), 65536.f) - R;
+    const int x0 = window_origin(x, R);
+    const int y0 = window_origin(y, R);
     auto texel = [&](int px, int py, bool in, float& out, bool& ok) {
       const int xx = x0 + px, yy = y0 + py;
       ok = have && in && xx >= 0 && xx < wl && yy >= 0 && yy < hl;
diff --git a/video-flow-ml_amd/vfml/csrc/gemm_resident_walk.h b/video-flow-ml_amd/vfml/csrc/gemm_resident_walk.h
--- /dev/null
+++ b/video-flow-ml_amd/vfml/csrc/gemm_resident_walk.h
@@ -0,0 +1,203 @@
+#pragma once
+#include "conv_split_common.h"
+
+namespace {
+
+struct ResidentRun {
+  int nt0, nt1;
+  __device__ __forceinline__ int first() const { return nt0 < nt1 ? nt0 : -1; }
+  __device__ __forceinline__ int next(int nt) const { return nt + 1 < nt1 ? nt + 1 : -1; }
+};
+
+template <bool H16, bool BIAS, class Cols>
+__device__ __forceinline__ void gemm_resident_unit(const SplitArgs& a, char* smem, int mt, const Cols& cols) {
+  constexpr int NW = 4;
+  constexpr int RBM = 128, RBN = 64;
+  constexpr int NSTEP = VFML_RESIDENT_KMAX / 64;
+  constexpr int ASTEP = RBM * 128, BSTEP = RBN * 128;
+  constexpr int BOFF = 0, BBUF = NSTEP * BSTEP, SLAB = BOFF + 2 * BBUF;
+  constexpr int AP = RBM / (8 * NW), BP = RBN / (8 * NW);
+  constexpr int ES = H16 ? 2 : 4;
+  constexpr int NSTORE = 8, NSTORE_T = 16;
+  constexpr int STORE_NT = 2;
+  static_assert(NSTEP * ASTEP == 2 * BBUF, "the A image of a unit fills the two B buffers");
+  static_assert(SLAB + NW * 32 * 32 * 4 == VFML_RESIDENT_LDS, "LDS budget of the resident-A walk: two workgroups per CU");
+
+  const int t = threadIdx.x;
+  const int lane = t & 63;
+  const int wave = __builtin_amdgcn_readfirstlane(t >> 6);
+  const int lrow = 8 * wave + (lane >> 3);
+  const int piece = (lane & 7) ^ ((4 * wave + (lane >> 4)) & 7);
+  const int nk = (a.Kp / 64 + 1) & ~1;
+  const __amdgpu_buffer_rsrc_t rb = __builtin_amdgcn_make_buffer_rsrc(const_cast<char*>(a.wbase), 0, a.bytesb, 0x00020000);
+  const int r = lane & 31, half = lane >> 5;
+  const int q16 = (((r >> 1) & 7) ^ half) * 16;
+  const int aoff = (wave * 32 + r) * 128 + q16;
+  const int boff = r * 128 + q16;
+  float* ws = reinterpret_cast<float*>(smem + SLAB) + wave * (32 * 32);
+  const int c4 = (lane % 8) * 4, rr = lane / 8;
+
+  const int m0 = mt * RBM;
+  const int rows_valid = a.M - m0 < RBM ? a.M - m0 : RBM;
+  __amdgpu_buffer_rsrc_t r0;
+  if (a.tilebase)
+    r0 = __builtin_amdgcn_make_buffer_rsrc(const_cast<float*>(a.in0) + (int64_t)m0 * a.ld0, 0,
+                                           ((rows_valid - 1) * a.ld0 + a.d0off + a.c0) * 4, 0x00020000);
+  else
+    r0 = __builtin_amdgcn_make_buffer_rsrc(const_cast<float*>(a.in0), 0, a.bytes0, 0x00020000);
+  int va[AP];
+#pragma unroll
+  for (int j = 0; j < AP; ++j) {
+    const int m = m0 + 8 * NW * j + lrow;
+    const int mrow = a.tilebase ? m - m0 : m;
+    va[j] = m < a.M ? (mrow * a.ld0 + a.d0off) * 4 + piece * 32 : OOB;
+  }
+  auto issue_b = [&](int nt, int buf) {
+    int colbase[BP];
+#pragma unroll
+    for (int j = 0; j < BP; ++j) {
+      const int col = nt * RBN + 8 * NW * j + lrow;
+      colbase[j] = col < a.cout ? a.whi_off + col * a.Kp * 2 + piece * 16 : (a.bhi ? 0x7ffffff0 : 0x40000000);
+    }
+    for (int s = 0; s < nk; ++s)
+#pragma unroll
+      for (int j = 0; j < BP; ++j)
+        dma16(rb, colbase[j], s * 128, smem + BOFF + buf * BBUF + s * BSTEP + wave * (8 * 128) + j * (8 * NW * 128));
+  };
+
+  h16x8 af[4 * NSTEP];
+#pragma unroll
+  for (int q = 0; q < 4 * NSTEP; ++q) af[q] = h16x8{0, 0, 0, 0, 0, 0, 0, 0};
+  lds_barrier();
+  for (int s = 0; s < nk; ++s) {
+    const bool past = s * 64 >= a.ctot;
+#pragma unroll
+    for (int j = 0; j < AP; ++j)
+      dma16(r0, past ? OOB : va[j], s * 256, smem + s * ASTEP + wave * (8 * 128) + j * (8 * NW * 128));
+  }
+  asm volatile("s_waitcnt vmcnt(0)" ::: "memory");
+  lds_barrier();
+  static_for<NSTEP>([&](auto sc) {
+    constexpr int s = decltype(sc)::value;
+    if (s < nk) {
+#pragma unroll
+      for (int ks = 0; ks < 4; ++ks) af[s * 4 + ks] = *reinterpret_cast<const h16x8*>(smem + s * ASTEP + (aoff ^ (ks * 32)));
+    }
+  });
+  lds_barrier();
+  int nt = cols.first();
+  if (nt >= 0) issue_b(nt, 0);
+
+  for (int i = 0; nt >= 0; ++i) {
+    const int buf = i & 1;
+    const int nxt = cols.next(nt);
+    const int n0 = nt * RBN;
+    if (i == 0) asm volatile("s_waitcnt vmcnt(0)" ::: "memory");
+    else if (a.out_t) asm volatile("s_waitcnt vmcnt(%0)" ::"n"(NSTORE_T) : "memory");
+    else asm volatile("s_waitcnt vmcnt(%0)" ::"n"(NSTORE) : "memory");
+    lds_barrier();
+    f32x4 bv[2] = {{0.f, 0.f, 0.f, 0.f}, {0.f, 0.f, 0.f, 0.f}};
+    if constexpr (BIAS) {
+#pragma unroll
+      for (int j = 0; j < 2; ++j)
+        if (n0 + j * 32 + c4 < a.cout) bv[j] = *reinterpret_cast<const f32x4*>(a.bias + n0 + j * 32 + c4);
+    }
+    if (nxt >= 0) issue_b(nxt, buf ^ 1);
+
+    f32x16 acc[2];
+#pragma unroll
+    for (int j = 0; j < 2; ++j)
+#pragma unroll
+      for (int e = 0; e < 16; ++e) acc[j][e] = 0.f;
+    const char* bb = smem + BOFF + buf * BBUF;
+    static_for<NSTEP / 2>([&](auto pc) {
+      constexpr int s0 = 2 * decltype(pc)::value;
+      if (s0 < nk) {
+        h16x8 b0[8], b1[8];
+#pragma unroll
+        for (int q = 0; q < 8; ++q) {
+          b0[q] = *reinterpret_cast<const h16x8*>(bb + (s0 + (q >> 2)) * BSTEP + (boff ^ ((q & 3) * 32)));
+          b1[q] = *reinterpret_cast<const h16x8*>(bb + (s0 + (q >> 2)) * BSTEP + (boff ^ ((q & 3) * 32)) + 4096);
+        }
+#pragma unroll
+        for (int q = 0; q < 8; ++q) {
+          acc[0] = __builtin_amdgcn_mfma_f32_32x32x16_f16(af[s0 * 4 + q], b0[q], acc[0], 0, 0, 0);
+          acc[1] = __builtin_amdgcn_mfma_f32_32x32x16_f16(af[s0 * 4 + q], b1[q], acc[1], 0, 0, 0);
+        }
+      }
+    });
+
+    const int cols_valid = a.cout - n0 < RBN ? a.cout - n0 : RBN;
+    char* tbase = reinterpret_cast<char*>(a.out) + ((int64_t)m0 * a.ldo + n0) * ES;
+    const __amdgpu_buffer_rsrc_t ro =
+        __builtin_amdgcn_make_buffer_rsrc(tbase, 0, ((rows_valid - 1) * a.ldo + cols_valid) * ES, 0x00020000);
+    const int rows_t = cols_valid, cols_t = rows_valid;
+    __amdgpu_buffer_rsrc_t rt = ro;
+    if (a.out_t) {
+      char* tbase_t = reinterpret_cast<char*>(a.out_t) + ((int64_t)n0 * a.ld_out_t + m0) * ES;
+      rt = __builtin_amdgcn_make_buffer_rsrc(tbase_t, 0, ((rows_t - 1) * a.ld_out_t + cols_t) * ES, 0x00020000);
+    }
+    static_for<2>([&](auto jc) {
+      constexpr int j = decltype(jc)::value;
+      const int gcol = j * 32 + c4;
+#pragma unroll
+      for (int e = 0; e < 16; ++e) ws[((e & 3) + 8 * (e >> 2) + 4 * half) * 32 + r] = acc[j][e];
+#pragma unroll
+      for (int p = 0; p < 4; ++p) {
+        f32x4 v = *reinterpret_cast<const f32x4*>(ws + (p * 8 + rr) * 32 + c4);
+#pragma unroll
+        for (int e = 0; e < 4; ++e) {
+          v[e] = (v[e] * a.w_inv + bv[j][e]) * a.out_scale;
+          if (a.epilogue == VFML_EPI_RELU) v[e] = fmaxf(v[e], 0.f);
+        }
+        const int off = gcol < cols_valid ? ((wave * 32 + p * 8 + rr) * a.ldo + gcol) * ES : OOB;
+        if constexpr (H16) {
+          const h16x2 p0 = {(_Float16)v[0], (_Float16)v[1]}, p1 = {(_Float16)v[2], (_Float16)v[3]};
+          const u32x2 hv = {__builtin_bit_cast(unsigned, p0), __builtin_bit_cast(unsigned, p1)};
+          __builtin_amdgcn_raw_buffer_store_b64(hv, ro, off, 0, STORE_NT);
+        } else {
+          __builtin_amdgcn_raw_buffer_store_b128(__builtin_bit_cast(u32x4, v), ro, off, 0, STORE_NT);
+        }
+      }
+      if (a.out_t) {
+#pragma unroll
+        for (int e = 0; e < 16; ++e) {
+          const int row = (e & 3) + 8 * (e >> 2) + 4 * half;
+          ws[r * 32 + ((row + (r >> 1)) & 31)] = acc[j][e];
+        }
+        const int g = lane >> 3, cl = lane & 7;
+#pragma unroll
+        for (int pp = 0; pp < 4; ++pp) {
+          const int c = pp * 8 + cl;
+          f32x4 v;
+#pragma unroll
+          for (int k = 0; k < 4; ++k) v[k] = ws[c * 32 + ((4 * g + k + (c >> 1)) & 31)] * a.w_inv * a.out_scale;
+          const int trow = j * 32 + c;
+          const int q0 = wave * 32 + 4 * g;
+          const bool ok = trow < rows_t && q0 < cols_t;
+          if constexpr (H16) {
+            const h16x2 p0 = {(_Float16)v[0], (_Float16)v[1]}, p1 = {(_Float16)v[2], (_Float16)v[3]};
+            const u32x2 hv = {__builtin_bit_cast(unsigned, p0), __builtin_bit_cast(unsigned, p1)};
+            __builtin_amdgcn_raw_buffer_store_b64(hv, rt, ok ? (trow * a.ld_out_t + q0) * 2 : OOB, 0, STORE_NT);
+          } else {
+            __builtin_amdgcn_raw_buffer_store_b128(__builtin_bit_cast(u32x4, v), rt, ok ? (trow * a.ld_out_t + q0) * 4 : OOB, 0, STORE_NT);
+          }
+        }
+      }
+    });
+    nt = nxt;
+  }
+}
+
+template <bool H16, bool BIAS>
+__device__ __forceinline__ void gemm_resident_walk(const SplitArgs& a, char* smem) {
+  const int units = a.mtiles * a.res_nc;
+  for (int u = blockIdx.x; u < units; u += gridDim.x) {
+    const int run = u / a.mtiles, mt = u - run * a.mtiles;
+    const int nt0 = run * a.res_cl;
+    const int nt1 = nt0 + a.res_cl < a.ntiles ? nt0 + a.res_cl : a.ntiles;
+    gemm_resident_unit<H16, BIAS>(a, smem, mt, ResidentRun{nt0, nt1});
+  }
+}
+
+}
diff --git a/video-flow-ml_amd/vfml/hip.py b/video-flow-ml_amd/vfml/hip.py
--- a/video-flow-ml_amd/vfml/hip.py
+++ b/video-flow-ml_amd/vfml/hip.py
@@ -8,7 +8,7 @@
 _HERE = os.path.dirname(os.path.abspath(__file__))
 LIB_PATH = os.environ.get("VFML_LIB") or os.path.join(_HERE, "libvfml_hip.so")
 CSRC = os.path.join(_HERE, "csrc")
-SOURCES = ["api.hip", "conv_gemm.hip", "conv_gemm_split.hip", "conv_gemm_tapx.hip", "conv_split_plan.hip", "stem.hip", "flow_half.hip", "enc_conv.hip", "norm_pool.hip", "flow_ops.hip", "effects.hip", "correct.hip", "render.hip", "text.hip", "turbulence.hip", "resize.hip", "jpeg.hip", "jpeg_decode.hip", "jpeg_decode_sync.hip", "deflate.hip", "attention.hip", "dwconv.hip", "twins.hip", "warm_start.hip"]
+SOURCES = ["api.hip", "conv_gemm.hip", "conv_gemm_split.hip", "corr_ensure.hip", "conv_gemm_tapx.hip", "conv_split_plan.hip", "stem.hip", "flow_half.hip", "enc_conv.hip", "norm_pool.hip", "flow_ops.hip", "effects.hip", "correct.hip", "render.hip", "text.hip", "turbulence.hip", "resize.hip", "jpeg.hip", "jpeg_decode.hip", "jpeg_decode_sync.hip", "deflate.hip", "attention.hip", "dwconv.hip", "twins.hip", "warm_start.hip"]
 
 STATS_ROWS_F32, STATS_ROWS_S16 = 128, 32
 EPI_NONE, EPI_RELU, EPI_TANH, EPI_SIGMOID, EPI_TANH_RELU, EPI_GRU_ZR, EPI_GRU_Q, EPI_ADD_AUX = range(8)
@@ -56,6 +56,7 @@
 def build(force=False, verbose=False):
     srcs = [os.path.join(CSRC, s) for s in SOURCES]
     hdrs = [os.path.join(CSRC, "vfml_common.h"), os.path.join(CSRC, "conv_split_common.h"),
+            os.path.join(CSRC, "gemm_resident_walk.h"), os.path.join(CSRC, "corr_window.h"),
             os.path.join(CSRC, "jet_table.inc"), os.path.join(CSRC, "jpeg_tables.inc"), os.path.join(CSRC, "jpeg_decode_common.h"),
             os.path.join(CSRC, "jpeg_sync_steps.h"), os.path.join(CSRC, "deflate_code.h"), os.path.join(_HERE, "..", "..", "include", "vfml.h")]
     deps = srcs + hdrs
@@ -148,6 +149,8 @@
                                                   c_int, c_int, c_int, c_int, c_void_p, c_int, c_int, c_void_p, c_int, c_int,
                                                   c_int, c_int, c_int, c_int, c_void_p]
     L.vfml_ptr_table_set.argtypes = [c_void_p, POINTER(c_void_p), c_int, c_void_p]
+    L.vfml_corr_level0_ensure.argtypes = L.vfml_conv2d_split.argtypes[:5] + [c_int, c_int, c_int] + [
+        c_void_p, c_int, c_int, c_int, c_void_p, c_int, c_int, c_int, c_int, c_int, c_int, c_void_p, c_void_p]
     L.vfml_window_seed.argtypes = [c_void_p, c_int, c_int, c_int, c_void_p, c_int, c_int, c_int, c_int, c_void_p]
     L.vfml_tapsum3x3_update.argtypes = [c_void_p, c_int, c_void_p, c_int, c_int, c_int, c_int, ctypes.c_int64, c_void_p, c_void_p,
                                         c_int, c_void_p, c_int, c_int, c_void_p]
@@ -235,7 +238,7 @@
     "vfml_conv2d", "vfml_conv2d_split", "vfml_conv2d_variant", "vfml_conv2d_split_variant", "vfml_conv2d_split_variant_at", "vfml_split_f16", "vfml_to_s16", "vfml_softmax_rows_s16", "vfml_softmax_rows_f16", "vfml_attention_plane_workspace_bytes", "vfml_attention_plane_f16", "vfml_attention_bank_planes_f16", "vfml_axpy_f32", "vfml_dwconv2d", "vfml_gelu_rows", "vfml_layernorm_rows", "vfml_window_attention", "vfml_attention_shared_keys", "vfml_transpose_to_s16", "vfml_add_to_s16",
     "vfml_transpose_split_f16", "vfml_frames_to_nhwc4", "vfml_instnorm_workspace_bytes", "vfml_instnorm_stats",
     "vfml_instnorm_apply", "vfml_instnorm_finalize", "vfml_instnorm_finalize_workspace_bytes", "vfml_avgpool2x2", "vfml_corr_lookup", "vfml_corr_lookup_indirect", "vfml_corr_lookup_indirect_bidir",
-    "vfml_ptr_table_set", "vfml_window_seed", "vfml_coords_update", "vfml_coords_init", "vfml_tapsum3x3", "vfml_tapsum3x3_update", "vfml_flow_rows7", "vfml_flow_half", "vfml_conv3x3_c64",
+    "vfml_ptr_table_set", "vfml_corr_level0_ensure", "vfml_window_seed", "vfml_coords_update", "vfml_coords_init", "vfml_tapsum3x3", "vfml_tapsum3x3_update", "vfml_flow_rows7", "vfml_flow_half", "vfml_conv3x3_c64",
     "vfml_flow_forward_interpolate_workspace_bytes", "vfml_flow_forward_interpolate",
     "vfml_convex_upsample", "vfml_stem7x7s2", "vfml_stem7x7s2_chunks", "vfml_flow_lod", "vfml_flow_encode", "vfml_taa_blend", "vfml_flow_quality_map", "vfml_flow_correct_workspace_bytes", "vfml_flow_correct",
     "vfml_flow_colorize", "vfml_compose_frame", "vfml_flow_decode", "vfml_flow_diff_overlay", "vfml_text_draw",
@@ -611,6 +614,33 @@
         raise ValueError("ptr_table_set: table must be an int64 device tensor with room for the pointers")
     ptrs = (c_void_p * n)(*[t if isinstance(t, int) else t.data_ptr() for t in tensors])
     _check(lib().vfml_ptr_table_set(c_void_p(table.data_ptr()), ptrs, n, _stream()), "vfml_ptr_table_set")
+
+
+def corr_bitmap_words(rows, cols):
+    return ((rows + 127) // 128) * (((cols + 63) // 64 + 31) // 32)
+
+
+def corr_level0_ensure(rows, c, weight, level0, n_rows, n_cols, ldo, out_scale, cells, centres, dirs, dir_cells, coords,
+                       coords_off, ld_coords, dir_coords, h, w, radius, vol_tile, counter=None, in_fmt=FMT_S16, mfma=1):
+    if not isinstance(weight, SplitWeight) or weight.lo is None:
+        raise ValueError("corr_level0_ensure: the target operand is a SplitWeight")
+    ndirs = 2 if dirs == 2 else 1
+    if not (cells.is_cuda and cells.dtype == torch.int64 and cells.numel() >= 4 * ((ndirs - 1) * dir_cells + centres)):
+        raise ValueError("corr_level0_ensure: cells must be an int64 device tensor, four per direction and centre frame")
+    if counter is not None and not (counter.is_cuda and counter.dtype == torch.int32):
+        raise ValueError("corr_level0_ensure: the counter is an int32 device tensor")
+    d = ConvDesc()
+    d.in0, d.c0, d.ld0 = _ptr(_dev(rows)), c, c
+    d.n, d.h, d.w = 1, 1, n_rows
+    d.cout, d.kh, d.kw, d.stride, d.pad_h, d.pad_w = n_cols, 1, 1, 1, 0, 0
+    d.out, d.ldo = _ptr(_dev(level0)), ldo
+    d.epilogue, d.split, d.out_scale = EPI_NONE, 0, out_scale
+    d.flags = {3: 0, 2: CONV_MFMA2, 1: CONV_MFMA1}[mfma]
+    _check(lib().vfml_corr_level0_ensure(ctypes.byref(d), c_void_p(weight.hi.data_ptr()), c_void_p(weight.lo.data_ptr()),
+                                         weight.kp, weight.scale, in_fmt, FMT_F32, weight.order, c_void_p(cells.data_ptr()),
+                                         centres, ndirs, dir_cells, _ptr(_dev(coords), coords_off), ld_coords, dir_coords, h, w,
+                                         radius, vol_tile, c_void_p(counter.data_ptr()) if counter is not None else None,
+                                         _stream()), "vfml_corr_level0_ensure")
 
 
 SEED_NONE, SEED_LOAD, SEED_STORE = 0, 1, 2
diff --git a/video-flow-ml_amd/vfml/network.py b/video-flow-ml_amd/vfml/network.py
--- a/video-flow-ml_amd/vfml/network.py
+++ b/video-flow-ml_amd/vfml/network.py
@@ -776,7 +776,7 @@
         return self._run(src.contiguous(), src.shape[0], src.shape[2], src.shape[3], return_lowres)
 
     @torch.no_grad()
-    def forward_u8(self, frames, return_lowres=True, frame_keys=None, tri_batch=False, pick_only=False):
+    def forward_u8(self, frames, return_lowres=True, frame_keys=None, tri_batch=False, pick_only=False, dense_corr=False):
         if not (isinstance(frames, torch.Tensor) and frames.is_cuda and frames.dtype == torch.uint8
                 and frames.dim() == 4 and frames.shape[3] == 3):
             raise ValueError("forward_u8 expects a uint8 [N,H,W,3] device tensor")
@@ -785,7 +785,7 @@
         if tri_batch and not self.tri_frame:
             raise ValueError("tri_batch applies to tri-frame (BOF) networks")
         return self._run(frames.contiguous(), frames.shape[0], frames.shape[1], frames.shape[2], return_lowres,
-                         frame_keys, tri_batch, pick_only and not return_lowres)
+                         frame_keys, tri_batch, pick_only and not return_lowres, dense_corr)
 
     FEATURE_CACHE_FRAMES = 12
     FMAP_ROW_SCALE = 16.0
@@ -895,17 +895,46 @@
         return types.SimpleNamespace(L=L, AF=AF, hl=hl, wl=wl, Sl=Sl, VT=VT, Nl=Nl, Pv=Pv, TILE=TILE, vol16=mask, VF=VF,
                                      VFl=VFl, ldl=ldl, psz=psz)
 
-    def _window_pyramids(self, feats, keys, N, geo, dev):
+    corr_on_demand = True
+
+    def _corr_scale(self, AF):
+        scale = 1.0 / float(self.cfg.feat_dim) ** 0.5
+        if AF == hip.FMT_S16:
+            scale /= self.FMAP_ROW_SCALE
+        return scale
+
+    def _level0_on_demand(self, keys, N, geo, dense_corr=False):
+        return (self.corr_on_demand and not dense_corr and keys is not None and self._split() and not self.tri_frame
+                and not self.gma and not self.sk and geo.AF == hip.FMT_S16 and geo.Pv % 4 == 0 and geo.Nl[0] >= 1024
+                and geo.VT is not None and geo.Pv == geo.Nl[0] and geo.VFl[0] == hip.FMT_F32 and self._nm("corr") == 1
+                and self.cfg.feat_dim <= 256 and 2 * (N - 2) <= 8 and (geo.Nl[0] + 63) // 64 <= 2048)
+
+    @staticmethod
+    def _pyramid_bitmap(pyr, L):
+        return pyr[L].view(torch.int32)
+
+    def corr_tiles_computed(self, reset=True):
+        count = self._ws.get("ensure_count")
+        if count is None:
+            return 0
+        n = int(count.item())
+        if reset:
+            count.zero_()
+        return n
+
+    def _window_pyramids(self, feats, keys, N, geo, dev, on_demand=False):
         D, L = self.cfg.feat_dim, geo.L
         AF, VFl, Nl, Pv, ldl, psz = geo.AF, geo.VFl, geo.Nl, geo.Pv, geo.ldl, geo.psz
-        scale = 1.0 / float(D) ** 0.5
-        if AF == hip.FMT_S16:
-            scale /= self.FMAP_ROW_SCALE
+        scale = self._corr_scale(AF)
         lim = 2 * (N - 2) + 2
         pyrs = {"f": [], "b": []}
+        od = ("od",) if on_demand else ()
+        if on_demand:
+            psz = psz + [hip.corr_bitmap_words(Pv, Nl[0])]
+        first = 1 if on_demand else 0
         for c in range(1, N - 1):
             for d, tgt in (("f", c + 1), ("b", c - 1)):
-                pk = ("p", keys[c], keys[tgt]) if keys is not None else None
+                pk = ("p", keys[c], keys[tgt]) + od if keys is not None else None
                 if pk is not None and self.gma and d == "b" and keys[c] == keys[tgt]:
                     pk += ("b",)
                 pyr = self._cache_get("p", pk) if pk is not None else None
@@ -915,7 +944,7 @@
                     else:
                         pyr = self._pyramid_buffers(psz, dev, limit=lim)
                         self._cache_put("p", pk, pyr, limit=lim)
-                    rk = ("p", keys[tgt], keys[c]) if pk is not None else None
+                    rk = ("p", keys[tgt], keys[c]) + od if pk is not None else None
                     gemm_form = AF == hip.FMT_S16 and Pv % 4 == 0 and Nl[0] >= 1024
                     dual = rk is not None and d == "f" and gemm_form and ("p", rk) not in self._feat_cache
                     rev = None
@@ -923,7 +952,7 @@
                         rev = self._pyramid_buffers(psz, dev, limit=lim)
                         self._cache_put("p", rk, rev, limit=lim)
                     cnm = self._nm("corr") if self._split() else 3
-                    for l in range(L):
+                    for l in range(first, L):
                         hip.conv2d(feats[c][0], D, D, 1, 1, Pv, feats[tgt][1][l], None, Nl[l], 1, 1, pyr[l],
                                    ldl[l], out_scale=scale, in_fmt=AF, out_fmt=VFl[l],
                                    swap_cross=(d == "b" and l == 0 and gemm_form and cnm == 3),
@@ -933,8 +962,24 @@
                         for l in range(1, L):
                             hip.conv2d(feats[tgt][0], D, D, 1, 1, Pv, feats[c][1][l], None, Nl[l], 1, 1, rev[l],
                                        ldl[l], out_scale=scale, in_fmt=AF, out_fmt=VFl[l], mfma=cnm)
+                    if on_demand:
+                        for p in (pyr, rev) if dual else (pyr,):
+                            self._pyramid_bitmap(p, L).zero_()
                 pyrs[d].append(pyr)
         return pyrs
+
+    def _ensure_plan(self, pyrs, feats, N, geo, dev):
+        M = N - 2
+        cells = self._buf("ensure_cells", 64, dev, torch.int64)
+        ptrs = []
+        for d, step in (("f", 1), ("b", -1)):
+            for i, c in enumerate(range(1, N - 1)):
+                pyr = pyrs[d][i]
+                ptrs += [feats[c][0], feats[c + step][1][0].hi, pyr[0], self._pyramid_bitmap(pyr, geo.L)]
+        hip.ptr_table_set(cells, ptrs)
+        count = self._buf("ensure_count", 1, dev, torch.int32, zero=True)
+        return types.SimpleNamespace(cells=cells, M=M, rows=feats[1][0], weight=feats[2][1][0], level0=pyrs["f"][0][0],
+                                     D=self.cfg.feat_dim, scale=self._corr_scale(geo.AF), counter=count)
 
     def _frame_features(self, src, sel, keys, H, W, P, dev, L, hl, wl, Sl, vt=None):
         D = self.cfg.feat_dim
@@ -1094,12 +1139,12 @@
     def _pyramid_tables(self, pyrs, dev, M, L, cor_p):
         if 2 * M <= 8 and 2 * M * L <= 48:
             tab_fb = self._buf("pyr_table_fb", 64, dev, torch.int64)
-            hip.ptr_table_set(tab_fb, [p for d in ("f", "b") for m in pyrs[d] for p in m])
+            hip.ptr_table_set(tab_fb, [p for d in ("f", "b") for m in pyrs[d] for p in m[:L]])
             return (tab_fb,), (2, cor_p, M)
         tab_f = self._buf("pyr_table_f", 64, dev, torch.int64)
         tab_b = self._buf("pyr_table_b", 64, dev, torch.int64)
-        hip.ptr_table_set(tab_f, [p for m in pyrs["f"] for p in m])
-        hip.ptr_table_set(tab_b, [p for m in pyrs["b"] for p in m])
+        hip.ptr_table_set(tab_f, [p for m in pyrs["f"] for p in m[:L]])
+        hip.ptr_table_set(tab_b, [p for m in pyrs["b"] for p in m[:L]])
         return (tab_f, tab_b), None
 
     def _gma_readout(self, s, win, ng):
@@ -1119,6 +1164,8 @@
                 ub.flow_half(s, ne, r0)
                 join = torch.cuda.Event()
                 join.record()
+        if win.ensure is not None:
+            ub.ensure_level0(s, ne, r0, win.ensure)
         ub.lookup(s, ne, r0, win.tables, win.bidir)
         ub.convc1(s, ne, r0)
         ub.convc2(s, ne, r0)
@@ -1152,7 +1199,7 @@
         blk(f"{ub}.flow_head", P, G, GLD, s.HH, ng, h, w, s.delta, 4, 0, ws, out_fmt=hip.FMT_F32)
         update_block.update_coords(s, ng)
 
-    def _run(self, src, N, H, W, return_lowres, frame_keys=None, tri_batch=False, pick_only=False):
+    def _run(self, src, N, H, W, return_lowres, frame_keys=None, tri_batch=False, pick_only=False, dense_corr=False):
         cfg = self.cfg
         if N < 3:
             raise ValueError(f"need at least 3 frames, got {N}")
@@ -1187,7 +1234,8 @@
                 keys = [(k, H, W, L, self._plan_key(), self._packed_serial) for k in frame_keys]
 
             feats = self._frame_features(src, list(range(N)), keys, H, W, P, dev, L, geo.hl, geo.wl, geo.Sl, vt=geo.VT)
-            pyrs = self._window_pyramids(feats, keys, N, geo, dev)
+            on_demand = self._level0_on_demand(keys, N, geo, dense_corr)
+            pyrs = self._window_pyramids(feats, keys, N, geo, dev, on_demand)
             s = self._window_state(P, dev, M, h, w, geo, R, AF, cor_p)
             ctx = self._frame_context(src, list(range(1, N - 1)), keys, H, W, P, dev, Pn, M)
             win = types.SimpleNamespace(M=M, dev=dev, att_slots=(), readout=None)
@@ -1201,6 +1249,7 @@
             win.gates = self._gate_addends(ctx, dev, Pn, M)
             win.sk_ws = self._sk_workspace(MP, dev) if self.sk else None
             win.tables, win.bidir = self._pyramid_tables(pyrs, dev, M, L, cor_p)
+            win.ensure = self._ensure_plan(pyrs, feats, N, geo, dev) if on_demand else None
             no, nflows = (1, 1) if short else (M, 2 * M)
             up_fixed = self._buf("up_out", nflows * H * W * 2, dev)
             mask = self._buf("mask", MP * 1152, dev)
@@ -1234,7 +1283,7 @@
                                                 up_fixed, out_off=(d * M + c) * H * W * 2)
 
             gkey = (H, W, N, M, bool(tri_batch), bool(pick_only), cfg.decoder_depth, L, R, self._plan_key(), geo.vol16,
-                    self._packed_serial, str(dev), os.environ.get("VFML_FLOW_BRANCH", "0"), win.warm, win.att_slots)
+                    self._packed_serial, str(dev), os.environ.get("VFML_FLOW_BRANCH", "0"), win.warm, win.att_slots, on_demand)
             if self.sk:
                 gkey += ("sk",)
             self._pre_body = torch.cuda.Event()
diff --git a/video-flow-ml_amd/vfml/update_block.py b/video-flow-ml_amd/vfml/update_block.py
--- a/video-flow-ml_amd/vfml/update_block.py
+++ b/video-flow-ml_amd/vfml/update_block.py
@@ -31,6 +31,13 @@
     for d, tab in enumerate(tables):
         hip.corr_lookup(None, g.hl, g.wl, g.ldl, s.R, s.Pn, s.coords1, r0 * 4 + 2 * d, 4, s.corr, r0 * s.ld_corr + d * s.cor_p,
                         s.ld_corr, out_fmt=s.AF, table=tab[t0:], nmaps=n, vol_fmt=g.VF, vol_tile=g.TILE, bidir=bidir)
+
+
+def ensure_level0(s, n, r0, en):
+    g = s.geo
+    c0 = r0 // s.Pn
+    hip.corr_level0_ensure(en.rows, en.D, en.weight, en.level0, g.Pv, g.Nl[0], g.ldl[0], en.scale, en.cells[4 * c0:], n, 2,
+                           en.M, s.coords1, r0 * 4, 4, 2, g.hl[0], g.wl[0], s.R, g.TILE, counter=en.counter, in_fmt=s.AF)
 
 
 def convc1(s, n, r0):
```

After: 50.03 (median of 6 runs). 7.4% higher.
